# ColinWine/Multi-modal-Multi-label-Facial-Action-Unit-Detection-with-Transformer

Hardware: NVIDIA B200
Metric: AVFormer hot-path clips/sec (forward) (higher is better)
Workload: dtype bf16

## Files before the change

include/avformer_b200.h:

```cpp
#ifndef AVFORMER_B200_H_
#define AVFORMER_B200_H_

#include <stddef.h>
#include <stdint.h>

#ifdef __cplusplus
extern "C" {
#endif

#define AVF_ABI_VERSION 1

enum { AVF_FP32 = 0, AVF_BF16 = 1 };
enum { AVF_EINVAL = -1, AVF_ENODEVICE = -2, AVF_EWORKSPACE = -3, AVF_EUNSUPPORTED = -4 };

enum { AVF_EPI_BIAS = 1, AVF_EPI_GELU = 2, AVF_EPI_RESIDUAL = 4, AVF_EPI_DGELU = 8 ,
       AVF_EPI_SAVE_PRE = 16 ,
       AVF_EPI_DROPOUT = 32 ,
       AVF_EPI_ACCUMULATE = 64  };

typedef struct avf_layer_weights {
  const float* ln1_gamma;
  const float* ln1_beta;
  const void*  w_qkv;
  const void*  w_out;
  const float* b_out;
  const float* ln2_gamma;
  const float* ln2_beta;
  const void*  w_ff1;
  const float* b_ff1;
  const void*  w_ff2;
  const float* b_ff2;
} avf_layer_weights;

typedef struct avf_stack_shape {
  int32_t n_seq;
  int32_t n_tok;
  int32_t dim;
  int32_t heads;
  int32_t dim_head;
  int32_t mlp_dim;
  int32_t depth;
} avf_stack_shape;

int         avf_abi_version(void);
const char* avf_last_error(void);
uint64_t    avf_launch_count(void);
int         avf_device_info(int32_t* sm_count, int32_t* cc, int32_t* has_tcgen05);

int         avf_set_fused_enabled(int enabled);
int         avf_encoder_fused_supported(const avf_stack_shape* s, int mode);
int         avf_set_sm_cap(int cap);
int         avf_set_pdl_enabled(int enabled);
int         avf_debug_fused_prof(uint64_t* out64, int reset);
int         avf_debug_set_trap_buffer(void* host_mapped_words);
int         avf_debug_tmap_cache(uint64_t* hits, uint64_t* misses);
int         avf_debug_gemm_prof(uint64_t* out16);

size_t avf_encoder_workspace_bytes(const avf_stack_shape* s, int mode);

int avf_encoder_stack_fwd(int mode, const avf_stack_shape* s, const avf_layer_weights* layers,
                          float* x, int32_t ld_x, float* out, int32_t ld_out,
                          void* workspace, size_t workspace_bytes, void* stream);

int avf_layernorm_fwd(int out_mode, const float* x, int32_t ld_x, const float* gamma, const float* beta,
                      void* y, int32_t rows, int32_t dim, void* stream);
int avf_linear_fwd(int mode, const void* a, int32_t lda, const void* w, const float* bias,
                   const float* residual, int32_t ld_res, void* c, int32_t ldc, int c_mode,
                   int32_t m, int32_t n, int32_t k, int epilogue_flags, void* stream);
int avf_attention_fwd(int io_mode, const void* qkv, void* out, int32_t n_seq, int32_t n_tok,
                      int32_t heads, int32_t dim_head, void* stream);

int avf_sformer_tokens_pack(int io_mode, const void* fmap, const float* pos, float* x,
                            int32_t n_frames, int32_t dim, int32_t hw, void* stream);
int avf_sformer_tokens_unpack(int io_mode, const float* x, void* fmap,
                              int32_t n_frames, int32_t dim, int32_t hw, void* stream);
int avf_sformer_fwd(int mode, int io_mode, const avf_stack_shape* s, const avf_layer_weights* layers,
                    const float* pos, const void* fmap_in, void* fmap_out,
                    void* workspace, size_t workspace_bytes, void* stream);
size_t avf_sformer_workspace_bytes(const avf_stack_shape* s, int mode);

int avf_tformer_embed(int io_mode, const void* frames, const float* cls_token, const float* pos, float* x,
                      int32_t n_clips, int32_t n_frames, int32_t dim, void* stream);
size_t avf_tformer_workspace_bytes(const avf_stack_shape* s, int mode);
int avf_tformer_fwd(int mode, int io_mode, const avf_stack_shape* s, const avf_layer_weights* layers, const void* frames,
                    const float* cls_token, const float* pos, float* cls_out, void* workspace, size_t workspace_bytes, void* stream);
int avf_tformer_cls_extract(const float* x, float* cls, int32_t n_clips, int32_t n_tok, int32_t dim, void* stream);

int avf_au_former_front_fwd(int mode, const float* emb, int32_t ld_emb,
                            const float* bn_gamma, const float* bn_beta, const float* bn_mean, const float* bn_var,
                            const void* w_cat, const float* b_cat, const float* pos, float* x,
                            int32_t n_clips, int32_t in_dim, int32_t emb_dim,
                            void* workspace, size_t workspace_bytes, void* stream);
int avf_token_front_fwd(int mode, const float* emb, int32_t ld_emb,
                        const float* bn_gamma, const float* bn_beta, const float* bn_mean, const float* bn_var,
                        const void* w_cat, const float* b_cat, const float* pos, float* x,
                        int32_t n_clips, int32_t in_dim, int32_t emb_dim, int32_t n_tok,
                        void* workspace, size_t workspace_bytes, void* stream);

int avf_au_logits_fwd(const float* x, int32_t ld_x, const float* w_last, float* out21, int32_t* decisions,
                      int32_t n_clips, int32_t dim, void* stream);
int avf_au_bce_loss(const float* logits, int32_t ld_logits, const float* labels, const float* pos_weight,
                    float* loss_out, float* dlogits, int32_t n_clips, void* stream);

int avf_au_confusion_update(const float* pred, int32_t ld_pred, float threshold, const float* labels, int32_t ld_labels, float ignore,
                            uint64_t* counts48, int32_t n_rows, void* stream);

size_t avf_peer_gather_bytes(int32_t world, size_t n_floats);
int avf_logits_push(const float* logits, size_t n_floats, const uint64_t* peer_base, int32_t world, int32_t rank, const uint32_t* state, void* stream);
int avf_logits_wait(const void* my_base, size_t n_floats, int32_t world, uint32_t* state, uint64_t timeout_ns, void* stream);

size_t avf_peer_allreduce_bytes(int32_t world, size_t n_floats);
int avf_grad_allreduce(const uint64_t* peer_base, size_t n_floats, int32_t world, int32_t rank, uint32_t* state, uint64_t timeout_ns, void* stream);

int avf_adam_allreduce_step(const uint64_t* peer_base, size_t n_floats, int32_t world, int32_t rank, uint32_t* state, uint64_t timeout_ns,
                            float* params, float* exp_avg, float* exp_avg_sq, void* bf16_shadow, float lr, float beta1, float beta2, float eps,
                            float weight_decay, int32_t step, int decoupled, float grad_scale, void* stream);

int avf_cast_f32_to_bf16(const float* src, void* dst, size_t n, void* stream);
int avf_cast_bf16_to_f32(const void* src, float* dst, size_t n, void* stream);
int avf_add_row_periodic(float* x, int32_t ld_x, const float* pos, int32_t rows, int32_t dim, int32_t period, void* stream);


typedef struct avf_layer_grads {
  float* ln1_gamma; float* ln1_beta; float* w_qkv; float* w_out; float* b_out;
  float* ln2_gamma; float* ln2_beta; float* w_ff1; float* b_ff1; float* w_ff2; float* b_ff2;
} avf_layer_grads;

size_t avf_gemm_workspace_bytes(int mode, int trans_a, int trans_b, int32_t m, int32_t n, int32_t k);
int avf_gemm(int mode, int trans_a, int trans_b, const void* a, int32_t lda, const void* b, int32_t ldb,
             const float* bias, const float* residual, int32_t ld_res, void* aux, int32_t ld_aux,
             void* c, int32_t ldc, int c_mode, int32_t m, int32_t n, int32_t k, int epilogue_flags,
             void* workspace, size_t workspace_bytes, void* stream);

size_t avf_encoder_tape_bytes(const avf_stack_shape* s, int mode);
size_t avf_encoder_bwd_workspace_bytes(const avf_stack_shape* s, int mode);
int avf_encoder_stack_fwd_train(int mode, const avf_stack_shape* s, const avf_layer_weights* layers,
                                const float* x, int32_t ld_x, float* out, int32_t ld_out,
                                void* tape, size_t tape_bytes, float dropout_p, uint64_t dropout_seed,
                                const uint32_t* dropout_salt, void* stream);
int avf_encoder_stack_bwd(int mode, const avf_stack_shape* s, const avf_layer_weights* layers,
                          const void* tape, size_t tape_bytes, float* dx, int32_t ld_dx,
                          const avf_layer_grads* grads, int accumulate, void* workspace, size_t workspace_bytes,
                          float dropout_p, uint64_t dropout_seed, const uint32_t* dropout_salt, void* stream);
int avf_dropout_mask(float dropout_p, uint64_t dropout_seed, const uint32_t* dropout_salt, int32_t layer, int32_t site,
                     int32_t rows, int32_t cols, float* out, void* stream);

size_t avf_colsum_workspace_bytes(int32_t rows, int32_t cols);
int avf_colsum(int in_mode, const void* x, size_t ld, int32_t rows, int32_t cols, float* out,
               void* workspace, size_t workspace_bytes, void* stream);
size_t avf_layernorm_bwd_workspace_bytes(int32_t rows, int32_t dim);
int avf_layernorm_bwd(const float* x, int32_t ld_x, const float* gamma, const float* dy_norm, float* dres, int32_t ld_d,
                      void* dx_bf16, float* dgamma, float* dbeta, float* dbias, int32_t rows, int32_t dim,
                      void* workspace, size_t workspace_bytes, void* stream);
int avf_attention_bwd(int io_mode, const void* qkv, const void* dout, void* dqkv, int32_t n_seq, int32_t n_tok,
                      int32_t heads, int32_t dim_head, void* stream);

size_t avf_au_former_front_tape_bytes(int mode, int32_t n_clips, int32_t in_dim);
int avf_au_former_front_fwd_train(int mode, const float* emb, int32_t ld_emb,
                                  const float* bn_gamma, const float* bn_beta, float* bn_mean, float* bn_var,
                                  int batch_stats, float momentum, const void* w_cat, const float* b_cat, const float* pos,
                                  float* x, int32_t n_clips, int32_t in_dim, int32_t emb_dim,
                                  void* tape, size_t tape_bytes, void* stream);
size_t avf_au_former_front_bwd_workspace_bytes(int mode, int32_t n_clips, int32_t in_dim, int32_t emb_dim);
int avf_au_former_front_bwd(int mode, const float* emb, int32_t ld_emb, const float* bn_gamma,
                            const float* bn_mean, const float* bn_var, int batch_stats, const void* w_cat,
                            const void* tape, size_t tape_bytes, const float* dx,
                            float* demb, int32_t ld_demb, float* dbn_gamma, float* dbn_beta, float* dw_cat, float* db_cat,
                            int32_t n_clips, int32_t in_dim, int32_t emb_dim,
                            void* workspace, size_t workspace_bytes, void* stream);

int avf_au_logits_bwd(const float* dlogits, int32_t ld_dlogits, const float* x, int32_t ld_x, const float* w_last,
                      float* dx, int32_t ld_dx, float* dw_last, int32_t n_clips, int32_t dim, void* stream);

int avf_adam_step(float* params, const float* grads, float* exp_avg, float* exp_avg_sq, void* bf16_shadow, size_t n,
                  float lr, float beta1, float beta2, float eps, float weight_decay, int32_t step, int decoupled,
                  float grad_scale, void* stream);

#ifdef __cplusplus
}
#endif
#endif
```

multi-modal-multi-label-facial-action-unit-detection-with-transformer_b200/_lib.py:

```python
from __future__ import annotations

import ctypes
import glob
import os
import shutil
import subprocess
import threading

_PKG = os.path.dirname(os.path.abspath(__file__))
_ROOT = os.path.dirname(_PKG)
_CSRC = os.path.join(_PKG, "csrc")
LIB_PATH = os.path.join(_PKG, "libavformer_b200.so")
_OVERRIDE = os.environ.get("AVF_LIB_OVERRIDE", "")

NVCC_FLAGS = [
    "-gencode", "arch=compute_100a,code=sm_100a", "-lineinfo", "-O3", "-std=c++17",
    "-Xcompiler", "-fPIC", "-shared", "-cudart", "static", "-t", "0",
]

AVF_FP32, AVF_BF16 = 0, 1
EPI_BIAS, EPI_GELU, EPI_RESIDUAL, EPI_DGELU, EPI_SAVE_PRE = 1, 2, 4, 8, 16

_c_p = ctypes.c_void_p
_i32 = ctypes.c_int32
_sz = ctypes.c_size_t


class LayerWeights(ctypes.Structure):
    _fields_ = [(n, _c_p) for n in ("ln1_gamma", "ln1_beta", "w_qkv", "w_out", "b_out", "ln2_gamma", "ln2_beta",
                                    "w_ff1", "b_ff1", "w_ff2", "b_ff2")]


class LayerGrads(ctypes.Structure):
    _fields_ = LayerWeights._fields_


class StackShape(ctypes.Structure):
    _fields_ = [(n, _i32) for n in ("n_seq", "n_tok", "dim", "heads", "dim_head", "mlp_dim", "depth")]


SIGNATURES = {
    "avf_abi_version": (ctypes.c_int, []),
    "avf_last_error": (ctypes.c_char_p, []),
    "avf_launch_count": (ctypes.c_uint64, []),
    "avf_device_info": (ctypes.c_int, [ctypes.POINTER(_i32)] * 3),
    "avf_set_fused_enabled": (ctypes.c_int, [ctypes.c_int]),
    "avf_encoder_fused_supported": (ctypes.c_int, [ctypes.POINTER(StackShape), ctypes.c_int]),
    "avf_debug_fused_prof": (ctypes.c_int, [ctypes.POINTER(ctypes.c_uint64), ctypes.c_int]),
    "avf_encoder_workspace_bytes": (_sz, [ctypes.POINTER(StackShape), ctypes.c_int]),
    "avf_encoder_stack_fwd": (ctypes.c_int, [ctypes.c_int, ctypes.POINTER(StackShape), ctypes.POINTER(LayerWeights), _c_p, _i32,
                                             _c_p, _i32, _c_p, _sz, _c_p]),
    "avf_layernorm_fwd": (ctypes.c_int, [ctypes.c_int, _c_p, _i32, _c_p, _c_p, _c_p, _i32, _i32, _c_p]),
    "avf_linear_fwd": (ctypes.c_int, [ctypes.c_int, _c_p, _i32, _c_p, _c_p, _c_p, _i32, _c_p, _i32, ctypes.c_int, _i32, _i32, _i32,
                                      ctypes.c_int, _c_p]),
    "avf_attention_fwd": (ctypes.c_int, [ctypes.c_int, _c_p, _c_p, _i32, _i32, _i32, _i32, _c_p]),
    "avf_sformer_tokens_pack": (ctypes.c_int, [ctypes.c_int, _c_p, _c_p, _c_p, _i32, _i32, _i32, _c_p]),
    "avf_sformer_tokens_unpack": (ctypes.c_int, [ctypes.c_int, _c_p, _c_p, _i32, _i32, _i32, _c_p]),
    "avf_sformer_workspace_bytes": (_sz, [ctypes.POINTER(StackShape), ctypes.c_int]),
    "avf_sformer_fwd": (ctypes.c_int, [ctypes.c_int, ctypes.c_int, ctypes.POINTER(StackShape), ctypes.POINTER(LayerWeights), _c_p, _c_p,
                                       _c_p, _c_p, _sz, _c_p]),
    "avf_tformer_embed": (ctypes.c_int, [ctypes.c_int, _c_p, _c_p, _c_p, _c_p, _i32, _i32, _i32, _c_p]),
    "avf_tformer_workspace_bytes": (_sz, [ctypes.POINTER(StackShape), ctypes.c_int]),
    "avf_tformer_fwd": (ctypes.c_int, [ctypes.c_int, ctypes.c_int, ctypes.POINTER(StackShape), ctypes.POINTER(LayerWeights), _c_p, _c_p, _c_p, _c_p,
                                       _c_p, _sz, _c_p]),
    "avf_tformer_cls_extract": (ctypes.c_int, [_c_p, _c_p, _i32, _i32, _i32, _c_p]),
    "avf_au_former_front_fwd": (ctypes.c_int, [ctypes.c_int, _c_p, _i32, _c_p, _c_p, _c_p, _c_p, _c_p, _c_p, _c_p, _c_p, _i32, _i32, _i32,
                                               _c_p, _sz, _c_p]),
    "avf_token_front_fwd": (ctypes.c_int, [ctypes.c_int, _c_p, _i32, _c_p, _c_p, _c_p, _c_p, _c_p, _c_p, _c_p, _c_p, _i32, _i32, _i32, _i32,
                                           _c_p, _sz, _c_p]),
    "avf_au_logits_fwd": (ctypes.c_int, [_c_p, _i32, _c_p, _c_p, _c_p, _i32, _i32, _c_p]),
    "avf_au_bce_loss": (ctypes.c_int, [_c_p, _i32, _c_p, _c_p, _c_p, _c_p, _i32, _c_p]),
    "avf_au_confusion_update": (ctypes.c_int, [_c_p, _i32, ctypes.c_float, _c_p, _i32, ctypes.c_float, _c_p, _i32, _c_p]),
    "avf_peer_gather_bytes": (_sz, [_i32, _sz]),
    "avf_logits_push": (ctypes.c_int, [_c_p, _sz, _c_p, _i32, _i32, _c_p, _c_p]),
    "avf_logits_wait": (ctypes.c_int, [_c_p, _sz, _i32, _c_p, ctypes.c_uint64, _c_p]),
    "avf_peer_allreduce_bytes": (_sz, [_i32, _sz]),
    "avf_grad_allreduce": (ctypes.c_int, [_c_p, _sz, _i32, _i32, _c_p, ctypes.c_uint64, _c_p]),
    "avf_adam_allreduce_step": (ctypes.c_int, [_c_p, _sz, _i32, _i32, _c_p, ctypes.c_uint64, _c_p, _c_p, _c_p, _c_p] + [ctypes.c_float] * 5
                                + [_i32, ctypes.c_int, ctypes.c_float, _c_p]),
    "avf_cast_f32_to_bf16": (ctypes.c_int, [_c_p, _c_p, _sz, _c_p]),
    "avf_cast_bf16_to_f32": (ctypes.c_int, [_c_p, _c_p, _sz, _c_p]),
    "avf_add_row_periodic": (ctypes.c_int, [_c_p, _i32, _c_p, _i32, _i32, _i32, _c_p]),
    "avf_gemm_workspace_bytes": (_sz, [ctypes.c_int, ctypes.c_int, ctypes.c_int, _i32, _i32, _i32]),
    "avf_gemm": (ctypes.c_int, [ctypes.c_int, ctypes.c_int, ctypes.c_int, _c_p, _i32, _c_p, _i32, _c_p, _c_p, _i32, _c_p, _i32, _c_p, _i32,
                                ctypes.c_int, _i32, _i32, _i32, ctypes.c_int, _c_p, _sz, _c_p]),
    "avf_encoder_tape_bytes": (_sz, [ctypes.POINTER(StackShape), ctypes.c_int]),
    "avf_encoder_bwd_workspace_bytes": (_sz, [ctypes.POINTER(StackShape), ctypes.c_int]),
    "avf_encoder_stack_fwd_train": (ctypes.c_int, [ctypes.c_int, ctypes.POINTER(StackShape), ctypes.POINTER(LayerWeights), _c_p, _i32, _c_p, _i32,
                                                   _c_p, _sz, ctypes.c_float, ctypes.c_uint64, _c_p, _c_p]),
    "avf_encoder_stack_bwd": (ctypes.c_int, [ctypes.c_int, ctypes.POINTER(StackShape), ctypes.POINTER(LayerWeights), _c_p, _sz, _c_p, _i32,
                                             ctypes.POINTER(LayerGrads), ctypes.c_int, _c_p, _sz, ctypes.c_float, ctypes.c_uint64, _c_p, _c_p]),
    "avf_dropout_mask": (ctypes.c_int, [ctypes.c_float, ctypes.c_uint64, _c_p, _i32, _i32, _i32, _i32, _c_p, _c_p]),
    "avf_set_sm_cap": (ctypes.c_int, [ctypes.c_int]),
    "avf_set_pdl_enabled": (ctypes.c_int, [ctypes.c_int]),
    "avf_debug_set_trap_buffer": (ctypes.c_int, [_c_p]),
    "avf_debug_gemm_prof": (ctypes.c_int, [ctypes.POINTER(ctypes.c_uint64)]),
    "avf_debug_tmap_cache": (ctypes.c_int, [ctypes.POINTER(ctypes.c_uint64), ctypes.POINTER(ctypes.c_uint64)]),
    "avf_colsum_workspace_bytes": (_sz, [_i32, _i32]),
    "avf_colsum": (ctypes.c_int, [ctypes.c_int, _c_p, _sz, _i32, _i32, _c_p, _c_p, _sz, _c_p]),
    "avf_layernorm_bwd_workspace_bytes": (_sz, [_i32, _i32]),
    "avf_layernorm_bwd": (ctypes.c_int, [_c_p, _i32, _c_p, _c_p, _c_p, _i32, _c_p, _c_p, _c_p, _c_p, _i32, _i32, _c_p, _sz, _c_p]),
    "avf_attention_bwd": (ctypes.c_int, [ctypes.c_int, _c_p, _c_p, _c_p, _i32, _i32, _i32, _i32, _c_p]),
    "avf_au_former_front_tape_bytes": (_sz, [ctypes.c_int, _i32, _i32]),
    "avf_au_former_front_fwd_train": (ctypes.c_int, [ctypes.c_int, _c_p, _i32, _c_p, _c_p, _c_p, _c_p, ctypes.c_int, ctypes.c_float, _c_p, _c_p,
                                                     _c_p, _c_p, _i32, _i32, _i32, _c_p, _sz, _c_p]),
    "avf_au_former_front_bwd_workspace_bytes": (_sz, [ctypes.c_int, _i32, _i32, _i32]),
    "avf_au_former_front_bwd": (ctypes.c_int, [ctypes.c_int, _c_p, _i32, _c_p, _c_p, _c_p, ctypes.c_int, _c_p, _c_p, _sz, _c_p, _c_p, _i32,
                                               _c_p, _c_p, _c_p, _c_p, _i32, _i32, _i32, _c_p, _sz, _c_p]),
    "avf_au_logits_bwd": (ctypes.c_int, [_c_p, _i32, _c_p, _i32, _c_p, _c_p, _i32, _c_p, _i32, _i32, _c_p]),
    "avf_adam_step": (ctypes.c_int, [_c_p, _c_p, _c_p, _c_p, _c_p, _sz] + [ctypes.c_float] * 5 + [_i32, ctypes.c_int, ctypes.c_float, _c_p]),
}

_lock = threading.Lock()
_lib = None


def sources():
    return sorted(glob.glob(os.path.join(_CSRC, "*.cu")))


def _stale() -> bool:
    if not os.path.exists(LIB_PATH):
        return True
    t = os.path.getmtime(LIB_PATH)
    deps = sources() + glob.glob(os.path.join(_CSRC, "*.cuh")) + glob.glob(os.path.join(_CSRC, "*.h")) + \
        [os.path.join(_ROOT, "include", "avformer_b200.h")]
    return any(os.path.getmtime(d) > t for d in deps)


def build(force: bool = False, verbose: bool = False, out: str = "") -> str:
    if out:
        force = True
    if not force and not _stale():
        return LIB_PATH
    nvcc = shutil.which("nvcc") or "/usr/local/cuda/bin/nvcc"
    if not os.path.exists(nvcc):
        raise RuntimeError("avformer_b200: nvcc not found and libavformer_b200.so is missing/stale; cannot build the CUDA path")
    extra = os.environ.get("AVF_NVCC_EXTRA", "").split()
    cmd = [nvcc] + NVCC_FLAGS + extra + (["-Xptxas", "-v"] if verbose else []) + ["-o", out or LIB_PATH] + sources()
    res = subprocess.run(cmd, capture_output=True, text=True)
    if res.returncode != 0:
        raise RuntimeError("avformer_b200: nvcc failed\n" + res.stdout + res.stderr)
    if verbose:
        print(res.stderr)
    return out or LIB_PATH


def lib() -> ctypes.CDLL:
    global _lib
    if _lib is not None:
        return _lib
    with _lock:
        if _lib is None:
            if _OVERRIDE:
                handle = ctypes.CDLL(_OVERRIDE)
            else:
                try:
                    build()
                except RuntimeError:
                    if not os.path.exists(LIB_PATH):
                        raise
                handle = ctypes.CDLL(LIB_PATH)
            for name, (res, args) in SIGNATURES.items():
                fn = getattr(handle, name)
                fn.restype, fn.argtypes = res, args
            if os.environ.get("AVF_PDL", "") in ("0", "off"):
                handle.avf_set_pdl_enabled(0)
            if handle.avf_abi_version() != 1:
                raise RuntimeError("avformer_b200: ABI version mismatch")
            _lib = handle
    return _lib


def check(rc: int, what: str = "") -> None:
    if rc != 0:
        msg = lib().avf_last_error().decode("utf-8", "replace")
        raise RuntimeError(f"avformer_b200 {what} failed (code {rc}): {msg}")
```

multi-modal-multi-label-facial-action-unit-detection-with-transformer_b200/csrc/avf_api.cu:

```cuda
#include <atomic>
#include <cstdarg>
#include <cstdio>
#include <cstring>

#include "avf_common.cuh"
#include "avf_internal.h"

namespace avf {

static thread_local char g_err[512] = "";
static std::atomic<uint64_t> g_launches{0};
static std::atomic<int> g_pdl{1};
bool pdl_enabled() { return g_pdl.load() != 0; }
static std::atomic<int> g_sm_cap{0};
int sm_cap() { return g_sm_cap.load(); }
static std::atomic<int> g_fused{1};

void count_launch() { g_launches.fetch_add(1, std::memory_order_relaxed); }

void set_error(const char* fmt, ...) {
  va_list ap;
  va_start(ap, fmt);
  vsnprintf(g_err, sizeof(g_err), fmt, ap);
  va_end(ap);
}

int check_cuda(cudaError_t e, const char* what) {
  if (e == cudaSuccess) return 0;
  set_error("CUDA error %d (%s) at %s", int(e), cudaGetErrorString(e), what);
  return int(e);
}

static int require_device() {
  static int state = 0;
  if (state == 0) {
    int n = 0;
    cudaError_t e = cudaGetDeviceCount(&n);
    if (e != cudaSuccess || n == 0) {
      cudaGetLastError();
      state = -1;
    } else {
      state = 1;
    }
  }
  if (state < 0) {
    set_error("no CUDA device: the AVFormer B200 path has no CPU fallback");
    return AVF_ENODEVICE;
  }
  return 0;
}

static bool tcgen05_ok() {
  static int state = 0;
  if (state == 0) {
    int dev = 0, major = 0;
    if (cudaGetDevice(&dev) == cudaSuccess && cudaDeviceGetAttribute(&major, cudaDevAttrComputeCapabilityMajor, dev) == cudaSuccess)
      state = (major == 10) ? 1 : -1;
    else
      state = -1;
  }
  return state > 0;
}

static inline size_t align_up(size_t v, size_t a = 256) { return (v + a - 1) / a * a; }
static inline size_t elt(int mode) { return mode == AVF_BF16 ? 2 : 4; }

struct EncoderWs {
  void* ln;
  void* qkv;
  void* attn;
  void* hid;
  size_t total;
};

static EncoderWs carve_encoder_ws(const avf_stack_shape* s, int mode, void* base) {
  const size_t R = size_t(s->n_seq) * s->n_tok, I = size_t(s->heads) * s->dim_head, e = elt(mode);
  uint8_t* p = static_cast<uint8_t*>(base);
  EncoderWs w;
  size_t off = 0;
  w.ln = p + off;   off += align_up(R * s->dim * e);
  w.qkv = p + off;  off += align_up(R * 3 * I * e);
  w.attn = p + off; off += align_up(R * I * e);
  w.hid = p + off;  off += align_up(R * s->mlp_dim * e);
  w.total = off;
  return w;
}

static int check_shape(const avf_stack_shape* s) {
  AVF_REQUIRE(s != nullptr, AVF_EINVAL, "null stack shape");
  AVF_REQUIRE(s->n_seq > 0 && s->n_tok > 0 && s->depth > 0, AVF_EINVAL, "empty stack: n_seq=%d n_tok=%d depth=%d", s->n_seq, s->n_tok, s->depth);
  AVF_REQUIRE(s->dim % 128 == 0 && s->dim <= 1536, AVF_EUNSUPPORTED, "dim=%d must be a multiple of 128 (<= 1536)", s->dim);
  AVF_REQUIRE(s->dim_head == 32 || s->dim_head == 64, AVF_EUNSUPPORTED, "dim_head=%d (supported: 32, 64)", s->dim_head);
  AVF_REQUIRE((s->heads * s->dim_head) % 64 == 0 && s->mlp_dim % 64 == 0, AVF_EUNSUPPORTED, "inner=%d / mlp=%d must be multiples of 64", s->heads * s->dim_head, s->mlp_dim);
  AVF_REQUIRE(s->n_tok <= 64, AVF_EUNSUPPORTED, "n_tok=%d: sequences longer than 64 tokens are not part of this path", s->n_tok);
  return 0;
}

int linear(int mode, const void* a, int lda, const void* w, const float* bias, const float* res, int ld_res, void* c, int ldc,
           int c_mode, int m, int n, int k, int flags, cudaStream_t st) {
  if (mode == AVF_BF16) {
    AVF_REQUIRE(tcgen05_ok(), AVF_EUNSUPPORTED, "bf16 mode needs an sm_100 device (tcgen05)");
    return linear_umma(a, lda, w, bias, res, ld_res, c, ldc, c_mode, m, n, k, flags, st);
  }
  return linear_f32(static_cast<const float*>(a), lda, static_cast<const float*>(w), bias, res, ld_res, c, ldc, c_mode, m, n, k, flags, st);
}

static int encoder_stack(int mode, const avf_stack_shape* s, const avf_layer_weights* L, float* x, int ld_x, float* out, int ld_out,
                         void* ws, size_t ws_bytes, cudaStream_t st) {
  int e = check_shape(s);
  if (e) return e;
  AVF_REQUIRE(mode == AVF_BF16 || mode == AVF_FP32, AVF_EINVAL, "mode=%d", mode);
  AVF_REQUIRE(L != nullptr && x != nullptr && ws != nullptr, AVF_EINVAL, "null pointer argument");
  if (mode == AVF_BF16 && g_fused.load() && tcgen05_ok() && encoder_fused_supported(s) && ld_x % 4 == 0 && (out == nullptr || ld_out % 4 == 0))
    return encoder_fused(1, s, L, x, ld_x, out ? out : x, out ? ld_out : ld_x, nullptr, nullptr, st);
  const EncoderWs w = carve_encoder_ws(s, mode, ws);
  AVF_REQUIRE(ws_bytes >= w.total, AVF_EWORKSPACE, "workspace too small: %zu < %zu bytes", ws_bytes, w.total);
  const int R = s->n_seq * s->n_tok, D = s->dim, I = s->heads * s->dim_head, M = s->mlp_dim;
  for (int l = 0; l < s->depth; ++l) {
    const avf_layer_weights& W = L[l];
    if ((e = layernorm(mode, x, ld_x, W.ln1_gamma, W.ln1_beta, w.ln, R, D, st))) return e;
    if ((e = linear(mode, w.ln, D, W.w_qkv, nullptr, nullptr, 0, w.qkv, 3 * I, mode, R, 3 * I, D, 0, st))) return e;
    if ((e = attention_small(mode, w.qkv, w.attn, s->n_seq, s->n_tok, s->heads, s->dim_head, st))) return e;
    if ((e = linear(mode, w.attn, I, W.w_out, W.b_out, x, ld_x, x, ld_x, AVF_FP32, R, D, I, AVF_EPI_BIAS | AVF_EPI_RESIDUAL, st))) return e;
    if ((e = layernorm(mode, x, ld_x, W.ln2_gamma, W.ln2_beta, w.ln, R, D, st))) return e;
    if ((e = linear(mode, w.ln, D, W.w_ff1, W.b_ff1, nullptr, 0, w.hid, M, mode, R, M, D, AVF_EPI_BIAS | AVF_EPI_GELU, st))) return e;
    const bool last = (l == s->depth - 1) && out != nullptr;
    if ((e = linear(mode, w.hid, M, W.w_ff2, W.b_ff2, x, ld_x, last ? out : x, last ? ld_out : ld_x, AVF_FP32, R, D, M,
                    AVF_EPI_BIAS | AVF_EPI_RESIDUAL, st)))
      return e;
  }
  return 0;
}

}

using namespace avf;

extern "C" {

int avf_abi_version(void) { return AVF_ABI_VERSION; }

const char* avf_last_error(void) { return g_err; }

uint64_t avf_launch_count(void) { return g_launches.load(std::memory_order_relaxed); }

int avf_set_fused_enabled(int enabled) {
  const int old = g_fused.exchange(enabled ? 1 : 0);
  return old;
}

int avf_set_pdl_enabled(int enabled) { return g_pdl.exchange(enabled ? 1 : 0); }

int avf_set_sm_cap(int cap) { return g_sm_cap.exchange(cap > 0 ? cap : 0); }

int avf_encoder_fused_supported(const avf_stack_shape* s, int mode) {
  return (s != nullptr && mode == AVF_BF16 && s->n_seq > 0 && encoder_fused_supported(s)) ? 1 : 0;
}

int avf_debug_fused_prof(uint64_t* out64, int reset) { return fused_prof_read(reinterpret_cast<unsigned long long*>(out64), reset); }

int avf_debug_tmap_cache(uint64_t* hits, uint64_t* misses) {
  if (hits == nullptr || misses == nullptr) return AVF_EINVAL;
  tmap_cache_stats(hits, misses);
  return 0;
}

int avf_debug_gemm_prof(uint64_t* out16) { return gemm_prof_read(reinterpret_cast<unsigned long long*>(out16)); }

int avf_debug_set_trap_buffer(void* host_mapped_words) { return fused_set_trap_buffer(host_mapped_words); }

int avf_device_info(int32_t* sm_count, int32_t* cc, int32_t* has_tcgen05) {
  int e = require_device();
  if (e) return e;
  int dev = 0, sms = 0, major = 0, minor = 0;
  AVF_CUDA(cudaGetDevice(&dev));
  AVF_CUDA(cudaDeviceGetAttribute(&sms, cudaDevAttrMultiProcessorCount, dev));
  AVF_CUDA(cudaDeviceGetAttribute(&major, cudaDevAttrComputeCapabilityMajor, dev));
  AVF_CUDA(cudaDeviceGetAttribute(&minor, cudaDevAttrComputeCapabilityMinor, dev));
  if (sm_count) *sm_count = sms;
  if (cc) *cc = major * 10 + minor;
  if (has_tcgen05) *has_tcgen05 = major == 10 ? 1 : 0;
  return 0;
}

size_t avf_encoder_workspace_bytes(const avf_stack_shape* s, int mode) {
  if (s == nullptr || s->n_seq <= 0 || s->n_tok <= 0) return 0;
  return carve_encoder_ws(s, mode, nullptr).total;
}

int avf_encoder_stack_fwd(int mode, const avf_stack_shape* s, const avf_layer_weights* layers, float* x, int32_t ld_x, float* out,
                          int32_t ld_out, void* workspace, size_t workspace_bytes, void* stream) {
  int e = require_device();
  if (e) return e;
  return encoder_stack(mode, s, layers, x, ld_x, out, ld_out, workspace, workspace_bytes, static_cast<cudaStream_t>(stream));
}

int avf_layernorm_fwd(int out_mode, const float* x, int32_t ld_x, const float* gamma, const float* beta, void* y, int32_t rows,
                      int32_t dim, void* stream) {
  int e = require_device();
  if (e) return e;
  AVF_REQUIRE(x && gamma && beta && y, AVF_EINVAL, "layernorm: null pointer");
  return layernorm(out_mode, x, ld_x, gamma, beta, y, rows, dim, static_cast<cudaStream_t>(stream));
}

int avf_linear_fwd(int mode, const void* a, int32_t lda, const void* w, const float* bias, const float* residual, int32_t ld_res,
                   void* c, int32_t ldc, int c_mode, int32_t m, int32_t n, int32_t k, int epilogue_flags, void* stream) {
  int e = require_device();
  if (e) return e;
  AVF_REQUIRE(a && w && c, AVF_EINVAL, "linear: null pointer");
  AVF_REQUIRE(!(epilogue_flags & AVF_EPI_BIAS) || bias, AVF_EINVAL, "linear: bias flag without bias");
  AVF_REQUIRE(!(epilogue_flags & AVF_EPI_RESIDUAL) || residual, AVF_EINVAL, "linear: residual flag without residual");
  return linear(mode, a, lda, w, bias, residual, ld_res, c, ldc, c_mode, m, n, k, epilogue_flags, static_cast<cudaStream_t>(stream));
}

int avf_attention_fwd(int io_mode, const void* qkv, void* out, int32_t n_seq, int32_t n_tok, int32_t heads, int32_t dim_head, void* stream) {
  int e = require_device();
  if (e) return e;
  AVF_REQUIRE(qkv && out, AVF_EINVAL, "attention: null pointer");
  return attention_small(io_mode, qkv, out, n_seq, n_tok, heads, dim_head, static_cast<cudaStream_t>(stream));
}

int avf_sformer_tokens_pack(int io_mode, const void* fmap, const float* pos, float* x, int32_t n_frames, int32_t dim, int32_t hw, void* stream) {
  int e = require_device();
  if (e) return e;
  AVF_REQUIRE(fmap && x, AVF_EINVAL, "sformer_tokens_pack: null pointer");
  return sformer_pack(io_mode, fmap, pos, x, n_frames, dim, hw, static_cast<cudaStream_t>(stream));
}

int avf_sformer_tokens_unpack(int io_mode, const float* x, void* fmap, int32_t n_frames, int32_t dim, int32_t hw, void* stream) {
  int e = require_device();
  if (e) return e;
  AVF_REQUIRE(fmap && x, AVF_EINVAL, "sformer_tokens_unpack: null pointer");
  return sformer_unpack(io_mode, x, fmap, n_frames, dim, hw, static_cast<cudaStream_t>(stream));
}

size_t avf_sformer_workspace_bytes(const avf_stack_shape* s, int mode) {
  if (s == nullptr || s->n_seq <= 0 || s->n_tok <= 0) return 0;
  return align_up(size_t(s->n_seq) * s->n_tok * s->dim * 4) + carve_encoder_ws(s, mode, nullptr).total + align_up(encoder_fused_scratch_bytes());
}

int avf_sformer_fwd(int mode, int io_mode, const avf_stack_shape* s, const avf_layer_weights* layers, const float* pos,
                    const void* fmap_in, void* fmap_out, void* workspace, size_t workspace_bytes, void* stream) {
  int e = require_device();
  if (e) return e;
  if ((e = check_shape(s))) return e;
  AVF_REQUIRE(layers && pos && fmap_in && fmap_out && workspace, AVF_EINVAL, "sformer_fwd: null pointer");
  const size_t need = avf_sformer_workspace_bytes(s, mode);
  AVF_REQUIRE(workspace_bytes >= need, AVF_EWORKSPACE, "workspace too small: %zu < %zu bytes", workspace_bytes, need);
  cudaStream_t st = static_cast<cudaStream_t>(stream);
  if (mode == AVF_BF16 && io_mode == AVF_BF16 && g_fused.load() && tcgen05_ok() && encoder_fused_supported(s))
    return encoder_fused(0, s, layers, fmap_in, 0, fmap_out, 0, pos, workspace, st);
  float* x = static_cast<float*>(workspace);
  const size_t xbytes = align_up(size_t(s->n_seq) * s->n_tok * s->dim * 4);
  if ((e = sformer_pack(io_mode, fmap_in, pos, x, s->n_seq, s->dim, s->n_tok, st))) return e;
  if ((e = encoder_stack(mode, s, layers, x, s->dim, nullptr, 0, static_cast<uint8_t*>(workspace) + xbytes, workspace_bytes - xbytes, st))) return e;
  return sformer_unpack(io_mode, x, fmap_out, s->n_seq, s->dim, s->n_tok, st);
}

int avf_tformer_embed(int io_mode, const void* frames, const float* cls_token, const float* pos, float* x, int32_t n_clips,
                      int32_t n_frames, int32_t dim, void* stream) {
  int e = require_device();
  if (e) return e;
  AVF_REQUIRE(frames && cls_token && pos && x, AVF_EINVAL, "tformer_embed: null pointer");
  return tformer_embed(io_mode, frames, cls_token, pos, x, n_clips, n_frames, dim, static_cast<cudaStream_t>(stream));
}

size_t avf_tformer_workspace_bytes(const avf_stack_shape* s, int mode) {
  if (s == nullptr || s->n_seq <= 0 || s->n_tok <= 0) return 0;
  const size_t B = s->n_seq, D = s->dim, I = size_t(s->heads) * s->dim_head, M = s->mlp_dim, e = elt(mode);
  return align_up(B * s->n_tok * D * 4) + carve_encoder_ws(s, mode, nullptr).total + align_up(B * D * 4) + align_up(B * D * e) + align_up(B * I * e) +
         align_up(B * M * e);
}

int avf_tformer_fwd(int mode, int io_mode, const avf_stack_shape* s, const avf_layer_weights* layers, const void* frames,
                    const float* cls_token, const float* pos, float* cls_out, void* workspace, size_t workspace_bytes, void* stream) {
  int e = require_device();
  if (e) return e;
  if ((e = check_shape(s))) return e;
  AVF_REQUIRE(layers && frames && cls_token && pos && cls_out && workspace, AVF_EINVAL, "tformer_fwd: null pointer");
  AVF_REQUIRE(s->n_tok >= 2, AVF_EINVAL, "tformer_fwd: n_tok=%d (cls + at least one frame)", s->n_tok);
  const size_t need = avf_tformer_workspace_bytes(s, mode);
  AVF_REQUIRE(workspace_bytes >= need, AVF_EWORKSPACE, "workspace too small: %zu < %zu bytes", workspace_bytes, need);
  cudaStream_t st = static_cast<cudaStream_t>(stream);
  const int B = s->n_seq, N = s->n_tok, R = B * N, D = s->dim, I = s->heads * s->dim_head, M = s->mlp_dim;
  uint8_t* p = static_cast<uint8_t*>(workspace);
  float* x = reinterpret_cast<float*>(p);   p += align_up(size_t(R) * D * 4);
  void* enc_ws = p;
  const EncoderWs w = carve_encoder_ws(s, mode, enc_ws);
  p += w.total;
  float* xc = reinterpret_cast<float*>(p);  p += align_up(size_t(B) * D * 4);
  void* lnc = p;                            p += align_up(size_t(B) * D * elt(mode));
  void* oc = p;                             p += align_up(size_t(B) * I * elt(mode));
  void* hc = p;
  if ((e = tformer_embed(io_mode, frames, cls_token, pos, x, B, N - 1, D, st))) return e;
  if (s->depth > 1) {
    avf_stack_shape head = *s;
    head.depth = s->depth - 1;
    if ((e = encoder_stack(mode, &head, layers, x, D, nullptr, 0, enc_ws, w.total, st))) return e;
  }
  const avf_layer_weights& W = layers[s->depth - 1];
  if ((e = layernorm(mode, x, D, W.ln1_gamma, W.ln1_beta, w.ln, R, D, st))) return e;
  if ((e = linear(mode, w.ln, D, W.w_qkv, nullptr, nullptr, 0, w.qkv, 3 * I, mode, R, 3 * I, D, 0, st))) return e;
  if (mode == AVF_BF16) {
    if ((e = attention_mma_bf16(w.qkv, oc, B, N, s->heads, s->dim_head, st, 1))) return e;
  } else {
    if ((e = attention_small(mode, w.qkv, w.attn, B, N, s->heads, s->dim_head, st))) return e;
    AVF_CUDA(cudaMemcpy2DAsync(oc, size_t(I) * 4, w.attn, size_t(N) * I * 4, size_t(I) * 4, B, cudaMemcpyDeviceToDevice, st));
  }
  if ((e = rows_gather(x, size_t(N) * D, xc, B, D, st))) return e;
  if ((e = linear(mode, oc, I, W.w_out, W.b_out, xc, D, xc, D, AVF_FP32, B, D, I, AVF_EPI_BIAS | AVF_EPI_RESIDUAL, st))) return e;
  if ((e = layernorm(mode, xc, D, W.ln2_gamma, W.ln2_beta, lnc, B, D, st))) return e;
  if ((e = linear(mode, lnc, D, W.w_ff1, W.b_ff1, nullptr, 0, hc, M, mode, B, M, D, AVF_EPI_BIAS | AVF_EPI_GELU, st))) return e;
  return linear(mode, hc, M, W.w_ff2, W.b_ff2, xc, D, cls_out, D, AVF_FP32, B, D, M, AVF_EPI_BIAS | AVF_EPI_RESIDUAL, st);
}

int avf_tformer_cls_extract(const float* x, float* cls, int32_t n_clips, int32_t n_tok, int32_t dim, void* stream) {
  int e = require_device();
  if (e) return e;
  AVF_REQUIRE(x && cls, AVF_EINVAL, "tformer_cls_extract: null pointer");
  return rows_gather(x, size_t(n_tok) * dim, cls, n_clips, dim, static_cast<cudaStream_t>(stream));
}

int avf_token_front_fwd(int mode, const float* emb, int32_t ld_emb, const float* bn_gamma, const float* bn_beta, const float* bn_mean,
                        const float* bn_var, const void* w_cat, const float* b_cat, const float* pos, float* x, int32_t n_clips,
                        int32_t in_dim, int32_t emb_dim, int32_t n_tok, void* workspace, size_t workspace_bytes, void* stream) {
  int e = require_device();
  if (e) return e;
  AVF_REQUIRE(emb && bn_gamma && bn_beta && bn_mean && bn_var && w_cat && b_cat && pos && x && workspace, AVF_EINVAL, "token_front: null pointer");
  AVF_REQUIRE(n_clips > 0 && in_dim > 0 && emb_dim > 0 && n_tok > 0, AVF_EINVAL, "token_front: n_clips=%d n_tok=%d", n_clips, n_tok);
  const size_t need = align_up(size_t(n_clips) * in_dim * elt(mode));
  AVF_REQUIRE(workspace_bytes >= need, AVF_EWORKSPACE, "workspace too small: %zu < %zu bytes", workspace_bytes, need);
  cudaStream_t st = static_cast<cudaStream_t>(stream);
  if ((e = bn_rows(mode, emb, ld_emb, bn_gamma, bn_beta, bn_mean, bn_var, workspace, n_clips, in_dim, st))) return e;
  if ((e = linear(mode, workspace, in_dim, w_cat, b_cat, nullptr, 0, x, n_tok * emb_dim, AVF_FP32, n_clips, n_tok * emb_dim, in_dim, AVF_EPI_BIAS, st))) return e;
  return add_row_periodic(x, emb_dim, pos, n_clips * n_tok, emb_dim, n_tok, st);
}

int avf_au_former_front_fwd(int mode, const float* emb, int32_t ld_emb, const float* bn_gamma, const float* bn_beta, const float* bn_mean,
                            const float* bn_var, const void* w_cat, const float* b_cat, const float* pos, float* x, int32_t n_clips,
                            int32_t in_dim, int32_t emb_dim, void* workspace, size_t workspace_bytes, void* stream) {
  return avf_token_front_fwd(mode, emb, ld_emb, bn_gamma, bn_beta, bn_mean, bn_var, w_cat, b_cat, pos, x, n_clips, in_dim, emb_dim, 12, workspace,
                             workspace_bytes, stream);
}

int avf_au_logits_fwd(const float* x, int32_t ld_x, const float* w_last, float* out21, int32_t* decisions, int32_t n_clips, int32_t dim, void* stream) {
  int e = require_device();
  if (e) return e;
  AVF_REQUIRE(x && w_last, AVF_EINVAL, "au_logits: null pointer");
  return au_logits(x, ld_x, w_last, out21, decisions, n_clips, dim, static_cast<cudaStream_t>(stream));
}

int avf_au_bce_loss(const float* logits, int32_t ld_logits, const float* labels, const float* pos_weight, float* loss_out, float* dlogits,
                    int32_t n_clips, void* stream) {
  int e = require_device();
  if (e) return e;
  AVF_REQUIRE(logits && labels && pos_weight && loss_out, AVF_EINVAL, "au_bce_loss: null pointer");
  return au_bce(logits, ld_logits, labels, pos_weight, loss_out, dlogits, n_clips, static_cast<cudaStream_t>(stream));
}

size_t avf_peer_gather_bytes(int32_t world, size_t n_floats) { return (world > 0 && world <= 1024) ? peer_gather_bytes(world, n_floats) : 0; }

int avf_logits_push(const float* logits, size_t n_floats, const uint64_t* peer_base, int32_t world, int32_t rank, const uint32_t* state, void* stream) {
  int e = require_device();
  if (e) return e;
  AVF_REQUIRE(logits && peer_base && state, AVF_EINVAL, "logits_push: null pointer");
  AVF_REQUIRE(world > 0 && world <= 1024 && rank >= 0 && rank < world && n_floats > 0, AVF_EINVAL, "logits_push: world %d rank %d n %zu", world, rank, n_floats);
  return logits_push(logits, n_floats, reinterpret_cast<const unsigned long long*>(peer_base), world, rank, state, static_cast<cudaStream_t>(stream));
}

int avf_logits_wait(const void* my_base, size_t n_floats, int32_t world, uint32_t* state, uint64_t timeout_ns, void* stream) {
  int e = require_device();
  if (e) return e;
  AVF_REQUIRE(my_base && state, AVF_EINVAL, "logits_wait: null pointer");
  AVF_REQUIRE(world > 0 && world <= 1024 && n_floats > 0, AVF_EINVAL, "logits_wait: world %d n %zu", world, n_floats);
  return logits_wait(my_base, n_floats, world, state, timeout_ns, static_cast<cudaStream_t>(stream));
}

size_t avf_peer_allreduce_bytes(int32_t world, size_t n_floats) { return (world > 0 && world <= 16) ? peer_allreduce_bytes(world, n_floats) : 0; }

int avf_grad_allreduce(const uint64_t* peer_base, size_t n_floats, int32_t world, int32_t rank, uint32_t* state, uint64_t timeout_ns, void* stream) {
  int e = require_device();
  if (e) return e;
  AVF_REQUIRE(peer_base && state, AVF_EINVAL, "grad_allreduce: null pointer");
  AVF_REQUIRE(world > 0 && world <= 16 && rank >= 0 && rank < world && n_floats > 0, AVF_EINVAL, "grad_allreduce: world %d (1..16) rank %d n %zu", world, rank, n_floats);
  return grad_allreduce(reinterpret_cast<const unsigned long long*>(peer_base), n_floats, world, rank, state, timeout_ns, static_cast<cudaStream_t>(stream));
}

int avf_adam_allreduce_step(const uint64_t* peer_base, size_t n_floats, int32_t world, int32_t rank, uint32_t* state, uint64_t timeout_ns, float* params,
                            float* exp_avg, float* exp_avg_sq, void* bf16_shadow, float lr, float beta1, float beta2, float eps, float weight_decay, int32_t step,
                            int decoupled, float grad_scale, void* stream) {
  int e = require_device();
  if (e) return e;
  AVF_REQUIRE(peer_base && state, AVF_EINVAL, "adam_allreduce_step: null pointer");
  AVF_REQUIRE(world > 0 && world <= 16 && rank >= 0 && rank < world && n_floats > 0, AVF_EINVAL, "adam_allreduce_step: world %d (1..16) rank %d n %zu", world, rank, n_floats);
  return adam_allreduce_step(reinterpret_cast<const unsigned long long*>(peer_base), n_floats, world, rank, state, timeout_ns, params, exp_avg, exp_avg_sq, bf16_shadow,
                             lr, beta1, beta2, eps, weight_decay, step, decoupled, grad_scale, static_cast<cudaStream_t>(stream));
}

int avf_au_confusion_update(const float* pred, int32_t ld_pred, float threshold, const float* labels, int32_t ld_labels, float ignore,
                            uint64_t* counts48, int32_t n_rows, void* stream) {
  int e = require_device();
  if (e) return e;
  return au_confusion(pred, ld_pred, threshold, labels, ld_labels, ignore, reinterpret_cast<unsigned long long*>(counts48), n_rows,
                      static_cast<cudaStream_t>(stream));
}

int avf_cast_f32_to_bf16(const float* src, void* dst, size_t n, void* stream) {
  int e = require_device();
  if (e) return e;
  AVF_REQUIRE((src && dst) || n == 0, AVF_EINVAL, "cast: null pointer");
  return cast_f32_bf16(src, dst, n, static_cast<cudaStream_t>(stream));
}

int avf_cast_bf16_to_f32(const void* src, float* dst, size_t n, void* stream) {
  int e = require_device();
  if (e) return e;
  AVF_REQUIRE((src && dst) || n == 0, AVF_EINVAL, "cast: null pointer");
  return cast_bf16_f32(src, dst, n, static_cast<cudaStream_t>(stream));
}

int avf_add_row_periodic(float* x, int32_t ld_x, const float* pos, int32_t rows, int32_t dim, int32_t period, void* stream) {
  int e = require_device();
  if (e) return e;
  AVF_REQUIRE(x && pos, AVF_EINVAL, "add_row_periodic: null pointer");
  return add_row_periodic(x, ld_x, pos, rows, dim, period, static_cast<cudaStream_t>(stream));
}

}
```

multi-modal-multi-label-facial-action-unit-detection-with-transformer_b200/csrc/avf_internal.h:

```cpp
#pragma once
#include <cuda_runtime.h>
#include <stddef.h>

#include "../../include/avformer_b200.h"
#include "avf_common.cuh"

namespace avf {

int layernorm(int out_mode, const float* x, int ld_x, const float* g, const float* b, void* y, int rows, int dim, cudaStream_t st);
int bn_rows(int out_mode, const float* x, int ld_x, const float* g, const float* b, const float* mean, const float* var, void* y,
            int rows, int dim, cudaStream_t st);
int sformer_pack(int io_mode, const void* fmap, const float* pos, float* x, int n_frames, int dim, int hw, cudaStream_t st);
int sformer_unpack(int io_mode, const float* x, void* fmap, int n_frames, int dim, int hw, cudaStream_t st);
int tformer_embed(int io_mode, const void* frames, const float* cls, const float* pos, float* x, int n_clips, int T, int dim, cudaStream_t st);
int rows_gather(const float* x, size_t src_row_stride, float* y, int rows, int dim, cudaStream_t st);
int add_row_periodic(float* x, int ld_x, const float* pos, int rows, int dim, int period, cudaStream_t st);
int cast_f32_bf16(const float* s, void* d, size_t n, cudaStream_t st);
int cast_bf16_f32(const void* s, float* d, size_t n, cudaStream_t st);
int au_logits(const float* x, int ld_x, const float* w_last, float* out21, int* decisions, int n_clips, int dim, cudaStream_t st);
int au_bce(const float* logits, int ld, const float* labels, const float* pw, float* loss_out, float* dlogits, int n_clips, cudaStream_t st);
size_t peer_gather_bytes(int world, size_t n);
int logits_push(const float* logits, size_t n, const unsigned long long* peer_base, int world, int rank, const uint32_t* state, cudaStream_t st);
size_t peer_allreduce_bytes(int world, size_t n);
int grad_allreduce(const unsigned long long* peer_base, size_t n, int world, int rank, uint32_t* state, unsigned long long timeout_ns, cudaStream_t st);
int adam_allreduce_step(const unsigned long long* peer_base, size_t n, int world, int rank, uint32_t* state, unsigned long long timeout_ns, float* p, float* m,
                        float* v, void* shadow, float lr, float b1, float b2, float eps, float wd, int step, int decoupled, float grad_scale, cudaStream_t st);
int logits_wait(const void* my_base, size_t n, int world, uint32_t* state, unsigned long long timeout_ns, cudaStream_t st);
int au_confusion(const float* pred, int ld_pred, float thresh, const float* labels, int ld_lab, float ignore, unsigned long long* counts, int n_rows,
                 cudaStream_t st);

int linear_f32(const float* a, int lda, const float* w, const float* bias, const float* res, int ld_res, void* c, int ldc,
               int c_mode, int m, int n, int k, int flags, cudaStream_t st);
int attention_small(int io_mode, const void* qkv, void* out, int n_seq, int n_tok, int heads, int dim_head, cudaStream_t st);

int gemm_f32(int trans_a, int trans_b, const float* a, int lda, const float* w, int ldw, const float* bias, const float* res, int ld_res,
             float* aux, int ld_aux, void* c, int ldc, int c_mode, int m, int n, int k, int flags, cudaStream_t st, DropSpec drop = DropSpec{});

size_t colsum_workspace_bytes(int rows, int cols);
int colsum(int in_mode, const void* x, size_t ld, int rows, int cols, float* out, float beta, void* ws, size_t ws_bytes, cudaStream_t st);
size_t layernorm_bwd_workspace_bytes(int rows, int dim);
int layernorm_bwd(const float* x, int ld_x, const float* gamma, const float* dyn, float* dres, int ld_d, void* dxb, int dxb_mode, float* dgamma,
                  float* dbeta, float* dbias, float beta_acc, int rows, int dim, void* ws, size_t ws_bytes, cudaStream_t st,
                  DropSpec drop_in = DropSpec{}, DropSpec drop_out = DropSpec{});
int masked_copy(const float* x, void* y, int y_mode, int rows, int dim, DropSpec drop, cudaStream_t st);
int dropout_mask(float* out, int rows, int cols, DropSpec drop, cudaStream_t st);
int attention_bwd(int io_mode, const void* qkv, const void* dout, void* dqkv, int n_seq, int n_tok, int heads, int dim_head, cudaStream_t st);
int au_logits_bwd(const float* dl, int ld_dl, const float* x, int ld_x, const float* w_last, float* dx, int ld_dx, float* dw, int n_clips,
                  int dim, cudaStream_t st);
int bn_train_fwd(int out_mode, const float* x, int ld_x, const float* g, const float* b, float* run_mean, float* run_var, float momentum,
                 void* y, float* save_mean, float* save_rstd, int rows, int dim, cudaStream_t st);
int bn_bwd(const float* x, int ld_x, const float* dy, const float* g, const float* mean, const float* rstd_or_var, int batch_stats, float* dx,
           int ld_dx, float* dgamma, float* dbeta, int rows, int dim, cudaStream_t st);
int adam_step(float* p, const float* g, float* m, float* v, void* shadow, size_t n, float lr, float b1, float b2, float eps, float wd, int step,
              int decoupled, float grad_scale, cudaStream_t st);

int attention_mma_bf16(const void* qkv, void* out, int n_seq, int n_tok, int heads, int dim_head, cudaStream_t st, int q_rows = 0);
int attention_bwd_mma_bf16(const void* qkv, const void* dout, void* dqkv, int n_seq, int n_tok, int heads, int dim_head, cudaStream_t st);

bool encoder_fused_supported(const avf_stack_shape* s);
int fused_prof_read(unsigned long long* out64, int reset);
int fused_set_trap_buffer(void* host_mapped_words);
size_t encoder_fused_scratch_bytes();
int encoder_fused(int io_kind, const avf_stack_shape* s, const avf_layer_weights* L, const void* in, int ld_in, void* out, int ld_out,
                  const float* pos, void* scratch, cudaStream_t st);

int gemm_umma(int trans_a, int trans_b, const void* a, int lda, const void* w, int ldw, const float* bias, const float* res, int ld_res,
              const void* aux, int ld_aux, void* c, int ldc, int c_mode, int m, int n, int k, int flags, void* ws, size_t ws_bytes,
              cudaStream_t stream, DropSpec drop = DropSpec{});
size_t gemm_umma_workspace_bytes(int m, int n, int k);
void tmap_cache_stats(uint64_t* hits, uint64_t* misses);
int gemm_prof_read(unsigned long long* out16);
int linear_umma(const void* a, int lda, const void* w, const float* bias, const float* res, int ld_res, void* c, int ldc,
                int c_mode, int m, int n, int k, int flags, cudaStream_t st);

}
```

multi-modal-multi-label-facial-action-unit-detection-with-transformer_b200/csrc/avf_layer_fused.cu:

```cuda
#include <cuda.h>
#include <stdlib.h>

#include "avf_common.cuh"
#include "avf_fused_helpers.cuh"
#include "avf_internal.h"

namespace avf {

int make_tmap_bf16_2d(CUtensorMap* tm, const void* ptr, uint64_t rows, uint64_t cols, uint64_t ld, uint32_t box_rows, uint32_t box_cols = 64);

namespace {
using namespace fused;

#ifndef AVF_PROD_POLL
#define AVF_PROD_POLL 2
#endif
#ifndef AVF_PROD_FASTPATH
#define AVF_PROD_FASTPATH 1
#endif
#ifndef AVF_O_TMEM
#define AVF_O_TMEM 1
#endif

constexpr int DIM = 256, HEADS = 8, DH = 32;
constexpr int MAX_DEPTH = 3, MAX_MLP = 1024;
#ifndef AVF_FUSED_NSPLIT
#define AVF_FUSED_NSPLIT 2
#endif
constexpr int NSPLIT = AVF_FUSED_NSPLIT;
static_assert(NSPLIT == 2, "two threads per token row (the packed softmax exchanges a pair)");
constexpr int WORKER_T0 = 96;
constexpr int NUM_WORKERS = 128 * NSPLIT;
constexpr int NUM_THREADS = WORKER_T0 + NUM_WORKERS;
constexpr int RING = 9, RING_LO = 2, RING_HI = 4, SLOT_BYTES = 16384;
#ifndef AVF_QRING
#define AVF_QRING 6
#endif
constexpr int QRING = AVF_QRING, QSLOT_BYTES = 12288;
#ifndef AVF_MLP_GROUP
#define AVF_MLP_GROUP 4
#endif
constexpr int MLPG = AVF_MLP_GROUP;
static_assert(MLPG == 2 || MLPG == 4, "MLP group size");

constexpr int OFF_A0 = 0;
constexpr int OFF_Q = 65536;
constexpr int OFF_K = OFF_Q + 8192;
constexpr int OFF_V = OFF_K + 8192;
constexpr int OFF_RING = OFF_V + 16384;
constexpr int OFF_OST = OFF_RING + (RING_HI - RING_LO) * SLOT_BYTES;
constexpr int OFF_QRING = OFF_OST + (AVF_O_TMEM ? 0 : 8192);
constexpr int OFF_OUTST = OFF_QRING;
static_assert(QRING * QSLOT_BYTES >= 2 * 64 * 256 * 2, "the NCHW output staging lives in the QKV ring");
static_assert(QRING >= 6 && QRING < 8, "one head-full barrier per head parity needs 6 or 7 sub-slots (see qkv_producer_main)");
constexpr int QRING_END = OFF_QRING + QRING * QSLOT_BYTES;
constexpr int OFF_XCH = QRING_END > OFF_Q + RING * SLOT_BYTES ? QRING_END : OFF_Q + RING * SLOT_BYTES;
static_assert(OFF_XCH - OFF_Q >= RING * SLOT_BYTES, "the nine MLP ring slots fit in [OFF_Q, OFF_XCH)");
static_assert(OFF_RING == OFF_Q + RING_LO * SLOT_BYTES, "ring slots are contiguous from OFF_Q");
__host__ __device__ constexpr int slot_offset(uint32_t s) { return OFF_Q + int(s) * SLOT_BYTES; }
constexpr int OFF_VEC = OFF_XCH + 2 * 128 * 4 * 4;
constexpr int V_BOUT = 0, V_BFF2 = 256, V_BFF1 = 512;
constexpr int V_B16 = V_BFF1 + MAX_MLP;
constexpr int OFF_BAR = OFF_VEC + (V_B16 + 512) * 4;
constexpr int SMEM_USED = OFF_BAR + 512;
constexpr int SMEM_ALLOC = SMEM_USED + 1024;
static_assert(SMEM_ALLOC <= 232448, "shared memory budget");

#ifndef AVF_A0_HALF
#define AVF_A0_HALF 1
#endif
#if AVF_A0_HALF
__device__ __forceinline__ constexpr int kpanel(int i) { return ((i & 1) << 1) | (i >> 1); }
#else
__device__ __forceinline__ constexpr int kpanel(int i) { return i; }
#endif

constexpr uint32_t TM_X = 0, TM_D1 = 256, TM_O = 352, TM_S = 384, TM_H0 = 256, TM_H1 = 384;

enum {
  B_RING_FULL = 0, B_RING_EMPTY = RING, B_X0_FULL = 2 * RING, B_A0_FREE, B_A0_READY, B_D1_FULL, B_STAGED, B_S_FULL, B_P_READY, B_O_FULL,
  B_O_DRAINED, B_X1_FULL, B_HACC_FULL, B_HACC_FULL1, B_H_READY, B_H_READY1, B_X2_FULL,
  B_QG_FULL, B_QR_EMPTY = B_QG_FULL + 2, B_A1_FREE = B_QR_EMPTY + QRING, B_OUT_READ, B_QKV_FREE, B_G_FULL, B_TQ_FULL = B_G_FULL + 8, B_A0_HALF = B_TQ_FULL + 4, NUM_BARS
};
static_assert(NUM_BARS * 8 + 8 + 16 <= 512, "barrier block (+ TMEM slot + tile queue)");

__device__ __forceinline__ int* tile_queue(uint64_t* bars) { return reinterpret_cast<int*>(bars + NUM_BARS) + 2; }
__device__ __forceinline__ int next_tile(uint64_t* bars, uint32_t k) {
  mbar_wait(&bars[B_TQ_FULL + (k & 3u)], (k >> 2) & 1u);
  return *reinterpret_cast<volatile int*>(tile_queue(bars) + (k & 3u));
}

enum { IO_NCHW_BF16 = 0, IO_ROWS_F32 = 1 };
constexpr int POS_LD = 64;

enum { PW_INPUT = 0, PW_VEC, PW_LN1, PW_WAIT_D1, PW_E1, PW_WAIT_O, PW_E3, PW_WAIT_S, PW_E2, PW_WAIT_X1, PW_LN2, PW_WAIT_HACC, PW_GELU, PW_WAIT_X2,
       PW_OUTPUT, PW_TILES, PW_E2_LD, PW_E2_EXP, PW_E2_XCH, PW_E2_ST,
       PM_WAIT_A0 = 32, PM_QKV, PM_WAIT_STAGED, PM_S, PM_WAIT_P, PM_PV, PM_WAIT_OD7, PM_OUT, PM_WAIT_A0B, PM_FF1, PM_WAIT_H, PM_FF2, PM_RINGWAIT,
       PM_RW_QKV, PM_RW_OUT, PM_RW_FF1, PM_RW_FF2, PM_REFILL_CYC, PM_REFILL_N };

struct LayerArgs {
  CUtensorMap tm_qkv, tm_out, tm_w1, tm_w2;
  const float *ln1_g, *ln1_b, *b_out, *ln2_g, *ln2_b, *b_ff1, *b_ff2;
  uint64_t pad_;
};

struct FusedArgs {
  LayerArgs layer[MAX_DEPTH];
  const void* in;
  void* out;
  const float* pos;
  const float* pos_t;
  int ld_in, ld_out;
  int* tile_counter;
  int n_seq, n_tok, slot, slot_log2, spt, n_tiles, n_chunks, depth;
};

__device__ unsigned* g_trap_buffer = nullptr;

constexpr int CW = DIM / NSPLIT;

struct Worker {
  uint8_t* smem;
  uint64_t* bars;
  const float* vec;
  uint32_t tl;
  int lane, q, g, row;
  uint32_t xslot;

  __device__ __forceinline__ const float* exchange(float mine) {
    float* s = reinterpret_cast<float*>(smem + OFF_XCH) + xslot * (128 * 4);
    xslot ^= 1;
    s[row * 4 + g] = mine;
    bar_sync(1 + q, 32 * NSPLIT);
    return s + row * 4;
  }
  __device__ __forceinline__ float2 exchange_pair(float a, float b) {
    static_assert(NSPLIT == 2, "pair exchange is written for two threads per row");
    float* s = reinterpret_cast<float*>(smem + OFF_XCH) + xslot * (128 * 4);
    xslot ^= 1;
    *reinterpret_cast<float2*>(s + row * 4 + g * 2) = make_float2(a, b);
    bar_sync(1 + q, 32 * NSPLIT);
    return *reinterpret_cast<const float2*>(s + row * 4 + (g ^ 1) * 2);
  }
  __device__ __forceinline__ float exchange_sum(float mine) {
    const float* v = exchange(mine);
    if constexpr (NSPLIT == 2) return v[0] + v[1];
    const float4 f = *reinterpret_cast<const float4*>(v);
    return (f.x + f.y) + (f.z + f.w);
  }
  __device__ __forceinline__ float exchange_max(float mine) {
    const float* v = exchange(mine);
    if constexpr (NSPLIT == 2) return fmaxf(v[0], v[1]);
    const float4 f = *reinterpret_cast<const float4*>(v);
    return fmaxf(fmaxf(f.x, f.y), fmaxf(f.z, f.w));
  }
  __device__ __forceinline__ void arrive(int bar) {
    fence_proxy_async_smem();
    tc_fence_before();
    __syncwarp();
    if (lane == 0) mbar_arrive(&bars[bar]);
  }
  __device__ __forceinline__ void arrive_tmem_only(int bar) {
    tc_fence_before();
    __syncwarp();
    if (lane == 0) mbar_arrive(&bars[bar]);
  }
  struct Stats {
    float shift, s, ss;
    __device__ __forceinline__ void add(const float (&x)[32], bool first) {
      if (first) shift = x[0];
      const uint64_t nshift = f2_pack(-shift, -shift);
      uint64_t s2 = f2_pack(0.f, 0.f), q2 = s2;
#pragma unroll
      for (int j = 0; j < 32; j += 2) {
        const uint64_t d = f2_add(f2_pack(x[j], x[j + 1]), nshift);
        s2 = f2_add(s2, d);
        q2 = f2_fma(d, d, q2);
      }
      float a, b;
      f2_unpack(s2, a, b);
      s += a + b;
      f2_unpack(q2, a, b);
      ss += a + b;
    }
  };
  __device__ __forceinline__ void finish_stats(const Stats& st, float& mean, float& rstd) {
    constexpr float n = float(CW);
    const float mean_g = st.shift + st.s * (1.f / n);
    const float m2_g = fmaxf(st.ss - st.s * st.s * (1.f / n), 0.f);
    mean = exchange_sum(mean_g) * (1.f / NSPLIT);
    const float dm = mean_g - mean;
    const float m2 = exchange_sum(fmaf(dm * dm, n, m2_g));
    rstd = rsqrtf(m2 * (1.f / DIM) + 1e-5f);
  }
  __device__ __forceinline__ void stats_from_tmem(float& mean, float& rstd) {
    Stats st{0.f, 0.f, 0.f};
#pragma unroll
    for (int c0 = 0; c0 < CW; c0 += 32) {
      float x[32];
      tmem_ld32(tl + TM_X + g * CW + c0, reinterpret_cast<uint32_t(&)[32]>(x));
      tmem_ld_wait();
      st.add(x, c0 == 0);
    }
    finish_stats(st, mean, rstd);
  }
  __device__ __forceinline__ void normalize_from_tmem(float mean, float rstd, int ln_sel, int v_next_bias) {
    const int cbase = g * CW;
    const float nmr = -mean * rstd;
    const uint64_t rstd2 = f2_pack(rstd, rstd), nmr2 = f2_pack(nmr, nmr);
#pragma unroll 1
    for (int c0 = 0; c0 < CW; c0 += 32) {
      float x[32];
      tmem_ld32(tl + TM_X + cbase + c0, reinterpret_cast<uint32_t(&)[32]>(x));
      tmem_ld_wait();
      const int col0 = cbase + c0;
      uint8_t* dst = smem + OFF_A0 + (col0 >> 6) * 16384 + row * 128;
      const int chunk0 = (col0 & 63) >> 3;
#pragma unroll
      for (int ch = 0; ch < 4; ++ch) {
        const __nv_bfloat16* v16 = reinterpret_cast<const __nv_bfloat16*>(vec + V_B16) + ln_sel * 512 + col0 + ch * 8;
        const uint4 gm = *reinterpret_cast<const uint4*>(v16), bt = *reinterpret_cast<const uint4*>(v16 + 256);
        uint4 pk;
        pk.x = fma_bf16x2(cvt_bf16x2_pair(f2_fma(f2_pack(x[ch * 8], x[ch * 8 + 1]), rstd2, nmr2)), gm.x, bt.x);
        pk.y = fma_bf16x2(cvt_bf16x2_pair(f2_fma(f2_pack(x[ch * 8 + 2], x[ch * 8 + 3]), rstd2, nmr2)), gm.y, bt.y);
        pk.z = fma_bf16x2(cvt_bf16x2_pair(f2_fma(f2_pack(x[ch * 8 + 4], x[ch * 8 + 5]), rstd2, nmr2)), gm.z, bt.z);
        pk.w = fma_bf16x2(cvt_bf16x2_pair(f2_fma(f2_pack(x[ch * 8 + 6], x[ch * 8 + 7]), rstd2, nmr2)), gm.w, bt.w);
        *reinterpret_cast<uint4*>(dst + (((chunk0 + ch) ^ (row & 7)) << 4)) = pk;
      }
#pragma unroll
      for (int j = 0; j < 32; j += 4) {
        const ulonglong2 b = *reinterpret_cast<const ulonglong2*>(vec + v_next_bias + col0 + j);
        f2_unpack(f2_add(f2_pack(x[j], x[j + 1]), b.x), x[j], x[j + 1]);
        f2_unpack(f2_add(f2_pack(x[j + 2], x[j + 3]), b.y), x[j + 2], x[j + 3]);
      }
      tmem_st32(tl + TM_X + col0, reinterpret_cast<const uint32_t(&)[32]>(x));
#if AVF_A0_HALF
      if (c0 == 32) arrive(B_A0_HALF);
#endif
    }
    tmem_st_wait();
    arrive(B_A0_READY);
  }
};

template <int NC, int TAILV>
__device__ __forceinline__ float softmax_fixed(Worker& w, uint32_t ts, uint32_t tp, float sm_scale, Prof& pf) {
  float s[NC][8];
#pragma unroll
  for (int c = 0; c < NC; ++c) tmem_ld8(ts + c * 8, reinterpret_cast<uint32_t(&)[8]>(s[c]));
  tmem_ld_wait();
  pf.mark(PW_E2_LD);
  float mc[NC];
#pragma unroll
  for (int c = 0; c < NC; ++c) {
    if (TAILV > 0 && c == NC - 1) {
      mc[c] = s[c][0];
#pragma unroll
      for (int j = 1; j < 8; ++j)
        if (j < TAILV) mc[c] = fmaxf(mc[c], s[c][j]);
    } else {
      mc[c] = fmaxf(fmaxf(fmaxf(s[c][0], s[c][1]), fmaxf(s[c][2], s[c][3])), fmaxf(fmaxf(s[c][4], s[c][5]), fmaxf(s[c][6], s[c][7])));
    }
  }
  float mloc = mc[0];
#pragma unroll
  for (int c = 1; c < NC; ++c) mloc = fmaxf(mloc, mc[c]);
  pf.mark(PW_E2_EXP);
  const float mrow = w.exchange_max(mloc);
  pf.mark(PW_E2_XCH);
  const float nml = -mrow * sm_scale;
  const uint64_t sc2 = f2_pack(sm_scale, sm_scale), nml2 = f2_pack(nml, nml);
  uint64_t sum2 = f2_pack(0.f, 0.f);
  float sum_lo = 0.f;
#pragma unroll
  for (int c = 0; c < NC; ++c) {
    const int nv = (TAILV > 0 && c == NC - 1) ? TAILV : 8;
    uint32_t e[4];
#pragma unroll
    for (int j = 0; j < 4; ++j) {
      if (2 * j + 1 < nv) {
        e[j] = ex2_bf16x2(cvt_bf16x2_pair(f2_fma(f2_pack(s[c][2 * j], s[c][2 * j + 1]), sc2, nml2)));
        sum2 = f2_add(sum2, f2_pack(__uint_as_float(e[j] << 16), __uint_as_float(e[j] & 0xFFFF0000u)));
      } else if (2 * j < nv) {
        e[j] = ex2_bf16x2(cvt_bf16x2(fmaf(s[c][2 * j], sm_scale, nml), -INFINITY)) & 0xFFFFu;
        sum_lo += __uint_as_float(e[j] << 16);
      } else {
        e[j] = 0u;
      }
    }
    tmem_st4(tp + c * 4, e[0], e[1], e[2], e[3]);
  }
  float a, b;
  f2_unpack(sum2, a, b);
  return sum_lo + (a + b);
}

__host__ __device__ constexpr int slot_of(int n_tok) { return n_tok <= 16 ? 16 : (n_tok <= 32 ? 32 : 64); }
__host__ __device__ constexpr int log2_of(int v) { return v == 16 ? 4 : (v == 32 ? 5 : 6); }

template <int IO, int NTOK>
__device__ void worker_main(const FusedArgs& a, uint8_t* smem, uint64_t* bars, uint32_t tmem) {
  Worker w;
  w.smem = smem;
  w.bars = bars;
  w.vec = reinterpret_cast<const float*>(smem + OFF_VEC);
  const int wt = threadIdx.x - WORKER_T0;
  w.lane = wt & 31;
  w.q = (threadIdx.x >> 5) & 3;
  w.g = wt >> 7;
  w.row = w.q * 32 + w.lane;
  w.tl = tmem + (uint32_t(w.q * 32) << 16);
  w.xslot = 0;
  const int q = w.q, g = w.g, row = w.row;
  const uint32_t tl = w.tl;
  const float* vec = w.vec;
  const int n_tok = NTOK ? NTOK : a.n_tok, slot = NTOK ? slot_of(NTOK) : a.slot, spt = NTOK ? 128 / slot_of(NTOK) : a.spt;
  const int slot_log2 = NTOK ? log2_of(slot_of(NTOK)) : a.slot_log2;
  const int seq_in_tile = row >> slot_log2, t_in_seq = row & (slot - 1);
  const int lo = seq_in_tile * slot, hi = lo + n_tok;
  const int s0 = (q * 32) >> slot_log2, s1 = (q * 32 + 31) >> slot_log2;
  const int c_lo = (s0 * slot) >> 3, c_hi = (s1 * slot + n_tok + 7) >> 3;
  constexpr int MAXC = 8 / NSPLIT;
  const int per = (c_hi - c_lo + NSPLIT - 1) / NSPLIT;
  const int my_c0 = c_lo + g * per;
  const int my_nc = max(0, min(per, c_hi - my_c0));
  const bool warp_one_seq = s0 == s1;
  const float sm_scale = 1.4426950408889634f * rsqrtf(float(DH));
  uint32_t n_x0 = 0, n_x1 = 0, n_x2 = 0, n_hacc0 = 0, n_hacc1 = 0;
  bool vec_loaded = false;
  Prof pf;
  pf.start(blockIdx.x == 0 && wt == 0);

  for (uint32_t tk = 0;; ++tk) {
    const int tile = next_tile(bars, tk);
    if (tile < 0) break;
    const int seqs_here = min(spt, a.n_seq - tile * spt);
    const bool valid = seq_in_tile < seqs_here && t_in_seq < n_tok;
    const size_t grow = (size_t(tile) * spt + seq_in_tile) * n_tok + t_in_seq;

    float mean, rstd;
    {
      Worker::Stats st{0.f, 0.f, 0.f};
      const int t_safe = valid ? t_in_seq : 0, seq_safe = valid ? seq_in_tile : 0;
      const float* pp = (IO == IO_ROWS_F32 && a.pos != nullptr) ? a.pos + t_safe * DIM + g * CW : nullptr;
      const float4* ppt = reinterpret_cast<const float4*>(a.pos_t) + size_t(g * CW / 4) * POS_LD + t_safe;
      if constexpr (IO == IO_NCHW_BF16) mbar_wait(&bars[B_X0_FULL], (n_x0++) & 1);
      const __nv_bfloat16* src16 = reinterpret_cast<const __nv_bfloat16*>(smem + OFF_A0) + size_t(seq_safe * DIM + g * CW) * n_tok + t_safe;
      const float* src32 = static_cast<const float*>(a.in) + ((size_t(tile) * spt + seq_safe) * n_tok + t_safe) * a.ld_in + g * CW;
#pragma unroll 1
      for (int c0 = 0; c0 < CW; c0 += 32) {
        float x[32];
        if constexpr (IO == IO_NCHW_BF16) {
          float4 p[8];
#pragma unroll
#ifdef AVF_EXP_POS_HOT
          for (int j = 0; j < 8; ++j) p[j] = __ldg(ppt + j * POS_LD);
#else
          for (int j = 0; j < 8; ++j) p[j] = __ldg(ppt + (c0 / 4 + j) * POS_LD);
#endif
#pragma unroll
          for (int j = 0; j < 8; ++j) {
            f2_unpack(f2_add(f2_pack(__bfloat162float(src16[(c0 + 4 * j) * n_tok]), __bfloat162float(src16[(c0 + 4 * j + 1) * n_tok])),
                             f2_pack(p[j].x, p[j].y)), x[4 * j], x[4 * j + 1]);
            f2_unpack(f2_add(f2_pack(__bfloat162float(src16[(c0 + 4 * j + 2) * n_tok]), __bfloat162float(src16[(c0 + 4 * j + 3) * n_tok])),
                             f2_pack(p[j].z, p[j].w)), x[4 * j + 2], x[4 * j + 3]);
          }
        } else {
          float4 p4[8];
          if (pp != nullptr) {
#pragma unroll
            for (int j = 0; j < 8; ++j) p4[j] = __ldg(reinterpret_cast<const float4*>(pp + c0) + j);
          }
#pragma unroll
          for (int j = 0; j < 32; j += 4) {
            const float4 x4 = *reinterpret_cast<const float4*>(src32 + c0 + j);
            x[j] = x4.x; x[j + 1] = x4.y; x[j + 2] = x4.z; x[j + 3] = x4.w;
          }
          if (pp != nullptr) {
#pragma unroll
            for (int j = 0; j < 8; ++j) {
              x[4 * j] += p4[j].x; x[4 * j + 1] += p4[j].y; x[4 * j + 2] += p4[j].z; x[4 * j + 3] += p4[j].w;
            }
          }
        }
        st.add(x, c0 == 0);
        tmem_st32(tl + TM_X + g * CW + c0, reinterpret_cast<const uint32_t(&)[32]>(x));
      }
      tmem_st_wait();
      w.finish_stats(st, mean, rstd);
      if constexpr (IO == IO_NCHW_BF16) {
        if (threadIdx.x == WORKER_T0) {
          bulk_wait_read0();
          mbar_arrive(&bars[B_OUT_READ]);
        }
        bar_sync(5, NUM_WORKERS);
      }
    }
    pf.mark(PW_INPUT);

    for (int l = 0; l < a.depth; ++l) {
      const LayerArgs& L = a.layer[l];
      if (a.depth > 1 || !vec_loaded) {
        if (vec_loaded) bar_sync(5, NUM_WORKERS);
        float* vs = reinterpret_cast<float*>(smem + OFF_VEC);
        for (int i = wt; i < DIM; i += NUM_WORKERS) {
          vs[V_BOUT + i] = L.b_out[i]; vs[V_BFF2 + i] = L.b_ff2[i];
          __nv_bfloat16* v16 = reinterpret_cast<__nv_bfloat16*>(vs + V_B16);
          v16[i] = __float2bfloat16_rn(L.ln1_g[i]); v16[256 + i] = __float2bfloat16_rn(L.ln1_b[i]);
          v16[512 + i] = __float2bfloat16_rn(L.ln2_g[i]); v16[768 + i] = __float2bfloat16_rn(L.ln2_b[i]);
        }
        for (int i = wt; i < a.n_chunks * 128; i += NUM_WORKERS) vs[V_BFF1 + i] = L.b_ff1[i];
        bar_sync(5, NUM_WORKERS);
        vec_loaded = true;
      }
      pf.mark(PW_VEC);
      w.normalize_from_tmem(mean, rstd, 0, V_BOUT);
      pf.mark(PW_LN1);

      float inv_l = 0.f;
#pragma unroll 1
      for (int h = 0; h <= HEADS; ++h) {
        if (h < HEADS) {
          mbar_wait(&bars[B_D1_FULL], h & 1);
          tc_fence_after();
          pf.mark(PW_WAIT_D1);
          constexpr int NCH = 12 / NSPLIT;
          const uint32_t sw = uint32_t((row >> 1) & 3);
          uint32_t r[NCH * 8];
          if constexpr (NSPLIT == 2) {
            tmem_ld32(tl + TM_D1 + g * 48, reinterpret_cast<uint32_t(&)[32]>(r[0]));
            tmem_ld16(tl + TM_D1 + g * 48 + 32, reinterpret_cast<uint32_t(&)[16]>(r[32]));
          } else {
            tmem_ld16(tl + TM_D1 + g * 24, reinterpret_cast<uint32_t(&)[16]>(r[0]));
            tmem_ld8(tl + TM_D1 + g * 24 + 16, reinterpret_cast<uint32_t(&)[8]>(r[16]));
          }
          tmem_ld_wait();
#pragma unroll
          for (int c = 0; c < NCH; ++c) {
            const int id = g * NCH + c;
            uint8_t* base = id < 4 ? smem + OFF_Q : (id < 8 ? smem + OFF_K : smem + OFF_V + (h & 1) * 8192);
            *reinterpret_cast<uint4*>(base + row * 64 + ((uint32_t(id & 3) ^ sw) << 4)) = pack8u(&r[c * 8]);
          }
          w.arrive(B_STAGED);
          pf.mark(PW_E1);
        }
        if (h > 0) {
          mbar_wait(&bars[B_O_FULL], (h - 1) & 1);
          tc_fence_after();
          pf.mark(PW_WAIT_O);
          constexpr int OW = DH / NSPLIT;
          uint32_t r[OW];
          if constexpr (OW == 16) tmem_ld16(tl + TM_O + g * OW, reinterpret_cast<uint32_t(&)[16]>(r[0]));
          else tmem_ld8(tl + TM_O + g * OW, reinterpret_cast<uint32_t(&)[8]>(r[0]));
          tmem_ld_wait();
#if AVF_FUSED_PACKED
          {
            const float* sums = reinterpret_cast<const float*>(smem + OFF_XCH) + ((h - 1) & 1) * (128 * 4) + row * 4 + 2;
            asm("rcp.approx.ftz.f32 %0, %1;" : "=f"(inv_l) : "f"(sums[0] + sums[1]));
          }
#endif
          const uint64_t inv2 = f2_pack(inv_l, inv_l);
#if AVF_O_TMEM
          static_assert(OW == 16, "TMEM-resident O operand is written for two threads per row");
          uint32_t pk[8];
#pragma unroll
          for (int j = 0; j < 8; ++j) pk[j] = cvt_bf16x2_pair(f2_mul(f2_pack(__uint_as_float(r[2 * j]), __uint_as_float(r[2 * j + 1])), inv2));
          tmem_st8(tl + TM_O + g * OW, pk);
          tmem_st_wait();
          w.arrive_tmem_only(B_O_DRAINED);
#else
          uint8_t* ob = smem + OFF_OST + row * 64;
          const uint32_t sw = uint32_t((row >> 1) & 3);
#pragma unroll
          for (int c = 0; c < OW / 8; ++c) {
            uint4 pk;
            pk.x = cvt_bf16x2_pair(f2_mul(f2_pack(__uint_as_float(r[c * 8]), __uint_as_float(r[c * 8 + 1])), inv2));
            pk.y = cvt_bf16x2_pair(f2_mul(f2_pack(__uint_as_float(r[c * 8 + 2]), __uint_as_float(r[c * 8 + 3])), inv2));
            pk.z = cvt_bf16x2_pair(f2_mul(f2_pack(__uint_as_float(r[c * 8 + 4]), __uint_as_float(r[c * 8 + 5])), inv2));
            pk.w = cvt_bf16x2_pair(f2_mul(f2_pack(__uint_as_float(r[c * 8 + 6]), __uint_as_float(r[c * 8 + 7])), inv2));
            *reinterpret_cast<uint4*>(ob + ((uint32_t(g * (OW / 8) + c) ^ sw) << 4)) = pk;
          }
          w.arrive(B_O_DRAINED);
#endif
          pf.mark(PW_E3);
        }
        if (h < HEADS) {
          mbar_wait(&bars[B_S_FULL], h & 1);
          tc_fence_after();
          pf.mark(PW_WAIT_S);
          if constexpr (NTOK > 32 && NSPLIT == 2 && AVF_FUSED_PACKED) {
            constexpr int NCH_ALL = (NTOK + 7) / 8, NC1 = NCH_ALL - 4, TAILV = NTOK & 7;
            static_assert(NC1 >= 1 && NC1 <= 4, "softmax split");
            const uint32_t sb = tl + TM_S + uint32_t(seq_in_tile) * 64, pb = tl + TM_S + uint32_t(seq_in_tile) * 32;
            const float sum_g = g == 0 ? softmax_fixed<4, 0>(w, sb, pb, sm_scale, pf) : softmax_fixed<NC1, TAILV>(w, sb + 32, pb + 16, sm_scale, pf);
            reinterpret_cast<float*>(smem + OFF_XCH)[(h & 1) * (128 * 4) + row * 4 + 2 + g] = sum_g;
            if (g == seq_in_tile) {
              zero_p_columns(tl + TM_S, 32 * g + NCH_ALL * 4, 32 * g + 32);
            } else {
              tmem_st16_zero(tl + TM_S + 32 * g);
              tmem_st16_zero(tl + TM_S + 32 * g + 16);
            }
            tmem_st_wait();
            pf.mark(PW_E2_ST);
            w.arrive_tmem_only(B_P_READY);
            pf.mark(PW_E2);
          } else {
          float s[MAXC][8];
#pragma unroll
          for (int c = 0; c < MAXC; ++c)
            if (c < my_nc) tmem_ld8(tl + TM_S + (my_c0 + c) * 8, reinterpret_cast<uint32_t(&)[8]>(s[c]));
          tmem_ld_wait();
          pf.mark(PW_E2_LD);
          float mloc = -INFINITY;
#pragma unroll
          for (int c = 0; c < MAXC; ++c) {
            if (c < my_nc) {
              const int col0 = (my_c0 + c) * 8;
              if (!warp_one_seq || col0 + 8 > hi) {
#pragma unroll
                for (int j = 0; j < 8; ++j) s[c][j] = (col0 + j >= lo && col0 + j < hi) ? s[c][j] : -INFINITY;
              }
              mloc = fmaxf(mloc, fmaxf(fmaxf(fmaxf(s[c][0], s[c][1]), fmaxf(s[c][2], s[c][3])), fmaxf(fmaxf(s[c][4], s[c][5]), fmaxf(s[c][6], s[c][7]))));
            }
          }
#if AVF_FUSED_PACKED
          pf.mark(PW_E2_EXP);
          const float mrow = w.exchange_max(mloc);
          pf.mark(PW_E2_XCH);
          const float nml = -mrow * sm_scale;
          float sum_g = 0.f;
#pragma unroll
          for (int c = 0; c < MAXC; ++c) {
            if (c < my_nc) {
              uint32_t e[4];
#pragma unroll
              for (int j = 0; j < 4; ++j) {
                e[j] = ex2_bf16x2(cvt_bf16x2(fmaf(s[c][2 * j], sm_scale, nml), fmaf(s[c][2 * j + 1], sm_scale, nml)));
                sum_g += __uint_as_float(e[j] << 16) + __uint_as_float(e[j] & 0xFFFF0000u);
              }
              tmem_st4(tl + TM_S + (my_c0 + c) * 4, e[0], e[1], e[2], e[3]);
            }
          }
          reinterpret_cast<float*>(smem + OFF_XCH)[(h & 1) * (128 * 4) + row * 4 + 2 + g] = sum_g;
#else
          const float nml = mloc == -INFINITY ? 0.f : -mloc * sm_scale;
          float sum_g = 0.f;
#pragma unroll
          for (int c = 0; c < MAXC; ++c) {
            if (c < my_nc) {
#pragma unroll
              for (int j = 0; j < 8; ++j) s[c][j] = fast_exp2(fmaf(s[c][j], sm_scale, nml));
              sum_g += ((s[c][0] + s[c][1]) + (s[c][2] + s[c][3])) + ((s[c][4] + s[c][5]) + (s[c][6] + s[c][7]));
            }
          }
          pf.mark(PW_E2_EXP);
          const float2 other = w.exchange_pair(mloc, sum_g);
          pf.mark(PW_E2_XCH);
          const float mrow = fmaxf(mloc, other.x);
          const float f = fast_exp2((mloc - mrow) * sm_scale), fo = fast_exp2((other.x - mrow) * sm_scale);
          inv_l = 1.f / fmaf(sum_g, f, other.y * fo);
#pragma unroll
          for (int c = 0; c < MAXC; ++c) {
            if (c < my_nc)
              tmem_st4(tl + TM_S + (my_c0 + c) * 4, pack_bf16x2(s[c][0] * f, s[c][1] * f), pack_bf16x2(s[c][2] * f, s[c][3] * f),
                       pack_bf16x2(s[c][4] * f, s[c][5] * f), pack_bf16x2(s[c][6] * f, s[c][7] * f));
          }
#endif
          {
            const int z_lo = g * 32, z_hi = z_lo + 32, w_lo = c_lo * 4, w_hi = c_hi * 4;
            zero_p_columns(tl + TM_S, z_lo, min(z_hi, max(z_lo, w_lo)));
            zero_p_columns(tl + TM_S, max(z_lo, min(z_hi, w_hi)), z_hi);
          }
          tmem_st_wait();
          pf.mark(PW_E2_ST);
          w.arrive_tmem_only(B_P_READY);
          pf.mark(PW_E2);
          }
        }
      }

      mbar_wait(&bars[B_X1_FULL], (n_x1++) & 1);
      tc_fence_after();
      pf.mark(PW_WAIT_X1);
      w.stats_from_tmem(mean, rstd);
      w.normalize_from_tmem(mean, rstd, 1, V_BFF2);
      pf.mark(PW_LN2);

#pragma unroll 1
      for (int c = 0; c < a.n_chunks; ++c) {
        const int b = c & 1;
        if (b == 0) mbar_wait(&bars[B_HACC_FULL], (n_hacc0++) & 1);
        else mbar_wait(&bars[B_HACC_FULL1], (n_hacc1++) & 1);
        tc_fence_after();
        pf.mark(PW_WAIT_HACC);
        constexpr int HW = 128 / NSPLIT;
        const uint32_t hbase = tl + (b ? TM_H1 : TM_H0) + g * HW;
#pragma unroll
        for (int c0 = 0; c0 < HW; c0 += 32) {
          const float* bias = vec + V_BFF1 + c * 128 + g * HW + c0;
          uint32_t r[32], yk[16];
          tmem_ld32(hbase + c0, r);
          tmem_ld_wait();
#pragma unroll
          for (int j = 0; j < 32; j += 4) {
            const float4 b4 = *reinterpret_cast<const float4*>(bias + j);
#if AVF_FUSED_PACKED
            yk[j / 2] = gelu_bf16x2(cvt_bf16x2_pair(f2_add(f2_pack(__uint_as_float(r[j]), __uint_as_float(r[j + 1])), f2_pack(b4.x, b4.y))));
            yk[j / 2 + 1] = gelu_bf16x2(cvt_bf16x2_pair(f2_add(f2_pack(__uint_as_float(r[j + 2]), __uint_as_float(r[j + 3])), f2_pack(b4.z, b4.w))));
#else
            yk[j / 2] = pack_bf16x2(gelu_fast(__uint_as_float(r[j]) + b4.x), gelu_fast(__uint_as_float(r[j + 1]) + b4.y));
            yk[j / 2 + 1] = pack_bf16x2(gelu_fast(__uint_as_float(r[j + 2]) + b4.z), gelu_fast(__uint_as_float(r[j + 3]) + b4.w));
#endif
          }
          tmem_st16(hbase + c0 / 2, yk);
        }
        tmem_st_wait();
        w.arrive_tmem_only(B_H_READY + b);
        pf.mark(PW_GELU);
      }

      mbar_wait(&bars[B_X2_FULL], (n_x2++) & 1);
      tc_fence_after();
      pf.mark(PW_WAIT_X2);
      if (l + 1 < a.depth) w.stats_from_tmem(mean, rstd);
    }

    {
      __nv_bfloat16* dst16 = reinterpret_cast<__nv_bfloat16*>(smem + OFF_OUTST) + size_t(seq_in_tile * DIM + g * CW) * n_tok + t_in_seq;
      float* dst32 = static_cast<float*>(a.out) + grow * a.ld_out + g * CW;
#pragma unroll 1
      for (int c0 = 0; c0 < CW; c0 += 32) {
        float x[32];
        tmem_ld32(tl + TM_X + g * CW + c0, reinterpret_cast<uint32_t(&)[32]>(x));
        tmem_ld_wait();
        if (valid) {
          if constexpr (IO == IO_NCHW_BF16) {
#pragma unroll
            for (int j = 0; j < 32; ++j) dst16[(c0 + j) * n_tok] = __float2bfloat16_rn(x[j]);
          } else {
#pragma unroll
            for (int j = 0; j < 32; j += 4) *reinterpret_cast<float4*>(dst32 + c0 + j) = make_float4(x[j], x[j + 1], x[j + 2], x[j + 3]);
          }
        }
      }
      if constexpr (IO == IO_NCHW_BF16) {
        fence_proxy_async_smem();
        bar_sync(5, NUM_WORKERS);
        if (threadIdx.x == WORKER_T0) {
          __nv_bfloat16* gdst = static_cast<__nv_bfloat16*>(a.out) + size_t(tile) * spt * n_tok * DIM;
          bulk_store_1d(gdst, smem + OFF_OUTST, uint32_t(seqs_here) * n_tok * DIM * 2);
        }
      }
    }
    pf.mark(PW_OUTPUT);
    pf.count(PW_TILES);
  }
  pf.flush(0, 32);
  if constexpr (IO == IO_NCHW_BF16) {
    if (threadIdx.x == WORKER_T0) bulk_wait_all0();
  }
}

template <int IO>
__device__ void producer_main(const FusedArgs& a, uint8_t* smem, uint64_t* bars) {
  uint32_t it = 0;
  int load_tile = blockIdx.x;
  uint32_t n_free = 0;
  bool need_free = false;
  auto poll_loader = [&]() {
    if (IO != IO_NCHW_BF16 || load_tile < 0) return;
    if (need_free) {
#if AVF_PROD_POLL >= 1
      if (!mbar_test_wait(&bars[B_A0_FREE], n_free & 1)) return;
#else
      if (!mbar_try_wait(&bars[B_A0_FREE], n_free & 1)) return;
#endif
      ++n_free;
    }
    const int seqs_here = min(a.spt, a.n_seq - load_tile * a.spt);
    const uint32_t bytes = uint32_t(seqs_here) * a.n_tok * DIM * 2;
    mbar_expect_tx(&bars[B_X0_FULL], bytes);
    bulk_load_1d(smem + OFF_A0, static_cast<const __nv_bfloat16*>(a.in) + size_t(load_tile) * a.spt * a.n_tok * DIM, bytes, &bars[B_X0_FULL]);
    load_tile = -1;
    need_free = true;
  };
  uint32_t pbits = 0, n_gate = 0;
  auto poll_wait = [&](uint64_t* bar, uint32_t parity) {
#if AVF_PROD_FASTPATH
    if (mbar_try_wait(bar, parity)) return;
#endif
    poll_loader();
    const long long t0 = clock64();
#if AVF_PROD_POLL == 1
    while (!mbar_test_wait(bar, parity)) {
#else
    while (!mbar_try_wait(bar, parity)) {
#endif
      poll_loader();
      if (clock64() - t0 > 4000000000LL) {
        unsigned* tb = g_trap_buffer;
        if (tb != nullptr) {
          tb[0] = blockIdx.x; tb[1] = threadIdx.x; tb[2] = (smem_u32(bar) & 1023u) >> 3; tb[3] = parity;
          __threadfence_system();
        }
        printf("avf: fused encoder producer timed out (block %d item %u)\n", blockIdx.x, it);
        __trap();
      }
    }
  };
  uint32_t gidx = 0;
  auto load = [&](uint32_t s, const CUtensorMap* tm, int c0, int c1, uint64_t* full_bar, uint32_t expect_bytes) {
    poll_wait(&bars[B_RING_EMPTY + s], ((pbits >> s) & 1u) ^ 1u);
    pbits ^= 1u << s;
    if (expect_bytes != 0) mbar_expect_tx(full_bar, expect_bytes);
    tma_load_2d(smem + slot_offset(s), tm, full_bar, c0, c1);
    ++it;
  };
  uint32_t kpub = 0;
  auto publish = [&](int t) {
    tile_queue(bars)[kpub & 3u] = t;
    mbar_arrive(&bars[B_TQ_FULL + (kpub & 3u)]);
    ++kpub;
  };
  int cur = blockIdx.x;
  publish(cur);
  for (;;) {
    int nxt;
    if (a.tile_counter != nullptr) nxt = atomicAdd(a.tile_counter, 1) + int(gridDim.x);
    else nxt = cur + int(gridDim.x);
    if (nxt >= a.n_tiles) nxt = -1;
    publish(nxt);
    if (IO == IO_NCHW_BF16) {
      while (load_tile >= 0) poll_loader();
      load_tile = nxt;
    }
    for (int l = 0; l < a.depth; ++l) {
      const LayerArgs& L = a.layer[l];
      for (int h = 0; h < HEADS; ++h) {
        const uint32_t s = RING_LO + h % (RING_HI - RING_LO);
        load(s, &L.tm_out, h * DH, 0, &bars[B_RING_FULL + s], SLOT_BYTES);
      }
      poll_wait(&bars[B_QKV_FREE], (n_gate++) & 1);
      uint32_t m = 0;
      auto ff1 = [&](int c) {
        for (int kp = 0; kp < 4; ++kp) {
          if (kp % MLPG == 0) ++gidx;
          load((m++) % RING, &L.tm_w1, kpanel(kp) * 64, c * 128, &bars[B_G_FULL + ((gidx - 1) & 7u)], kp % MLPG == 0 ? MLPG * SLOT_BYTES : 0);
        }
      };
      auto ff2 = [&](int c) {
        for (int i = 0; i < 4; ++i) {
          const int kp = i >> 1, nh = i & 1;
          if (i % MLPG == 0) ++gidx;
          load((m++) % RING, &L.tm_w2, c * 128 + kp * 64, nh * 128, &bars[B_G_FULL + ((gidx - 1) & 7u)], i % MLPG == 0 ? MLPG * SLOT_BYTES : 0);
        }
      };
      ff1(0);
      if (a.n_chunks > 1) ff1(1);
      for (int c = 0; c < a.n_chunks; ++c) {
        ff2(c);
        if (c + 2 < a.n_chunks) ff1(c + 2);
      }
    }
    if (nxt < 0) break;
    cur = nxt;
  }
}

template <int IO>
__device__ void qkv_producer_main(const FusedArgs& a, uint8_t* smem, uint64_t* bars) {
  uint32_t qit = 0, hq = 0, n_free = 0, n_read = 0;
  bool first = true;
  for (uint32_t tk = 0; next_tile(bars, tk) >= 0; ++tk) {
    if constexpr (IO == IO_NCHW_BF16) mbar_wait(&bars[B_OUT_READ], (n_read++) & 1);
    for (int l = 0; l < a.depth; ++l) {
      const LayerArgs& L = a.layer[l];
      if (!first) mbar_wait(&bars[B_A1_FREE], (n_free++) & 1);
      first = false;
      for (int h = 0; h < HEADS; ++h, ++hq) {
        uint64_t* fb = &bars[B_QG_FULL + (hq & 1u)];
        for (int kp = 0; kp < 4; ++kp) {
          const uint32_t s = qit % QRING, ph = (qit / QRING) & 1;
          mbar_wait(&bars[B_QR_EMPTY + s], ph ^ 1);
          uint8_t* d = smem + OFF_QRING + s * QSLOT_BYTES;
          if (kp == 0) mbar_expect_tx(fb, 4 * QSLOT_BYTES);
          for (int s3 = 0; s3 < 3; ++s3) tma_load_2d(d + s3 * 4096, &L.tm_qkv, fb, kpanel(kp) * 64, s3 * (HEADS * DH) + h * DH);
          ++qit;
        }
      }
    }
  }
}

__device__ void mma_main(const FusedArgs& a, uint8_t* smem, uint64_t* bars, uint32_t tmem) {
  const bool leader = elect_one();
  const uint32_t a0 = smem_u32(smem + OFF_A0);
  const uint32_t qs = smem_u32(smem + OFF_Q), ks = smem_u32(smem + OFF_K), vs = smem_u32(smem + OFF_V);
  const uint32_t smem0 = smem_u32(smem), qring = smem_u32(smem + OFF_QRING), ost = smem_u32(smem + OFF_OST);
  const int kmax = 128;
  const uint32_t id_qkv = make_idesc_bf16(128, 96), id_s = make_idesc_bf16(128, kmax), id_pv = make_idesc_bf16(128, DH, 0, 1),
                 id_128 = make_idesc_bf16(128, 128), id_256 = make_idesc_bf16(128, 256);
  uint32_t obits = 0, m = 0, qit = 0, hq = 0, gidx = 0, n_a0 = 0, n_hready[2] = {0, 0};
  Prof pf;
  pf.start(blockIdx.x == 0 && leader);
  int ring_phase = PM_QKV;
  auto slot_wait = [&](uint32_t s) -> uint32_t {
    pf.mark(ring_phase);
    mbar_wait(&bars[B_RING_FULL + s], (obits >> s) & 1u);
    obits ^= 1u << s;
    tc_fence_after();
    pf.mark(PM_RW_OUT);
    return smem0 + uint32_t(slot_offset(s));
  };
  auto group_wait = [&]() {
    pf.mark(ring_phase);
    mbar_wait(&bars[B_G_FULL + (gidx & 7u)], (gidx >> 3) & 1u);
    ++gidx;
    tc_fence_after();
    pf.mark(ring_phase == PM_FF1 ? PM_RW_FF1 : PM_RW_FF2);
  };
  auto slot_release = [&](uint32_t s) {
    if (leader) umma_commit(&bars[B_RING_EMPTY + s]);
  };
  auto a0_wait = [&](int i, bool fresh) {
#if AVF_A0_HALF
    if (!fresh || (i != 0 && i != 2)) return;
    pf.mark(ring_phase);
    if (i == 0) mbar_wait(&bars[B_A0_HALF], n_a0 & 1);
    else mbar_wait(&bars[B_A0_READY], (n_a0++) & 1);
#else
    if (!fresh || i != 0) return;
    pf.mark(ring_phase);
    mbar_wait(&bars[B_A0_READY], (n_a0++) & 1);
#endif
    tc_fence_after();
    pf.mark(ring_phase == PM_QKV ? PM_WAIT_A0 : PM_WAIT_A0B);
  };
  auto qkv = [&](bool fresh) {
    pf.mark(ring_phase);
    mbar_wait(&bars[B_QG_FULL + (hq & 1u)], (hq >> 1) & 1u);
    ++hq;
    tc_fence_after();
    pf.mark(PM_RW_QKV);
    for (int i = 0; i < 4; ++i) {
      const int kp = kpanel(i);
      a0_wait(i, fresh);
      const uint32_t s = qit % QRING;
      const uint64_t da = make_desc_sw128_kmajor(a0 + kp * 16384), db = make_desc_sw128_kmajor(qring + s * QSLOT_BYTES);
#pragma unroll
      for (int k = 0; k < 4; ++k) if (leader) umma_bf16(tmem + TM_D1, da + uint64_t(k * 2), db + uint64_t(k * 2), id_qkv, (i | k) != 0 ? 1u : 0u);
      if (leader) umma_commit(&bars[B_QR_EMPTY + s]);
      ++qit;
    }
    if (leader) umma_commit(&bars[B_D1_FULL]);
  };
  auto outproj = [&](int h) {
    const uint32_t s = RING_LO + h % (RING_HI - RING_LO), sb = slot_wait(s);
    const uint64_t db = desc_sw64(sb);
#if AVF_O_TMEM
    if (leader) umma_bf16_ts(tmem + TM_X, tmem + TM_O, db, id_256, 1u);
    if (leader) umma_bf16_ts(tmem + TM_X, tmem + TM_O + 16, db + 2, id_256, 1u);
#else
    const uint64_t da = desc_sw64(ost);
    if (leader) umma_bf16(tmem + TM_X, da, db, id_256, 1u);
    if (leader) umma_bf16(tmem + TM_X, da + 2, db + 2, id_256, 1u);
#endif
    slot_release(s);
  };
  bool last_layer = false;
  auto ff1 = [&](int c, bool fresh) {
    const uint32_t d = tmem + ((c & 1) ? TM_H1 : TM_H0);
    for (int i = 0; i < 4; ++i) {
      const int kp = kpanel(i);
      if (i % MLPG == 0) group_wait();
      a0_wait(i, fresh);
      const uint32_t s = (m++) % RING, sb = smem0 + uint32_t(slot_offset(s));
      const uint64_t da = make_desc_sw128_kmajor(a0 + kp * 16384), db = make_desc_sw128_kmajor(sb);
#pragma unroll
      for (int k = 0; k < 4; ++k) if (leader) umma_bf16(d, da + uint64_t(k * 2), db + uint64_t(k * 2), id_128, (i | k) != 0 ? 1u : 0u);
      slot_release(s);
    }
    if (leader) umma_commit(&bars[B_HACC_FULL + (c & 1)]);
    if (c == a.n_chunks - 1 && last_layer) if (leader) umma_commit(&bars[B_A0_FREE]);
  };

  for (uint32_t tk = 0; next_tile(bars, tk) >= 0; ++tk) {
    for (int l = 0; l < a.depth; ++l) {
      last_layer = l == a.depth - 1;
      ring_phase = PM_QKV;
      qkv(true);
      pf.mark(PM_QKV);
      for (int h = 0; h < HEADS; ++h) {
        mbar_wait(&bars[B_STAGED], h & 1);
        tc_fence_after();
        pf.mark(PM_WAIT_STAGED);
        {
          const uint64_t da = desc_sw64(qs), db = desc_sw64(ks);
          if (leader) umma_bf16(tmem + TM_S, da, db, id_s, 0u);
          if (leader) umma_bf16(tmem + TM_S, da + 2, db + 2, id_s, 1u);
          if (leader) umma_commit(&bars[B_S_FULL]);
        }
        pf.mark(PM_S);
        if (h + 1 < HEADS) qkv(false);
        pf.mark(PM_QKV);
        if (h > 0) {
          mbar_wait(&bars[B_O_DRAINED], (h - 1) & 1);
          tc_fence_after();
          pf.mark(PM_WAIT_OD7);
          ring_phase = PM_OUT;
          outproj(h - 1);
          pf.mark(PM_OUT);
          ring_phase = PM_QKV;
        }
        mbar_wait(&bars[B_P_READY], h & 1);
        tc_fence_after();
        pf.mark(PM_WAIT_P);
        for (int k = 0; k < kmax / 16; ++k)
          if (leader) umma_bf16_ts(tmem + TM_O, tmem + TM_S + uint32_t(k * 8), desc_sw64(vs + (h & 1) * 8192 + k * 1024), id_pv, k != 0 ? 1u : 0u);
        if (leader) umma_commit(&bars[B_O_FULL]);
        pf.mark(PM_PV);
      }
      mbar_wait(&bars[B_O_DRAINED], (HEADS - 1) & 1);
      tc_fence_after();
      pf.mark(PM_WAIT_OD7);
      ring_phase = PM_OUT;
      outproj(HEADS - 1);
      if (leader) umma_commit(&bars[B_X1_FULL]);
      if (leader) umma_commit(&bars[B_QKV_FREE]);
      m = 0;
      pf.mark(PM_OUT);

      ring_phase = PM_FF1;
      ff1(0, true);
      if (a.n_chunks > 1) ff1(1, false);
      for (int c = 0; c < a.n_chunks; ++c) {
        const int b = c & 1;
        pf.mark(PM_FF1);
        mbar_wait(&bars[B_H_READY + b], (n_hready[b]++) & 1);
        tc_fence_after();
        pf.mark(PM_WAIT_H);
        ring_phase = PM_FF2;
        for (int kp = 0; kp < 2; ++kp)
          for (int nh = 0; nh < 2; ++nh) {
            if ((kp * 2 + nh) % MLPG == 0) group_wait();
            const uint32_t s = (m++) % RING, sb = smem0 + uint32_t(slot_offset(s));
            const uint32_t ta = tmem + (b ? TM_H1 : TM_H0) + uint32_t(kp * 64);
            const uint64_t db = make_desc_sw128_kmajor(sb);
#pragma unroll
            for (int k = 0; k < 4; ++k) if (leader) umma_bf16_ts(tmem + TM_X + nh * 128, ta + uint32_t(k * 8), db + uint64_t(k * 2), id_128, 1u);
            slot_release(s);
          }
        pf.mark(PM_FF2);
        ring_phase = PM_FF1;
        if (c + 2 < a.n_chunks) ff1(c + 2, false);
      }
      if (leader) umma_commit(&bars[B_X2_FULL]);
      if (leader) umma_commit(&bars[B_A1_FREE]);
    }
  }
  pf.flush(32, 64);
}

template <int IO, int NTOK>
__global__ void __launch_bounds__(NUM_THREADS, 1) encoder_fused_kernel(const __grid_constant__ FusedArgs a) {
  extern __shared__ __align__(1024) uint8_t smem_raw[];
  uint8_t* smem = smem_raw;
  if (threadIdx.x == 0 && (smem_u32(smem_raw) & 1023u) != 0u) {
    printf("avf: encoder_fused_kernel: dynamic shared memory base is not 1024-byte aligned enough\n");
    __trap();
  }
  uint64_t* bars = reinterpret_cast<uint64_t*>(smem + OFF_BAR);
  uint32_t* tmem_slot = reinterpret_cast<uint32_t*>(bars + NUM_BARS);
  const int warp = threadIdx.x >> 5, lane = threadIdx.x & 31;

  if (threadIdx.x == 0) {
    for (int l = 0; l < a.depth; ++l) {
      tma_prefetch_desc(&a.layer[l].tm_qkv);
      tma_prefetch_desc(&a.layer[l].tm_out);
      tma_prefetch_desc(&a.layer[l].tm_w1);
      tma_prefetch_desc(&a.layer[l].tm_w2);
    }
    for (int i = 0; i < NUM_BARS; ++i) {
      const bool by_workers = i == B_A0_READY || i == B_A0_HALF || i == B_STAGED || i == B_P_READY || i == B_O_DRAINED || i == B_H_READY || i == B_H_READY1;
      mbar_init(&bars[i], by_workers ? NUM_WORKERS / 32 : 1);
    }
    fence_barrier_init();
  }
  if (warp == 1) {
    tmem_alloc(tmem_slot, 512);
    tmem_relinquish();
  }
  tc_fence_before();
  __syncthreads();
  tc_fence_after();
  const uint32_t tmem = *tmem_slot;
  pdl_wait();
  pdl_trigger();

  if (warp == 0) {
    if (lane == 0) producer_main<IO>(a, smem, bars);
  } else if (warp == 1) {
    mma_main(a, smem, bars, tmem);
  } else if (warp == 2) {
    if (lane == 0) qkv_producer_main<IO>(a, smem, bars);
  } else {
    worker_main<IO, NTOK>(a, smem, bars, tmem);
  }

  tc_fence_before();
  __syncthreads();
  if (warp == 1) tmem_dealloc(tmem, 512);
}

__global__ void __launch_bounds__(256) pos_transpose_kernel(const float* __restrict__ pos, float* __restrict__ pos_t, int n_tok, int* tile_counter) {
  pdl_wait();
  pdl_trigger();
  if (blockIdx.x == 0 && threadIdx.x == 0 && tile_counter != nullptr) *tile_counter = 0;
  const int c = blockIdx.x * 4 + (threadIdx.x & 3), t = threadIdx.x >> 2;
  pos_t[(blockIdx.x * POS_LD + t) * 4 + (threadIdx.x & 3)] = t < n_tok ? pos[t * DIM + c] : 0.f;
}

bool dynamic_tiles_enabled() {
  static int v = -1;
  if (v < 0) {
    const char* e = getenv("AVF_FUSED_DYNAMIC_TILES");
    v = (e != nullptr && e[0] == '0') ? 0 : 1;
  }
  return v != 0;
}

bool fixed_ntok_enabled() {
  static int v = -1;
  if (v < 0) {
    const char* e = getenv("AVF_FUSED_FIXED_NTOK");
    v = (e != nullptr && e[0] == '0') ? 0 : 1;
  }
  return v != 0;
}

int sm_count_cached() { return sm_count_of_current_device(); }

}

int fused_set_trap_buffer(void* host_mapped_words) {
  unsigned* p = static_cast<unsigned*>(host_mapped_words);
  AVF_CUDA(cudaMemcpyToSymbol(g_trap_buffer, &p, sizeof(p)));
  return 0;
}

int fused_prof_read(unsigned long long* out64, int reset) {
#ifdef AVF_FUSED_PROF
  AVF_CUDA(cudaDeviceSynchronize());
  AVF_CUDA(cudaMemcpyFromSymbol(out64, g_prof, sizeof(unsigned long long) * 64));
  if (reset) {
    static unsigned long long zeros[64] = {0};
    AVF_CUDA(cudaMemcpyToSymbol(g_prof, zeros, sizeof(zeros)));
  }
  return 0;
#else
  (void)out64; (void)reset;
  return AVF_EUNSUPPORTED;
#endif
}

bool encoder_fused_supported(const avf_stack_shape* s) {
  return s->dim == DIM && s->heads == HEADS && s->dim_head == DH && s->mlp_dim % 128 == 0 && s->mlp_dim >= 128 && s->mlp_dim <= MAX_MLP && s->n_tok >= 1 &&
         s->n_tok <= 64 && s->depth >= 1 && s->depth <= MAX_DEPTH;
}

size_t encoder_fused_scratch_bytes() { return size_t(DIM) * POS_LD * sizeof(float) + 64; }

int encoder_fused(int io_kind, const avf_stack_shape* s, const avf_layer_weights* L, const void* in, int ld_in, void* out, int ld_out,
                  const float* pos, void* scratch, cudaStream_t st) {
  AVF_REQUIRE(encoder_fused_supported(s), AVF_EUNSUPPORTED, "fused encoder: unsupported shape dim=%d heads=%d dh=%d mlp=%d n_tok=%d depth=%d",
              s->dim, s->heads, s->dim_head, s->mlp_dim, s->n_tok, s->depth);
  AVF_REQUIRE(io_kind == IO_ROWS_F32 || (pos != nullptr && scratch != nullptr), AVF_EINVAL,
              "fused encoder: NCHW input needs the positional embedding and the scratch buffer");
  AVF_REQUIRE(io_kind == IO_NCHW_BF16 || (ld_in % 4 == 0 && ld_out % 4 == 0), AVF_EINVAL, "fused encoder: row strides must be multiples of 4");
  static thread_local FusedArgs a;
  static_assert(sizeof(FusedArgs) <= 4000, "kernel parameter space");
  a.in = in; a.out = out; a.pos = pos; a.pos_t = static_cast<const float*>(scratch); a.ld_in = ld_in; a.ld_out = ld_out;
  a.tile_counter = nullptr;
  if (io_kind == IO_NCHW_BF16) {
    if (dynamic_tiles_enabled()) a.tile_counter = reinterpret_cast<int*>(static_cast<uint8_t*>(scratch) + size_t(DIM) * POS_LD * sizeof(float));
    launch_pdl(pos_transpose_kernel, DIM / 4, 256, 0, st, pos, static_cast<float*>(scratch), s->n_tok, a.tile_counter);
    AVF_LAUNCH_CHECK("pos_transpose_kernel");
  }
  a.n_seq = s->n_seq; a.n_tok = s->n_tok;
  a.slot = 16; a.slot_log2 = 4;
  while (a.slot < s->n_tok) { a.slot *= 2; ++a.slot_log2; }
  a.spt = 128 / a.slot;
  a.n_tiles = ceil_div(s->n_seq, a.spt);
  a.n_chunks = s->mlp_dim / 128; a.depth = s->depth;
  const int inner = HEADS * DH;
  for (int l = 0; l < s->depth; ++l) {
    LayerArgs& A = a.layer[l];
    int e;
    if ((e = make_tmap_bf16_2d(&A.tm_qkv, L[l].w_qkv, 3 * inner, DIM, DIM, 32))) return e;
    if ((e = make_tmap_bf16_2d(&A.tm_out, L[l].w_out, DIM, inner, inner, 256, DH))) return e;
    if ((e = make_tmap_bf16_2d(&A.tm_w1, L[l].w_ff1, s->mlp_dim, DIM, DIM, 128))) return e;
    if ((e = make_tmap_bf16_2d(&A.tm_w2, L[l].w_ff2, DIM, s->mlp_dim, s->mlp_dim, 128))) return e;
    A.ln1_g = L[l].ln1_gamma; A.ln1_b = L[l].ln1_beta; A.b_out = L[l].b_out;
    A.ln2_g = L[l].ln2_gamma; A.ln2_b = L[l].ln2_beta; A.b_ff1 = L[l].b_ff1; A.b_ff2 = L[l].b_ff2;
  }
  static PerDeviceOnce once;
  if (once.first()) {
    AVF_CUDA(cudaFuncSetAttribute(encoder_fused_kernel<IO_NCHW_BF16, 49>, cudaFuncAttributeMaxDynamicSharedMemorySize, SMEM_ALLOC));
    AVF_CUDA(cudaFuncSetAttribute(encoder_fused_kernel<IO_NCHW_BF16, 0>, cudaFuncAttributeMaxDynamicSharedMemorySize, SMEM_ALLOC));
    AVF_CUDA(cudaFuncSetAttribute(encoder_fused_kernel<IO_ROWS_F32, 0>, cudaFuncAttributeMaxDynamicSharedMemorySize, SMEM_ALLOC));
  }
  const int cap = sm_cap();
  const int grid = min(a.n_tiles, cap > 0 ? min(cap, sm_count_cached()) : sm_count_cached());
  if (io_kind == IO_NCHW_BF16 && a.n_tok == 49 && NSPLIT == 2 && fixed_ntok_enabled())
    launch_pdl(encoder_fused_kernel<IO_NCHW_BF16, 49>, grid, NUM_THREADS, SMEM_ALLOC, st, a);
  else if (io_kind == IO_NCHW_BF16)
    launch_pdl(encoder_fused_kernel<IO_NCHW_BF16, 0>, grid, NUM_THREADS, SMEM_ALLOC, st, a);
  else
    launch_pdl(encoder_fused_kernel<IO_ROWS_F32, 0>, grid, NUM_THREADS, SMEM_ALLOC, st, a);
  AVF_LAUNCH_CHECK("encoder_fused_kernel");
  return 0;
}

}
```

multi-modal-multi-label-facial-action-unit-detection-with-transformer_b200/encoder.py:

```python
from __future__ import annotations

from typing import Optional

import torch
from torch import nn

from . import functional as AF

_DEFAULT_PRECISION = "bf16"


def set_default_precision(precision: str) -> None:
    global _DEFAULT_PRECISION
    AF._mode(precision)
    _DEFAULT_PRECISION = precision


def default_precision() -> str:
    return _DEFAULT_PRECISION


def _rank_salt() -> int:
    import torch.distributed as dist
    if not (dist.is_available() and dist.is_initialized()):
        return 0
    h = (dist.get_rank() * 0x9E3779B97F4A7C15) & 0xFFFFFFFFFFFFFFFF
    h ^= h >> 31
    h = (h * 0xBF58476D1CE4E5B9) & 0xFFFFFFFFFFFFFFFF
    h ^= h >> 29
    return h & ((1 << 62) - 1)


def needs_grad(module: nn.Module, *inputs: torch.Tensor) -> bool:
    if not torch.is_grad_enabled():
        return False
    return any(t is not None and t.requires_grad for t in inputs) or any(p.requires_grad for p in module.parameters())


class GELU(nn.Module):

    def forward(self, x):
        raise RuntimeError("GELU is fused into FeedForward's first linear; call FeedForward or Transformer")


class Residual(nn.Module):
    def __init__(self, fn):
        super().__init__()
        self.fn = fn

    def forward(self, x, **kw):
        return self.fn(x, **kw) + x


class PreNorm(nn.Module):
    def __init__(self, dim, fn):
        super().__init__()
        self.norm = nn.LayerNorm(dim)
        self.fn = fn

    def forward(self, x, **kw):
        prec = default_precision()
        y = AF.layernorm_fwd(x, self.norm.weight, self.norm.bias, prec)
        return self.fn(y.view(x.shape), **kw)


class FeedForward(nn.Module):
    def __init__(self, dim, hidden_dim, dropout=0.0):
        super().__init__()
        self.net = nn.Sequential(nn.Linear(dim, hidden_dim), GELU(), nn.Dropout(dropout), nn.Linear(hidden_dim, dim), nn.Dropout(dropout))

    def forward(self, x):
        prec = default_precision()
        cast = AF.to_bf16 if prec == "bf16" else (lambda t: t.detach().float())
        a = x.reshape(-1, x.shape[-1])
        a = a if a.dtype == (torch.bfloat16 if prec == "bf16" else torch.float32) else cast(a)
        h = AF.linear_fwd(a, cast(self.net[0].weight), self.net[0].bias, gelu=True, out_dtype=a.dtype, precision=prec)
        y = AF.linear_fwd(h, cast(self.net[3].weight), self.net[3].bias, out_dtype=torch.float32, precision=prec)
        return y.view(*x.shape[:-1], -1)


class Attention(nn.Module):
    def __init__(self, dim, heads=8, dim_head=64, dropout=0.0):
        super().__init__()
        inner = dim_head * heads
        self.heads, self.dim_head = heads, dim_head
        self.scale = dim_head ** -0.5
        self.to_qkv = nn.Linear(dim, inner * 3, bias=False)
        project_out = not (heads == 1 and dim_head == dim)
        self.to_out = nn.Sequential(nn.Linear(inner, dim), nn.Dropout(dropout)) if project_out else nn.Identity()

    def forward(self, x, mask=None):
        if mask is not None:
            raise NotImplementedError("attention masks are never passed on the AVFormer path (models/heads.py:225-232 is dead code)")
        prec = default_precision()
        cast = AF.to_bf16 if prec == "bf16" else (lambda t: t.detach().float())
        b, n, _ = x.shape
        a = x.reshape(b * n, -1)
        a = a if a.dtype == (torch.bfloat16 if prec == "bf16" else torch.float32) else cast(a)
        qkv = AF.linear_fwd(a, cast(self.to_qkv.weight), out_dtype=a.dtype, precision=prec)
        o = AF.attention_fwd(qkv, b, n, self.heads, self.dim_head)
        if isinstance(self.to_out, nn.Identity):
            return AF.to_f32(o).view(b, n, -1) if o.dtype != torch.float32 else o.view(b, n, -1)
        y = AF.linear_fwd(o, cast(self.to_out[0].weight), self.to_out[0].bias, out_dtype=torch.float32, precision=prec)
        return y.view(b, n, -1)


class Transformer(nn.Module):

    def __init__(self, dim, depth, heads, dim_head, mlp_dim, dropout=0.0):
        super().__init__()
        self.dim, self.depth, self.heads, self.dim_head, self.mlp_dim, self.dropout = dim, depth, heads, dim_head, mlp_dim, dropout
        self.layers = nn.ModuleList([
            nn.ModuleList([Residual(PreNorm(dim, Attention(dim, heads=heads, dim_head=dim_head, dropout=dropout))),
                           Residual(PreNorm(dim, FeedForward(dim, mlp_dim, dropout=dropout)))])
            for _ in range(depth)])
        self.precision: Optional[str] = None
        self.fixed_dropout_seed: Optional[int] = None
        self.dropout_salt: Optional[torch.Tensor] = None
        self._packed: Optional[AF.PackedStack] = None

    def _layer_tensors(self):
        for attn, ff in self.layers:
            a, f = attn.fn, ff.fn
            yield dict(ln1_gamma=a.norm.weight, ln1_beta=a.norm.bias, w_qkv=a.fn.to_qkv.weight,
                       w_out=a.fn.to_out[0].weight, b_out=a.fn.to_out[0].bias,
                       ln2_gamma=f.norm.weight, ln2_beta=f.norm.bias,
                       w_ff1=f.fn.net[0].weight, b_ff1=f.fn.net[0].bias, w_ff2=f.fn.net[3].weight, b_ff2=f.fn.net[3].bias)

    def packed(self) -> AF.PackedStack:
        mode = AF._mode(self.precision or default_precision())
        p = self._packed
        if p is None or p.mode != mode or p.stale():
            p = self._packed = AF.PackedStack(list(self._layer_tensors()), mode)
        return p

    def shape(self, n_seq: int, n_tok: int):
        return AF.make_shape(n_seq, n_tok, self.dim, self.heads, self.dim_head, self.mlp_dim, self.depth)

    def param_list(self):
        names = [n for n, _ in AF.LayerWeights._fields_]
        return [lw[n] for lw in self._layer_tensors() for n in names]

    def dropout_state(self):
        if not self.training or self.dropout <= 0.0:
            return 0.0, 0, None
        seed = self.fixed_dropout_seed
        if seed is None:
            seed = int(torch.randint(0, 2 ** 62, (1,)).item())
            seed ^= _rank_salt()
        return float(self.dropout), seed, self.dropout_salt

    def forward_(self, x2d: torch.Tensor, n_seq: int, n_tok: int, out: Optional[torch.Tensor] = None, ld_out: int = 0) -> torch.Tensor:
        p, seed, salt = self.dropout_state()
        if p > 0.0:
            y, _ = AF.encoder_stack_fwd_train(x2d, self.packed(), self.shape(n_seq, n_tok), p, seed, salt)
            if out is None:
                x2d.copy_(y)
                return x2d
            torch.as_strided(out, (y.shape[0], y.shape[1]), (ld_out, 1)).copy_(y)
            return out
        return AF.encoder_stack_fwd_(x2d, self.packed(), self.shape(n_seq, n_tok), out, ld_out)

    def forward_train(self, x2d: torch.Tensor, n_seq: int, n_tok: int) -> torch.Tensor:
        from .autograd import EncoderStackFn
        return EncoderStackFn.apply(x2d, self, n_seq, n_tok, *self.param_list())

    def forward(self, x: torch.Tensor, mask=None) -> torch.Tensor:
        if mask is not None:
            raise NotImplementedError("attention masks are never passed on the AVFormer path (models/heads.py:225-232 is dead code)")
        AF._cuda(x, "x")
        b, n, d = x.shape
        if needs_grad(self, x):
            return self.forward_train(x.reshape(b * n, d), b, n).view(b, n, d)
        y = x.detach().float().reshape(b * n, d).clone()
        return self.forward_(y, b, n).view(b, n, d)
```

multi-modal-multi-label-facial-action-unit-detection-with-transformer_b200/functional.py:

```python
from __future__ import annotations

import ctypes
from typing import Dict, List, Optional, Sequence, Tuple

import torch

from . import _lib
from ._lib import AVF_BF16, AVF_FP32, LayerWeights, StackShape, check

PRECISIONS = {"fp32": AVF_FP32, "bf16": AVF_BF16}


def _mode(precision) -> int:
    if isinstance(precision, int):
        return precision
    try:
        return PRECISIONS[precision]
    except KeyError:
        raise ValueError(f"precision must be 'bf16' or 'fp32', got {precision!r}") from None


def _io_mode(t: torch.Tensor) -> int:
    if t.dtype == torch.float32:
        return AVF_FP32
    if t.dtype == torch.bfloat16:
        return AVF_BF16
    raise TypeError(f"avformer_b200: unsupported activation dtype {t.dtype} (float32 or bfloat16)")


def _cuda(t: torch.Tensor, name: str) -> torch.Tensor:
    if not t.is_cuda:
        raise RuntimeError(f"avformer_b200: '{name}' is on {t.device}; the B200 path has no CPU fallback")
    if t.device.index != torch.cuda.current_device():
        raise RuntimeError(f"avformer_b200: '{name}' is on {t.device} but the current CUDA device is cuda:{torch.cuda.current_device()}; "
                           f"select the tensor's device first (torch.cuda.set_device / with torch.cuda.device(...))")
    return t


def _ptr(t: Optional[torch.Tensor]):
    return None if t is None else ctypes.c_void_p(t.data_ptr())


def _stream():
    return ctypes.c_void_p(torch.cuda.current_stream().cuda_stream)


def _f32c(t: torch.Tensor) -> torch.Tensor:
    t = t.detach()
    return t if (t.dtype == torch.float32 and t.is_contiguous()) else t.float().contiguous()


_workspaces: Dict[Tuple[int, int], torch.Tensor] = {}


def workspace(nbytes: int, device: torch.device) -> torch.Tensor:
    key = (device.index if device.index is not None else torch.cuda.current_device(), torch.cuda.current_stream().cuda_stream)
    buf = _workspaces.get(key)
    if buf is None or buf.numel() < nbytes:
        buf = torch.empty(max(nbytes, 1 << 20), dtype=torch.uint8, device=device)
        _workspaces[key] = buf
    return buf


def to_bf16(src: torch.Tensor) -> torch.Tensor:
    src = _f32c(_cuda(src, "src"))
    dst = torch.empty(src.shape, dtype=torch.bfloat16, device=src.device)
    check(_lib.lib().avf_cast_f32_to_bf16(_ptr(src), _ptr(dst), src.numel(), _stream()), "cast_f32_to_bf16")
    return dst


def to_f32(src: torch.Tensor) -> torch.Tensor:
    src = _cuda(src, "src").contiguous()
    dst = torch.empty(src.shape, dtype=torch.float32, device=src.device)
    check(_lib.lib().avf_cast_bf16_to_f32(_ptr(src), _ptr(dst), src.numel(), _stream()), "cast_bf16_to_f32")
    return dst


def fresh_bf16_image(param: torch.Tensor) -> Optional[torch.Tensor]:
    img = getattr(param, "_avf_bf16", None)
    if img is not None and img[1] == param._version and img[0].device == param.device:
        return img[0]
    return None


def _src_version(t: torch.Tensor) -> tuple:
    return (t.data_ptr(), t._version, getattr(t, "_avf_wver", 0))


class PackedStack:

    def __init__(self, layers: Sequence[Dict[str, torch.Tensor]], mode: int):
        self.mode = mode
        self.depth = len(layers)
        self.keep: List[torch.Tensor] = []
        self.sources: List[torch.Tensor] = []
        self.array = (LayerWeights * self.depth)()
        mats = ("w_qkv", "w_out", "w_ff1", "w_ff2")
        for i, lw in enumerate(layers):
            for name, _ in LayerWeights._fields_:
                src = lw[name]
                self.sources.append(src)
                t = _f32c(_cuda(src, name))
                if name in mats and mode == AVF_BF16:
                    t = fresh_bf16_image(src)
                    if t is None:
                        t = to_bf16(_f32c(src))
                self.keep.append(t)
                setattr(self.array[i], name, t.data_ptr())
        self.versions = [_src_version(s) for s in self.sources]
        self.epoch = WEIGHTS_EPOCH

    def stale(self) -> bool:
        return self.epoch != WEIGHTS_EPOCH or any(_src_version(s) != v for s, v in zip(self.sources, self.versions))


def make_shape(n_seq, n_tok, dim, heads, dim_head, mlp_dim, depth) -> StackShape:
    return StackShape(n_seq, n_tok, dim, heads, dim_head, mlp_dim, depth)


def encoder_stack_fwd_(x: torch.Tensor, packed: PackedStack, shape: StackShape, out: Optional[torch.Tensor] = None,
                       ld_out: int = 0) -> torch.Tensor:
    _cuda(x, "x")
    if x.dtype != torch.float32 or x.stride(-1) != 1:
        raise TypeError("encoder_stack_fwd_: x must be a float32 residual stream with unit column stride")
    L = _lib.lib()
    need = L.avf_encoder_workspace_bytes(ctypes.byref(shape), packed.mode)
    ws = workspace(need, x.device)
    check(L.avf_encoder_stack_fwd(packed.mode, ctypes.byref(shape), packed.array, _ptr(x), x.stride(0), _ptr(out), ld_out,
                                  _ptr(ws), ws.numel(), _stream()), "encoder_stack_fwd")
    return x if out is None else out


def layernorm_fwd(x: torch.Tensor, gamma: torch.Tensor, beta: torch.Tensor, precision="bf16") -> torch.Tensor:
    x = _f32c(_cuda(x, "x"))
    rows, dim = x.numel() // x.shape[-1], x.shape[-1]
    mode = _mode(precision)
    y = torch.empty(x.shape, dtype=torch.bfloat16 if mode == AVF_BF16 else torch.float32, device=x.device)
    check(_lib.lib().avf_layernorm_fwd(mode, _ptr(x), dim, _ptr(_f32c(gamma)), _ptr(_f32c(beta)), _ptr(y), rows, dim, _stream()), "layernorm_fwd")
    return y


def linear_fwd(a: torch.Tensor, w: torch.Tensor, bias: Optional[torch.Tensor] = None, residual: Optional[torch.Tensor] = None,
               gelu: bool = False, out_dtype: torch.dtype = torch.float32, precision="bf16") -> torch.Tensor:
    mode = _mode(precision)
    want = torch.bfloat16 if mode == AVF_BF16 else torch.float32
    _cuda(a, "a")
    if a.dtype != want or w.dtype != want:
        raise TypeError(f"linear_fwd({precision}): operands must be {want}, got {a.dtype} / {w.dtype}")
    a, w = a.contiguous(), w.contiguous()
    m, k = a.shape
    n = w.shape[0]
    c = torch.empty((m, n), dtype=out_dtype, device=a.device)
    flags = (1 if bias is not None else 0) | (2 if gelu else 0) | (4 if residual is not None else 0)
    if residual is not None:
        residual = _f32c(residual)
    if bias is not None:
        bias = _f32c(bias)
    check(_lib.lib().avf_linear_fwd(mode, _ptr(a), k, _ptr(w), _ptr(bias), _ptr(residual), n, _ptr(c), n, _io_mode(c), m, n, k, flags,
                                    _stream()), "linear_fwd")
    return c


def attention_fwd(qkv: torch.Tensor, n_seq: int, n_tok: int, heads: int, dim_head: int) -> torch.Tensor:
    qkv = _cuda(qkv, "qkv").contiguous()
    out = torch.empty((n_seq * n_tok, heads * dim_head), dtype=qkv.dtype, device=qkv.device)
    check(_lib.lib().avf_attention_fwd(_io_mode(qkv), _ptr(qkv), _ptr(out), n_seq, n_tok, heads, dim_head, _stream()), "attention_fwd")
    return out


def sformer_fwd(fmap: torch.Tensor, pos: torch.Tensor, packed: PackedStack, heads: int, dim_head: int, mlp_dim: int,
                out: Optional[torch.Tensor] = None) -> torch.Tensor:
    fmap = _cuda(fmap, "fmap").contiguous()
    F_, C, H, W = fmap.shape
    shape = make_shape(F_, H * W, C, heads, dim_head, mlp_dim, packed.depth)
    L = _lib.lib()
    need = L.avf_sformer_workspace_bytes(ctypes.byref(shape), packed.mode)
    ws = workspace(need, fmap.device)
    if out is None:
        out = torch.empty_like(fmap)
    elif out.shape != fmap.shape or out.dtype != fmap.dtype or not out.is_contiguous():
        raise ValueError("sformer_fwd: `out` must be a contiguous tensor with the shape and dtype of the input map")
    check(L.avf_sformer_fwd(packed.mode, _io_mode(fmap), ctypes.byref(shape), packed.array, _ptr(_f32c(pos)), _ptr(fmap), _ptr(out),
                            _ptr(ws), ws.numel(), _stream()), "sformer_fwd")
    return out


def tformer_embed(frames: torch.Tensor, cls_token: torch.Tensor, pos: torch.Tensor, n_frames: int) -> torch.Tensor:
    frames = _cuda(frames, "frames").contiguous()
    dim = frames.shape[-1]
    n_clips = frames.numel() // (n_frames * dim)
    x = torch.empty((n_clips * (n_frames + 1), dim), dtype=torch.float32, device=frames.device)
    check(_lib.lib().avf_tformer_embed(_io_mode(frames), _ptr(frames), _ptr(_f32c(cls_token)), _ptr(_f32c(pos)), _ptr(x), n_clips, n_frames,
                                       dim, _stream()), "tformer_embed")
    return x


def tformer_fwd(frames: torch.Tensor, cls_token: torch.Tensor, pos: torch.Tensor, packed: PackedStack, shape: StackShape) -> torch.Tensor:
    frames = _cuda(frames, "frames").contiguous()
    cls = torch.empty((shape.n_seq, shape.dim), dtype=torch.float32, device=frames.device)
    L = _lib.lib()
    ws = workspace(L.avf_tformer_workspace_bytes(ctypes.byref(shape), packed.mode), frames.device)
    check(L.avf_tformer_fwd(packed.mode, _io_mode(frames), ctypes.byref(shape), packed.array, _ptr(frames), _ptr(_f32c(cls_token)), _ptr(_f32c(pos)),
                            _ptr(cls), _ptr(ws), ws.numel(), _stream()), "tformer_fwd")
    return cls


def tformer_cls_extract(x: torch.Tensor, n_clips: int, n_tok: int) -> torch.Tensor:
    dim = x.shape[-1]
    cls = torch.empty((n_clips, dim), dtype=torch.float32, device=x.device)
    check(_lib.lib().avf_tformer_cls_extract(_ptr(x), _ptr(cls), n_clips, n_tok, dim, _stream()), "tformer_cls_extract")
    return cls


def au_former_front(emb: torch.Tensor, ld_emb: int, n_clips: int, bn: Sequence[torch.Tensor], w_cat: torch.Tensor, b_cat: torch.Tensor,
                    pos: torch.Tensor, mode: int) -> torch.Tensor:
    _cuda(emb, "emb")
    in_dim, emb_dim = w_cat.shape[1], w_cat.shape[0] // 12
    x = torch.empty((n_clips * 12, emb_dim), dtype=torch.float32, device=emb.device)
    ws = workspace(n_clips * in_dim * 4 + 256, emb.device)
    g, b, mu, var = (_f32c(t) for t in bn)
    check(_lib.lib().avf_au_former_front_fwd(mode, _ptr(emb), ld_emb, _ptr(g), _ptr(b), _ptr(mu), _ptr(var), _ptr(w_cat), _ptr(b_cat),
                                             _ptr(_f32c(pos)), _ptr(x), n_clips, in_dim, emb_dim, _ptr(ws), ws.numel(), _stream()),
          "au_former_front_fwd")
    return x


def token_front(emb: torch.Tensor, ld_emb: int, n_clips: int, n_tok: int, bn: Sequence[torch.Tensor], w_cat: torch.Tensor, b_cat: torch.Tensor,
                pos: torch.Tensor, mode: int) -> torch.Tensor:
    _cuda(emb, "emb")
    in_dim, emb_dim = w_cat.shape[1], w_cat.shape[0] // n_tok
    x = torch.empty((n_clips * n_tok, emb_dim), dtype=torch.float32, device=emb.device)
    ws = workspace(n_clips * in_dim * 4 + 256, emb.device)
    g, b, mu, var = (_f32c(t) for t in bn)
    check(_lib.lib().avf_token_front_fwd(mode, _ptr(emb), ld_emb, _ptr(g), _ptr(b), _ptr(mu), _ptr(var), _ptr(w_cat), _ptr(b_cat),
                                         _ptr(_f32c(pos)), _ptr(x), n_clips, in_dim, emb_dim, n_tok, _ptr(ws), ws.numel(), _stream()),
          "token_front_fwd")
    return x


def au_logits(x: torch.Tensor, w_last: torch.Tensor, n_clips: int, want_decisions: bool = False):
    _cuda(x, "x")
    out = torch.empty((n_clips, 21), dtype=torch.float32, device=x.device)
    dec = torch.empty((n_clips, 12), dtype=torch.int32, device=x.device) if want_decisions else None
    check(_lib.lib().avf_au_logits_fwd(_ptr(x), x.stride(0), _ptr(w_last), _ptr(out), _ptr(dec), n_clips, x.shape[-1], _stream()), "au_logits_fwd")
    return (out, dec) if want_decisions else out


def au_bce_loss(y_pred: torch.Tensor, y_true: torch.Tensor, pos_weight: torch.Tensor, want_grad: bool = False):
    _cuda(y_pred, "y_pred")
    if y_pred.dtype != torch.float32 or y_pred.stride(-1) != 1:
        y_pred = y_pred.float().contiguous()
    y_true = _f32c(_cuda(y_true, "y_true"))
    n = y_pred.shape[0]
    res = torch.empty(2, dtype=torch.float32, device=y_pred.device)
    grad = torch.empty((n, 12), dtype=torch.float32, device=y_pred.device) if want_grad else None
    check(_lib.lib().avf_au_bce_loss(_ptr(y_pred), y_pred.stride(0), _ptr(y_true), _ptr(_f32c(pos_weight)), _ptr(res), _ptr(grad), n, _stream()),
          "au_bce_loss")
    return res[0], res[1], grad


def add_row_periodic_(x: torch.Tensor, pos: torch.Tensor, period: int) -> torch.Tensor:
    check(_lib.lib().avf_add_row_periodic(_ptr(x), x.stride(0), _ptr(_f32c(pos)), x.shape[0], x.shape[1], period, _stream()), "add_row_periodic")
    return x


def device_info() -> Dict[str, int]:
    a, b, c = _lib._i32(), _lib._i32(), _lib._i32()
    check(_lib.lib().avf_device_info(ctypes.byref(a), ctypes.byref(b), ctypes.byref(c)), "device_info")
    return {"sm_count": a.value, "cc": b.value, "has_tcgen05": c.value}


def set_fused_enabled(enabled: bool) -> bool:
    return bool(_lib.lib().avf_set_fused_enabled(1 if enabled else 0))


def encoder_fused_supported(shape: StackShape, precision="bf16") -> bool:
    return bool(_lib.lib().avf_encoder_fused_supported(ctypes.byref(shape), _mode(precision)))


WEIGHTS_EPOCH = 0


def bump_weights_epoch() -> None:
    global WEIGHTS_EPOCH
    WEIGHTS_EPOCH += 1


def _act_dtype(mode: int) -> torch.dtype:
    return torch.bfloat16 if mode == AVF_BF16 else torch.float32


def gemm(a: torch.Tensor, b: torch.Tensor, trans_a: bool = False, trans_b: bool = False, m: Optional[int] = None, n: Optional[int] = None,
         k: Optional[int] = None, bias=None, residual=None, aux=None, flags: int = 0, out_dtype=torch.float32, precision="bf16") -> torch.Tensor:
    mode = _mode(precision)
    _cuda(a, "a")
    a, b = a.contiguous(), b.contiguous()
    m = m if m is not None else (a.shape[1] if trans_a else a.shape[0])
    k = k if k is not None else (a.shape[0] if trans_a else a.shape[1])
    n = n if n is not None else (b.shape[1] if trans_b else b.shape[0])
    c = torch.empty((m, n), dtype=out_dtype, device=a.device)
    L = _lib.lib()
    need = L.avf_gemm_workspace_bytes(mode, int(trans_a), int(trans_b), m, n, k)
    ws = workspace(max(need, 256), a.device)
    check(L.avf_gemm(mode, int(trans_a), int(trans_b), _ptr(a), a.stride(0), _ptr(b), b.stride(0), _ptr(bias), _ptr(residual),
                     residual.stride(0) if residual is not None else 0, _ptr(aux), aux.stride(0) if aux is not None else 0, _ptr(c), n,
                     _io_mode(c), m, n, k, flags, _ptr(ws), ws.numel(), _stream()), "gemm")
    return c


def colsum(x: torch.Tensor) -> torch.Tensor:
    _cuda(x, "x")
    rows, cols = x.shape
    out = torch.empty(cols, dtype=torch.float32, device=x.device)
    L = _lib.lib()
    ws = workspace(L.avf_colsum_workspace_bytes(rows, cols), x.device)
    check(L.avf_colsum(_io_mode(x), _ptr(x), x.stride(0), rows, cols, _ptr(out), _ptr(ws), ws.numel(), _stream()), "colsum")
    return out


def layernorm_bwd_(x: torch.Tensor, gamma: torch.Tensor, dy_norm: torch.Tensor, dres: torch.Tensor, want_bf16: bool = False):
    rows, dim = dres.shape
    dev = dres.device
    dg, db, dbias = (torch.empty(dim, dtype=torch.float32, device=dev) for _ in range(3))
    xb = torch.empty((rows, dim), dtype=torch.bfloat16, device=dev) if want_bf16 else None
    L = _lib.lib()
    ws = workspace(L.avf_layernorm_bwd_workspace_bytes(rows, dim), dev)
    check(L.avf_layernorm_bwd(_ptr(x), x.stride(0), _ptr(_f32c(gamma)), _ptr(dy_norm), _ptr(dres), dres.stride(0), _ptr(xb), _ptr(dg), _ptr(db),
                              _ptr(dbias), rows, dim, _ptr(ws), ws.numel(), _stream()), "layernorm_bwd")
    return dres, xb, dg, db, dbias


def attention_bwd(qkv: torch.Tensor, dout: torch.Tensor, n_seq: int, n_tok: int, heads: int, dim_head: int) -> torch.Tensor:
    qkv, dout = _cuda(qkv, "qkv").contiguous(), dout.contiguous()
    dqkv = torch.empty_like(qkv)
    check(_lib.lib().avf_attention_bwd(_io_mode(qkv), _ptr(qkv), _ptr(dout), _ptr(dqkv), n_seq, n_tok, heads, dim_head, _stream()), "attention_bwd")
    return dqkv


def encoder_stack_fwd_train(x: torch.Tensor, packed: PackedStack, shape: StackShape, dropout_p: float = 0.0, dropout_seed: int = 0,
                            dropout_salt: Optional[torch.Tensor] = None):
    _cuda(x, "x")
    if x.dtype != torch.float32 or x.stride(-1) != 1:
        raise TypeError("encoder_stack_fwd_train: x must be a float32 residual stream with unit column stride")
    L = _lib.lib()
    tape = torch.empty(L.avf_encoder_tape_bytes(ctypes.byref(shape), packed.mode), dtype=torch.uint8, device=x.device)
    y = torch.empty((x.shape[0], shape.dim), dtype=torch.float32, device=x.device)
    check(L.avf_encoder_stack_fwd_train(packed.mode, ctypes.byref(shape), packed.array, _ptr(x), x.stride(0), _ptr(y), shape.dim, _ptr(tape),
                                        tape.numel(), float(dropout_p), int(dropout_seed), _ptr(dropout_salt), _stream()), "encoder_stack_fwd_train")
    return y, tape


def encoder_stack_bwd_(dx: torch.Tensor, packed: PackedStack, shape: StackShape, tape: torch.Tensor, want: Sequence[bool],
                       dropout_p: float = 0.0, dropout_seed: int = 0, dropout_salt: Optional[torch.Tensor] = None,
                       into: Optional[Sequence[Optional[torch.Tensor]]] = None):
    from ._lib import LayerGrads
    names = [n for n, _ in LayerWeights._fields_]
    n_par = packed.depth * len(names)
    direct = into is not None and all((not want[i]) or (into[i] is not None and into[i].dtype == torch.float32 and into[i].is_contiguous()
                                                         and into[i].is_cuda) for i in range(n_par))
    grads: List[Optional[torch.Tensor]] = []
    arr = (LayerGrads * packed.depth)()
    for l in range(packed.depth):
        for j, name in enumerate(names):
            i = l * len(names) + j
            g = None
            if want[i]:
                g = into[i] if direct else torch.empty(packed.sources[i].shape, dtype=torch.float32, device=dx.device)
            grads.append(None if direct else g)
            setattr(arr[l], name, g.data_ptr() if g is not None else None)
    L = _lib.lib()
    ws = workspace(L.avf_encoder_bwd_workspace_bytes(ctypes.byref(shape), packed.mode), dx.device)
    check(L.avf_encoder_stack_bwd(packed.mode, ctypes.byref(shape), packed.array, _ptr(tape), tape.numel(), _ptr(dx), dx.stride(0), arr,
                                  1 if direct else 0, _ptr(ws), ws.numel(), float(dropout_p), int(dropout_seed), _ptr(dropout_salt), _stream()),
          "encoder_stack_bwd")
    return dx, grads


def sformer_tokens_pack(fmap: torch.Tensor, pos: Optional[torch.Tensor]) -> torch.Tensor:
    fmap = _cuda(fmap, "fmap").contiguous()
    F_, C, H, W = fmap.shape
    x = torch.empty((F_ * H * W, C), dtype=torch.float32, device=fmap.device)
    check(_lib.lib().avf_sformer_tokens_pack(_io_mode(fmap), _ptr(fmap), _ptr(_f32c(pos)) if pos is not None else None, _ptr(x), F_, C, H * W,
                                             _stream()), "sformer_tokens_pack")
    return x


def sformer_tokens_unpack(x: torch.Tensor, shape4, dtype: torch.dtype) -> torch.Tensor:
    F_, C, H, W = shape4
    fmap = torch.empty((F_, C, H, W), dtype=dtype, device=x.device)
    check(_lib.lib().avf_sformer_tokens_unpack(_io_mode(fmap), _ptr(x), _ptr(fmap), F_, C, H * W, _stream()), "sformer_tokens_unpack")
    return fmap


def au_former_front_train(emb: torch.Tensor, n_clips: int, bn_w, bn_b, run_mean, run_var, batch_stats: bool, momentum: float,
                          w_cat: torch.Tensor, b_cat: torch.Tensor, pos: torch.Tensor, mode: int):
    _cuda(emb, "emb")
    in_dim, emb_dim = w_cat.shape[1], w_cat.shape[0] // 12
    L = _lib.lib()
    tape = torch.empty(L.avf_au_former_front_tape_bytes(mode, n_clips, in_dim), dtype=torch.uint8, device=emb.device)
    x = torch.empty((n_clips * 12, emb_dim), dtype=torch.float32, device=emb.device)
    check(L.avf_au_former_front_fwd_train(mode, _ptr(emb), emb.stride(0), _ptr(_f32c(bn_w)), _ptr(_f32c(bn_b)), _ptr(run_mean), _ptr(run_var),
                                          int(batch_stats), float(momentum), _ptr(w_cat), _ptr(b_cat), _ptr(_f32c(pos)), _ptr(x), n_clips, in_dim,
                                          emb_dim, _ptr(tape), tape.numel(), _stream()), "au_former_front_fwd_train")
    return x, tape


def au_former_front_bwd(emb: torch.Tensor, n_clips: int, bn_w, run_mean, run_var, batch_stats: bool, w_cat: torch.Tensor, tape: torch.Tensor,
                        dx: torch.Tensor, mode: int, want_emb=True, want_bn=True, want_w=True):
    in_dim, emb_dim = w_cat.shape[1], w_cat.shape[0] // 12
    dev = dx.device
    dx = dx.contiguous()
    demb = torch.empty((n_clips, in_dim), dtype=torch.float32, device=dev) if want_emb else None
    dg = torch.empty(in_dim, dtype=torch.float32, device=dev) if want_bn else None
    db = torch.empty(in_dim, dtype=torch.float32, device=dev) if want_bn else None
    dw = torch.empty((12 * emb_dim, in_dim), dtype=torch.float32, device=dev) if want_w else None
    dbc = torch.empty(12 * emb_dim, dtype=torch.float32, device=dev)
    L = _lib.lib()
    ws = workspace(L.avf_au_former_front_bwd_workspace_bytes(mode, n_clips, in_dim, emb_dim), dev)
    check(L.avf_au_former_front_bwd(mode, _ptr(emb), emb.stride(0), _ptr(_f32c(bn_w)), _ptr(run_mean), _ptr(run_var), int(batch_stats), _ptr(w_cat),
                                    _ptr(tape), tape.numel(), _ptr(dx), _ptr(demb), in_dim, _ptr(dg), _ptr(db), _ptr(dw), _ptr(dbc), n_clips, in_dim,
                                    emb_dim, _ptr(ws), ws.numel(), _stream()), "au_former_front_bwd")
    return demb, dg, db, dw, dbc


def au_logits_bwd(dlogits: torch.Tensor, x: torch.Tensor, w_last: torch.Tensor, n_clips: int, want_dx=True, want_dw=True):
    dim = w_last.shape[1]
    dx = torch.empty((n_clips * 12, dim), dtype=torch.float32, device=x.device) if want_dx else None
    dw = torch.empty((12, dim), dtype=torch.float32, device=x.device) if want_dw else None
    check(_lib.lib().avf_au_logits_bwd(_ptr(dlogits), dlogits.stride(0), _ptr(x), x.stride(0), _ptr(w_last), _ptr(dx), dim, _ptr(dw), n_clips, dim,
                                       _stream()), "au_logits_bwd")
    return dx, dw


def adam_step_(p: torch.Tensor, g: torch.Tensor, m: torch.Tensor, v: torch.Tensor, step: int, lr: float, beta1: float, beta2: float, eps: float,
               weight_decay: float, decoupled: bool = False, grad_scale: float = 1.0, shadow: Optional[torch.Tensor] = None) -> None:
    _cuda(p, "params")
    check(_lib.lib().avf_adam_step(_ptr(p), _ptr(g), _ptr(m), _ptr(v), _ptr(shadow), p.numel(), lr, beta1, beta2, eps, weight_decay, step,
                                   int(decoupled), grad_scale, _stream()), "adam_step")


def dropout_mask(dropout_p: float, dropout_seed: int, layer: int, site: int, rows: int, cols: int, device,
                 dropout_salt: Optional[torch.Tensor] = None) -> torch.Tensor:
    out = torch.empty((rows, cols), dtype=torch.float32, device=device)
    check(_lib.lib().avf_dropout_mask(float(dropout_p), int(dropout_seed), _ptr(dropout_salt), layer, site, rows, cols, _ptr(out), _stream()),
          "dropout_mask")
    return out
```

multi-modal-multi-label-facial-action-unit-detection-with-transformer_b200/heads.py:

```python
from __future__ import annotations

from typing import Optional

import torch
from torch import nn

from . import functional as AF
from .encoder import Transformer, default_precision, needs_grad


class _PackedFront:

    def __init__(self, linears, mode):
        self.mode = mode
        self.sources = [p for l in linears for p in (l.weight, l.bias)]
        w = torch.cat([l.weight.detach().float() for l in linears], dim=0).contiguous()
        self.w = AF.to_bf16(w) if mode == AF.AVF_BF16 else w
        self.b = torch.cat([l.bias.detach().float() for l in linears], dim=0).contiguous()
        self.versions = [AF._src_version(s) for s in self.sources]
        self.epoch = AF.WEIGHTS_EPOCH

    def stale(self):
        return self.epoch != AF.WEIGHTS_EPOCH or any(AF._src_version(s) != v for s, v in zip(self.sources, self.versions))


class _PackedLast:
    def __init__(self, linears):
        self.sources = [l.weight for l in linears]
        self.w = torch.cat([l.weight.detach().float() for l in linears], dim=0).contiguous()
        self.versions = [AF._src_version(s) for s in self.sources]
        self.epoch = AF.WEIGHTS_EPOCH

    def stale(self):
        return self.epoch != AF.WEIGHTS_EPOCH or any(AF._src_version(s) != v for s, v in zip(self.sources, self.versions))


class AU_former(nn.Module):

    def __init__(self, input_dim=512, emb_dim=128, dropout=0.0):
        super().__init__()
        self.emb_dim = input_dim
        self.token_dim = emb_dim
        self.AU_BN1 = nn.BatchNorm1d(input_dim)
        for i in range(1, 13):
            setattr(self, f"AU_linear_p{i}", nn.Linear(input_dim, emb_dim))
        self.pos_embedding = nn.Parameter(torch.randn(1, 12, emb_dim))
        self.corr_transformer = Transformer(emb_dim, depth=2, heads=8, mlp_dim=256, dim_head=32, dropout=dropout)
        for i in range(1, 13):
            setattr(self, f"AU_linear_last{i}", nn.Linear(emb_dim, 1, bias=False))
        self._front: Optional[_PackedFront] = None
        self._last: Optional[_PackedLast] = None

    def _packed_front(self):
        mode = AF._mode(self.corr_transformer.precision or default_precision())
        if self._front is None or self._front.mode != mode or self._front.stale():
            self._front = _PackedFront([getattr(self, f"AU_linear_p{i}") for i in range(1, 13)], mode)
        return self._front

    def _packed_last(self):
        if self._last is None or self._last.stale():
            self._last = _PackedLast([getattr(self, f"AU_linear_last{i}") for i in range(1, 13)])
        return self._last

    def tokens_into(self, emb: torch.Tensor, ld_emb: int, n_clips: int, out: Optional[torch.Tensor] = None, ld_out: int = 0):
        f = self._packed_front()
        bn = self.AU_BN1
        if bn.training:
            view = torch.as_strided(emb, (n_clips, f.w.shape[1]), (ld_emb, 1))
            x, _ = AF.au_former_front_train(view, n_clips, bn.weight, bn.bias, bn.running_mean, bn.running_var, True,
                                            0.1 if bn.momentum is None else bn.momentum, f.w, f.b, self.pos_embedding[0], f.mode)
            bn.num_batches_tracked += 1
        else:
            x = AF.au_former_front(emb, ld_emb, n_clips, (bn.weight, bn.bias, bn.running_mean, bn.running_var), f.w, f.b,
                                   self.pos_embedding[0], f.mode)
        return self.corr_transformer.forward_(x, n_clips, 12, out, ld_out)

    def front_params(self):
        return [p for i in range(1, 13) for p in (getattr(self, f"AU_linear_p{i}").weight, getattr(self, f"AU_linear_p{i}").bias)]

    def tokens_train(self, emb: torch.Tensor, n_clips: int) -> torch.Tensor:
        from .autograd import AUFrontFn
        x = AUFrontFn.apply(emb, self.AU_BN1.weight, self.AU_BN1.bias, self.pos_embedding, self, n_clips, *self.front_params())
        return self.corr_transformer.forward_train(x, n_clips, 12)

    def forward(self, emb):
        AF._cuda(emb, "emb")
        bs = emb.shape[0]
        if needs_grad(self, emb):
            tok = self.tokens_train(emb, bs)
            with torch.no_grad():
                au_out = AF.au_logits(tok.detach(), self._packed_last().w, bs)[:, :12]
            return au_out, tok.view(bs, 12, -1)
        emb = emb.detach().float().contiguous()
        tok = self.tokens_into(emb, emb.shape[1], bs)
        au_out = AF.au_logits(tok, self._packed_last().w, bs)[:, :12]
        return au_out, tok.view(bs, 12, -1)


class former_AU_head(nn.Module):

    def __init__(self, emb_dim=128, dropout=0.0):
        super().__init__()
        self.pos_embedding = nn.Parameter(torch.randn(1, 12, emb_dim))
        self.corr_transformer = Transformer(emb_dim, depth=3, heads=8, mlp_dim=256, dim_head=32, dropout=dropout)
        for i in range(1, 13):
            setattr(self, f"AU_linear_last{i}", nn.Linear(emb_dim, 1, bias=False))
        self._last: Optional[_PackedLast] = None

    def _packed_last(self):
        if self._last is None or self._last.stale():
            self._last = _PackedLast([getattr(self, f"AU_linear_last{i}") for i in range(1, 13)])
        return self._last

    def logits21_(self, tokens2d: torch.Tensor, n_clips: int, want_decisions: bool = False):
        AF.add_row_periodic_(tokens2d, self.pos_embedding[0], 12)
        self.corr_transformer.forward_(tokens2d, n_clips, 12)
        return AF.au_logits(tokens2d, self._packed_last().w, n_clips, want_decisions)

    def last_params(self):
        return [getattr(self, f"AU_linear_last{i}").weight for i in range(1, 13)]

    def logits21_train(self, tokens2d: torch.Tensor, n_clips: int) -> torch.Tensor:
        from .autograd import AddPosFn, AULogitsFn
        x = AddPosFn.apply(tokens2d, self.pos_embedding, 12)
        x = self.corr_transformer.forward_train(x, n_clips, 12)
        return AULogitsFn.apply(x, self, n_clips, *self.last_params())

    def forward(self, input):
        AF._cuda(input, "input")
        bs = input.shape[0]
        if needs_grad(self, input):
            return self.logits21_train(input.reshape(bs * 12, -1), bs)[:, :12]
        tok = input.detach().float().reshape(bs * 12, -1).clone()
        return self.logits21_(tok, bs)[:, :12]


tformer_AU_head = former_AU_head


class VA_former(nn.Module):

    def __init__(self, input_dim=512, emb_dim=128, dropout=0.0):
        super().__init__()
        self.emb_dim = input_dim
        self.VA_BN1 = nn.BatchNorm1d(input_dim)
        self.VA_linear_p1 = nn.Linear(input_dim, emb_dim)
        self.VA_linear_p2 = nn.Linear(input_dim, emb_dim)
        self.pos_embedding = nn.Parameter(torch.randn(1, 2, emb_dim))
        self.corr_transformer = Transformer(emb_dim, depth=2, heads=8, mlp_dim=128, dim_head=32, dropout=dropout)
        self.VA_linear_last1 = nn.Linear(emb_dim, 1, bias=False)
        self.VA_linear_last2 = nn.Linear(emb_dim, 1, bias=False)
        self._front: Optional[_PackedFront] = None

    def _packed_front(self):
        mode = AF._mode(self.corr_transformer.precision or default_precision())
        if self._front is None or self._front.mode != mode or self._front.stale():
            self._front = _PackedFront([self.VA_linear_p1, self.VA_linear_p2], mode)
        return self._front

    @torch.no_grad()
    def forward(self, emb):
        AF._cuda(emb, "emb")
        if self.training:
            raise RuntimeError("VA_former: only the inference kernels are instantiated for this variant; call .eval()")
        bs = emb.shape[0]
        emb = emb.detach().float().contiguous()
        f = self._packed_front()
        bn = self.VA_BN1
        x = AF.token_front(emb, emb.shape[1], bs, 2, (bn.weight, bn.bias, bn.running_mean, bn.running_var), f.w, f.b, self.pos_embedding[0], f.mode)
        tok = self.corr_transformer.forward_(x, bs, 2).view(bs, 2, -1)
        w = torch.stack([self.VA_linear_last1.weight[0], self.VA_linear_last2.weight[0]]).float()
        va_out = (tok * w.unsqueeze(0)).sum(-1)
        return va_out, tok
```

Before: 469,800.

## Extend fused tcgen05 encoder to D=128 stacks with fused pos-add and AU logits

Templates the persistent fused encoder-layer kernel on the model dimension so the small 128-dim token transformers (AU and VA heads) can use it instead of the multi-kernel path. The positional-embedding add and the final per-AU logit projection are folded into that kernel through a new token_stack entry point, which removes separate launches and round trips of the residual stream. This adds template complexity, changes QKV ring barrier parity bookkeeping, and gives an environment switch to turn the small-dim fused path off.

After: 485,500 (median of 6 runs). 1.03x the previous value.

```diff
diff --git a/include/avformer_b200.h b/include/avformer_b200.h
--- a/include/avformer_b200.h
+++ b/include/avformer_b200.h
@@ -48,6 +48,7 @@
 int         avf_device_info(int32_t* sm_count, int32_t* cc, int32_t* has_tcgen05);
 
 int         avf_set_fused_enabled(int enabled);
+int         avf_set_fused_small_enabled(int enabled);
 int         avf_encoder_fused_supported(const avf_stack_shape* s, int mode);
 int         avf_set_sm_cap(int cap);
 int         avf_set_pdl_enabled(int enabled);
@@ -61,6 +62,9 @@
 int avf_encoder_stack_fwd(int mode, const avf_stack_shape* s, const avf_layer_weights* layers,
                           float* x, int32_t ld_x, float* out, int32_t ld_out,
                           void* workspace, size_t workspace_bytes, void* stream);
+int avf_token_stack_fwd(int mode, const avf_stack_shape* s, const avf_layer_weights* layers, float* x, int32_t ld_x, const float* pos,
+                        float* out, int32_t ld_out, const float* w_last, float* out21, int32_t* decisions,
+                        void* workspace, size_t workspace_bytes, void* stream);
 
 int avf_layernorm_fwd(int out_mode, const float* x, int32_t ld_x, const float* gamma, const float* beta,
                       void* y, int32_t rows, int32_t dim, void* stream);
diff --git a/multi-modal-multi-label-facial-action-unit-detection-with-transformer_b200/_lib.py b/multi-modal-multi-label-facial-action-unit-detection-with-transformer_b200/_lib.py
--- a/multi-modal-multi-label-facial-action-unit-detection-with-transformer_b200/_lib.py
+++ b/multi-modal-multi-label-facial-action-unit-detection-with-transformer_b200/_lib.py
@@ -45,11 +45,14 @@
     "avf_launch_count": (ctypes.c_uint64, []),
     "avf_device_info": (ctypes.c_int, [ctypes.POINTER(_i32)] * 3),
     "avf_set_fused_enabled": (ctypes.c_int, [ctypes.c_int]),
+    "avf_set_fused_small_enabled": (ctypes.c_int, [ctypes.c_int]),
     "avf_encoder_fused_supported": (ctypes.c_int, [ctypes.POINTER(StackShape), ctypes.c_int]),
     "avf_debug_fused_prof": (ctypes.c_int, [ctypes.POINTER(ctypes.c_uint64), ctypes.c_int]),
     "avf_encoder_workspace_bytes": (_sz, [ctypes.POINTER(StackShape), ctypes.c_int]),
     "avf_encoder_stack_fwd": (ctypes.c_int, [ctypes.c_int, ctypes.POINTER(StackShape), ctypes.POINTER(LayerWeights), _c_p, _i32,
                                              _c_p, _i32, _c_p, _sz, _c_p]),
+    "avf_token_stack_fwd": (ctypes.c_int, [ctypes.c_int, ctypes.POINTER(StackShape), ctypes.POINTER(LayerWeights), _c_p, _i32, _c_p,
+                                           _c_p, _i32, _c_p, _c_p, _c_p, _c_p, _sz, _c_p]),
     "avf_layernorm_fwd": (ctypes.c_int, [ctypes.c_int, _c_p, _i32, _c_p, _c_p, _c_p, _i32, _i32, _c_p]),
     "avf_linear_fwd": (ctypes.c_int, [ctypes.c_int, _c_p, _i32, _c_p, _c_p, _c_p, _i32, _c_p, _i32, ctypes.c_int, _i32, _i32, _i32,
                                       ctypes.c_int, _c_p]),
@@ -166,6 +169,8 @@
                 fn.restype, fn.argtypes = res, args
             if os.environ.get("AVF_PDL", "") in ("0", "off"):
                 handle.avf_set_pdl_enabled(0)
+            if os.environ.get("AVF_FUSED_SMALL", "") in ("0", "off"):
+                handle.avf_set_fused_small_enabled(0)
             if handle.avf_abi_version() != 1:
                 raise RuntimeError("avformer_b200: ABI version mismatch")
             _lib = handle
diff --git a/multi-modal-multi-label-facial-action-unit-detection-with-transformer_b200/csrc/avf_api.cu b/multi-modal-multi-label-facial-action-unit-detection-with-transformer_b200/csrc/avf_api.cu
--- a/multi-modal-multi-label-facial-action-unit-detection-with-transformer_b200/csrc/avf_api.cu
+++ b/multi-modal-multi-label-facial-action-unit-detection-with-transformer_b200/csrc/avf_api.cu
@@ -15,6 +15,7 @@
 static std::atomic<int> g_sm_cap{0};
 int sm_cap() { return g_sm_cap.load(); }
 static std::atomic<int> g_fused{1};
+static std::atomic<int> g_fused_small{1};
 
 void count_launch() { g_launches.fetch_add(1, std::memory_order_relaxed); }
 
@@ -105,14 +106,19 @@
   return linear_f32(static_cast<const float*>(a), lda, static_cast<const float*>(w), bias, res, ld_res, c, ldc, c_mode, m, n, k, flags, st);
 }
 
+static bool fused_rows(int mode, const avf_stack_shape* s, int ld_x, const float* out, int ld_out) {
+  return mode == AVF_BF16 && g_fused.load() && tcgen05_ok() && encoder_fused_supported(s) && (s->dim == 256 || g_fused_small.load()) &&
+         ld_x % 4 == 0 && (out == nullptr || ld_out % 4 == 0);
+}
+
 static int encoder_stack(int mode, const avf_stack_shape* s, const avf_layer_weights* L, float* x, int ld_x, float* out, int ld_out,
                          void* ws, size_t ws_bytes, cudaStream_t st) {
   int e = check_shape(s);
   if (e) return e;
   AVF_REQUIRE(mode == AVF_BF16 || mode == AVF_FP32, AVF_EINVAL, "mode=%d", mode);
   AVF_REQUIRE(L != nullptr && x != nullptr && ws != nullptr, AVF_EINVAL, "null pointer argument");
-  if (mode == AVF_BF16 && g_fused.load() && tcgen05_ok() && encoder_fused_supported(s) && ld_x % 4 == 0 && (out == nullptr || ld_out % 4 == 0))
-    return encoder_fused(1, s, L, x, ld_x, out ? out : x, out ? ld_out : ld_x, nullptr, nullptr, st);
+  if (fused_rows(mode, s, ld_x, out, ld_out))
+    return encoder_fused(1, s, L, x, ld_x, out ? out : x, out ? ld_out : ld_x, nullptr, nullptr, nullptr, nullptr, nullptr, st);
   const EncoderWs w = carve_encoder_ws(s, mode, ws);
   AVF_REQUIRE(ws_bytes >= w.total, AVF_EWORKSPACE, "workspace too small: %zu < %zu bytes", ws_bytes, w.total);
   const int R = s->n_seq * s->n_tok, D = s->dim, I = s->heads * s->dim_head, M = s->mlp_dim;
@@ -149,12 +155,14 @@
   return old;
 }
 
+int avf_set_fused_small_enabled(int enabled) { return g_fused_small.exchange(enabled ? 1 : 0); }
+
 int avf_set_pdl_enabled(int enabled) { return g_pdl.exchange(enabled ? 1 : 0); }
 
 int avf_set_sm_cap(int cap) { return g_sm_cap.exchange(cap > 0 ? cap : 0); }
 
 int avf_encoder_fused_supported(const avf_stack_shape* s, int mode) {
-  return (s != nullptr && mode == AVF_BF16 && s->n_seq > 0 && encoder_fused_supported(s)) ? 1 : 0;
+  return (s != nullptr && mode == AVF_BF16 && s->n_seq > 0 && encoder_fused_supported(s) && (s->dim == 256 || g_fused_small.load())) ? 1 : 0;
 }
 
 int avf_debug_fused_prof(uint64_t* out64, int reset) { return fused_prof_read(reinterpret_cast<unsigned long long*>(out64), reset); }
@@ -195,6 +203,22 @@
   return encoder_stack(mode, s, layers, x, ld_x, out, ld_out, workspace, workspace_bytes, static_cast<cudaStream_t>(stream));
 }
 
+int avf_token_stack_fwd(int mode, const avf_stack_shape* s, const avf_layer_weights* layers, float* x, int32_t ld_x, const float* pos, float* out,
+                        int32_t ld_out, const float* w_last, float* out21, int32_t* decisions, void* workspace, size_t workspace_bytes, void* stream) {
+  int e = require_device();
+  if (e) return e;
+  if ((e = check_shape(s))) return e;
+  AVF_REQUIRE(layers && x && workspace, AVF_EINVAL, "token_stack: null pointer");
+  AVF_REQUIRE(w_last == nullptr || (s->n_tok == 12 && out21 != nullptr), AVF_EINVAL, "token_stack: AU logits need 12 tokens per clip and out21 (n_tok=%d)",
+              s->n_tok);
+  cudaStream_t st = static_cast<cudaStream_t>(stream);
+  if (g_fused_small.load() && fused_rows(mode, s, ld_x, out, ld_out))
+    return encoder_fused(1, s, layers, x, ld_x, (out || w_last) ? out : x, out ? ld_out : ld_x, pos, nullptr, w_last, out21, decisions, st);
+  if (pos != nullptr && (e = add_row_periodic(x, ld_x, pos, s->n_seq * s->n_tok, s->dim, s->n_tok, st))) return e;
+  if ((e = encoder_stack(mode, s, layers, x, ld_x, out, ld_out, workspace, workspace_bytes, st))) return e;
+  return w_last == nullptr ? 0 : au_logits(out ? out : x, out ? ld_out : ld_x, w_last, out21, decisions, s->n_seq, s->dim, st);
+}
+
 int avf_layernorm_fwd(int out_mode, const float* x, int32_t ld_x, const float* gamma, const float* beta, void* y, int32_t rows,
                       int32_t dim, void* stream) {
   int e = require_device();
@@ -248,8 +272,8 @@
   const size_t need = avf_sformer_workspace_bytes(s, mode);
   AVF_REQUIRE(workspace_bytes >= need, AVF_EWORKSPACE, "workspace too small: %zu < %zu bytes", workspace_bytes, need);
   cudaStream_t st = static_cast<cudaStream_t>(stream);
-  if (mode == AVF_BF16 && io_mode == AVF_BF16 && g_fused.load() && tcgen05_ok() && encoder_fused_supported(s))
-    return encoder_fused(0, s, layers, fmap_in, 0, fmap_out, 0, pos, workspace, st);
+  if (mode == AVF_BF16 && io_mode == AVF_BF16 && g_fused.load() && tcgen05_ok() && encoder_fused_supported(s) && s->dim == 256)
+    return encoder_fused(0, s, layers, fmap_in, 0, fmap_out, 0, pos, workspace, nullptr, nullptr, nullptr, st);
   float* x = static_cast<float*>(workspace);
   const size_t xbytes = align_up(size_t(s->n_seq) * s->n_tok * s->dim * 4);
   if ((e = sformer_pack(io_mode, fmap_in, pos, x, s->n_seq, s->dim, s->n_tok, st))) return e;
@@ -326,14 +350,14 @@
                         int32_t in_dim, int32_t emb_dim, int32_t n_tok, void* workspace, size_t workspace_bytes, void* stream) {
   int e = require_device();
   if (e) return e;
-  AVF_REQUIRE(emb && bn_gamma && bn_beta && bn_mean && bn_var && w_cat && b_cat && pos && x && workspace, AVF_EINVAL, "token_front: null pointer");
+  AVF_REQUIRE(emb && bn_gamma && bn_beta && bn_mean && bn_var && w_cat && b_cat && x && workspace, AVF_EINVAL, "token_front: null pointer");
   AVF_REQUIRE(n_clips > 0 && in_dim > 0 && emb_dim > 0 && n_tok > 0, AVF_EINVAL, "token_front: n_clips=%d n_tok=%d", n_clips, n_tok);
   const size_t need = align_up(size_t(n_clips) * in_dim * elt(mode));
   AVF_REQUIRE(workspace_bytes >= need, AVF_EWORKSPACE, "workspace too small: %zu < %zu bytes", workspace_bytes, need);
   cudaStream_t st = static_cast<cudaStream_t>(stream);
   if ((e = bn_rows(mode, emb, ld_emb, bn_gamma, bn_beta, bn_mean, bn_var, workspace, n_clips, in_dim, st))) return e;
   if ((e = linear(mode, workspace, in_dim, w_cat, b_cat, nullptr, 0, x, n_tok * emb_dim, AVF_FP32, n_clips, n_tok * emb_dim, in_dim, AVF_EPI_BIAS, st))) return e;
-  return add_row_periodic(x, emb_dim, pos, n_clips * n_tok, emb_dim, n_tok, st);
+  return pos == nullptr ? 0 : add_row_periodic(x, emb_dim, pos, n_clips * n_tok, emb_dim, n_tok, st);
 }
 
 int avf_au_former_front_fwd(int mode, const float* emb, int32_t ld_emb, const float* bn_gamma, const float* bn_beta, const float* bn_mean,
diff --git a/multi-modal-multi-label-facial-action-unit-detection-with-transformer_b200/csrc/avf_internal.h b/multi-modal-multi-label-facial-action-unit-detection-with-transformer_b200/csrc/avf_internal.h
--- a/multi-modal-multi-label-facial-action-unit-detection-with-transformer_b200/csrc/avf_internal.h
+++ b/multi-modal-multi-label-facial-action-unit-detection-with-transformer_b200/csrc/avf_internal.h
@@ -62,7 +62,7 @@
 int fused_set_trap_buffer(void* host_mapped_words);
 size_t encoder_fused_scratch_bytes();
 int encoder_fused(int io_kind, const avf_stack_shape* s, const avf_layer_weights* L, const void* in, int ld_in, void* out, int ld_out,
-                  const float* pos, void* scratch, cudaStream_t st);
+                  const float* pos, void* scratch, const float* w_last, float* out21, int* decisions, cudaStream_t st);
 
 int gemm_umma(int trans_a, int trans_b, const void* a, int lda, const void* w, int ldw, const float* bias, const float* res, int ld_res,
               const void* aux, int ld_aux, void* c, int ldc, int c_mode, int m, int n, int k, int flags, void* ws, size_t ws_bytes,
diff --git a/multi-modal-multi-label-facial-action-unit-detection-with-transformer_b200/csrc/avf_layer_fused.cu b/multi-modal-multi-label-facial-action-unit-detection-with-transformer_b200/csrc/avf_layer_fused.cu
--- a/multi-modal-multi-label-facial-action-unit-detection-with-transformer_b200/csrc/avf_layer_fused.cu
+++ b/multi-modal-multi-label-facial-action-unit-detection-with-transformer_b200/csrc/avf_layer_fused.cu
@@ -37,11 +37,17 @@
 #define AVF_QRING 6
 #endif
 constexpr int QRING = AVF_QRING, QSLOT_BYTES = 12288;
+template <int D> constexpr int KPH = D / 64;
+template <int D> constexpr int NQG = (QRING + KPH<D> - 1) / KPH<D>;
+constexpr int MAX_QG = NQG<128>;
+static_assert(KPH<256> * (NQG<256> - 1) < QRING && QRING <= KPH<256> * NQG<256>, "head-full barrier parity (D = 256)");
+static_assert(KPH<128> * (NQG<128> - 1) < QRING && QRING <= KPH<128> * NQG<128>, "head-full barrier parity (D = 128)");
 #ifndef AVF_MLP_GROUP
 #define AVF_MLP_GROUP 4
 #endif
 constexpr int MLPG = AVF_MLP_GROUP;
 static_assert(MLPG == 2 || MLPG == 4, "MLP group size");
+template <int D> constexpr int GSLOTS = MLPG < D / 64 ? MLPG : D / 64;
 
 constexpr int OFF_A0 = 0;
 constexpr int OFF_Q = 65536;
@@ -52,14 +58,14 @@
 constexpr int OFF_QRING = OFF_OST + (AVF_O_TMEM ? 0 : 8192);
 constexpr int OFF_OUTST = OFF_QRING;
 static_assert(QRING * QSLOT_BYTES >= 2 * 64 * 256 * 2, "the NCHW output staging lives in the QKV ring");
-static_assert(QRING >= 6 && QRING < 8, "one head-full barrier per head parity needs 6 or 7 sub-slots (see qkv_producer_main)");
+static_assert(QRING >= 6 && QRING < 8, "six or seven QKV sub-slots (one and a half heads in flight at D = 256; see NQG)");
 constexpr int QRING_END = OFF_QRING + QRING * QSLOT_BYTES;
 constexpr int OFF_XCH = QRING_END > OFF_Q + RING * SLOT_BYTES ? QRING_END : OFF_Q + RING * SLOT_BYTES;
 static_assert(OFF_XCH - OFF_Q >= RING * SLOT_BYTES, "the nine MLP ring slots fit in [OFF_Q, OFF_XCH)");
 static_assert(OFF_RING == OFF_Q + RING_LO * SLOT_BYTES, "ring slots are contiguous from OFF_Q");
 __host__ __device__ constexpr int slot_offset(uint32_t s) { return OFF_Q + int(s) * SLOT_BYTES; }
 constexpr int OFF_VEC = OFF_XCH + 2 * 128 * 4 * 4;
-constexpr int V_BOUT = 0, V_BFF2 = 256, V_BFF1 = 512;
+constexpr int V_BOUT = 0, V_BFF2 = DIM, V_BFF1 = 2 * DIM;
 constexpr int V_B16 = V_BFF1 + MAX_MLP;
 constexpr int OFF_BAR = OFF_VEC + (V_B16 + 512) * 4;
 constexpr int SMEM_USED = OFF_BAR + 512;
@@ -69,18 +75,16 @@
 #ifndef AVF_A0_HALF
 #define AVF_A0_HALF 1
 #endif
-#if AVF_A0_HALF
-__device__ __forceinline__ constexpr int kpanel(int i) { return ((i & 1) << 1) | (i >> 1); }
-#else
-__device__ __forceinline__ constexpr int kpanel(int i) { return i; }
-#endif
+template <int D> constexpr bool A0_HALF = AVF_A0_HALF && D == 256;
+template <int D>
+__device__ __forceinline__ constexpr int kpanel(int i) { return A0_HALF<D> ? (((i & 1) << 1) | (i >> 1)) : i; }
 
 constexpr uint32_t TM_X = 0, TM_D1 = 256, TM_O = 352, TM_S = 384, TM_H0 = 256, TM_H1 = 384;
 
 enum {
   B_RING_FULL = 0, B_RING_EMPTY = RING, B_X0_FULL = 2 * RING, B_A0_FREE, B_A0_READY, B_D1_FULL, B_STAGED, B_S_FULL, B_P_READY, B_O_FULL,
   B_O_DRAINED, B_X1_FULL, B_HACC_FULL, B_HACC_FULL1, B_H_READY, B_H_READY1, B_X2_FULL,
-  B_QG_FULL, B_QR_EMPTY = B_QG_FULL + 2, B_A1_FREE = B_QR_EMPTY + QRING, B_OUT_READ, B_QKV_FREE, B_G_FULL, B_TQ_FULL = B_G_FULL + 8, B_A0_HALF = B_TQ_FULL + 4, NUM_BARS
+  B_QG_FULL, B_QR_EMPTY = B_QG_FULL + MAX_QG, B_A1_FREE = B_QR_EMPTY + QRING, B_OUT_READ, B_QKV_FREE, B_G_FULL, B_TQ_FULL = B_G_FULL + 8, B_A0_HALF = B_TQ_FULL + 4, NUM_BARS
 };
 static_assert(NUM_BARS * 8 + 8 + 16 <= 512, "barrier block (+ TMEM slot + tile queue)");
 
@@ -109,6 +113,9 @@
   const void* in;
   void* out;
   const float* pos;
+  const float* w_last;
+  float* out21;
+  int* decisions;
   const float* pos_t;
   int ld_in, ld_out;
   int* tile_counter;
@@ -117,9 +124,10 @@
 
 __device__ unsigned* g_trap_buffer = nullptr;
 
-constexpr int CW = DIM / NSPLIT;
-
+template <int D>
 struct Worker {
+  static constexpr int CW = D / NSPLIT;
+
   uint8_t* smem;
   uint64_t* bars;
   const float* vec;
@@ -191,7 +199,7 @@
     mean = exchange_sum(mean_g) * (1.f / NSPLIT);
     const float dm = mean_g - mean;
     const float m2 = exchange_sum(fmaf(dm * dm, n, m2_g));
-    rstd = rsqrtf(m2 * (1.f / DIM) + 1e-5f);
+    rstd = rsqrtf(m2 * (1.f / D) + 1e-5f);
   }
   __device__ __forceinline__ void stats_from_tmem(float& mean, float& rstd) {
     Stats st{0.f, 0.f, 0.f};
@@ -218,8 +226,8 @@
       const int chunk0 = (col0 & 63) >> 3;
 #pragma unroll
       for (int ch = 0; ch < 4; ++ch) {
-        const __nv_bfloat16* v16 = reinterpret_cast<const __nv_bfloat16*>(vec + V_B16) + ln_sel * 512 + col0 + ch * 8;
-        const uint4 gm = *reinterpret_cast<const uint4*>(v16), bt = *reinterpret_cast<const uint4*>(v16 + 256);
+        const __nv_bfloat16* v16 = reinterpret_cast<const __nv_bfloat16*>(vec + V_B16) + ln_sel * (2 * DIM) + col0 + ch * 8;
+        const uint4 gm = *reinterpret_cast<const uint4*>(v16), bt = *reinterpret_cast<const uint4*>(v16 + DIM);
         uint4 pk;
         pk.x = fma_bf16x2(cvt_bf16x2_pair(f2_fma(f2_pack(x[ch * 8], x[ch * 8 + 1]), rstd2, nmr2)), gm.x, bt.x);
         pk.y = fma_bf16x2(cvt_bf16x2_pair(f2_fma(f2_pack(x[ch * 8 + 2], x[ch * 8 + 3]), rstd2, nmr2)), gm.y, bt.y);
@@ -234,17 +242,15 @@
         f2_unpack(f2_add(f2_pack(x[j + 2], x[j + 3]), b.y), x[j + 2], x[j + 3]);
       }
       tmem_st32(tl + TM_X + col0, reinterpret_cast<const uint32_t(&)[32]>(x));
-#if AVF_A0_HALF
-      if (c0 == 32) arrive(B_A0_HALF);
-#endif
+      if (A0_HALF<D> && c0 == 32) arrive(B_A0_HALF);
     }
     tmem_st_wait();
     arrive(B_A0_READY);
   }
 };
 
-template <int NC, int TAILV>
-__device__ __forceinline__ float softmax_fixed(Worker& w, uint32_t ts, uint32_t tp, float sm_scale, Prof& pf) {
+template <int NC, int TAILV, class W>
+__device__ __forceinline__ float softmax_fixed(W& w, uint32_t ts, uint32_t tp, float sm_scale, Prof& pf) {
   float s[NC][8];
 #pragma unroll
   for (int c = 0; c < NC; ++c) tmem_ld8(ts + c * 8, reinterpret_cast<uint32_t(&)[8]>(s[c]));
@@ -298,9 +304,11 @@
 __host__ __device__ constexpr int slot_of(int n_tok) { return n_tok <= 16 ? 16 : (n_tok <= 32 ? 32 : 64); }
 __host__ __device__ constexpr int log2_of(int v) { return v == 16 ? 4 : (v == 32 ? 5 : 6); }
 
-template <int IO, int NTOK>
+template <int IO, int NTOK, int D>
 __device__ void worker_main(const FusedArgs& a, uint8_t* smem, uint64_t* bars, uint32_t tmem) {
-  Worker w;
+  using W = Worker<D>;
+  constexpr int CW = W::CW;
+  W w;
   w.smem = smem;
   w.bars = bars;
   w.vec = reinterpret_cast<const float*>(smem + OFF_VEC);
@@ -340,12 +348,12 @@
 
     float mean, rstd;
     {
-      Worker::Stats st{0.f, 0.f, 0.f};
+      typename W::Stats st{0.f, 0.f, 0.f};
       const int t_safe = valid ? t_in_seq : 0, seq_safe = valid ? seq_in_tile : 0;
-      const float* pp = (IO == IO_ROWS_F32 && a.pos != nullptr) ? a.pos + t_safe * DIM + g * CW : nullptr;
+      const float* pp = (IO == IO_ROWS_F32 && a.pos != nullptr) ? a.pos + t_safe * D + g * CW : nullptr;
       const float4* ppt = reinterpret_cast<const float4*>(a.pos_t) + size_t(g * CW / 4) * POS_LD + t_safe;
       if constexpr (IO == IO_NCHW_BF16) mbar_wait(&bars[B_X0_FULL], (n_x0++) & 1);
-      const __nv_bfloat16* src16 = reinterpret_cast<const __nv_bfloat16*>(smem + OFF_A0) + size_t(seq_safe * DIM + g * CW) * n_tok + t_safe;
+      const __nv_bfloat16* src16 = reinterpret_cast<const __nv_bfloat16*>(smem + OFF_A0) + size_t(seq_safe * D + g * CW) * n_tok + t_safe;
       const float* src32 = static_cast<const float*>(a.in) + ((size_t(tile) * spt + seq_safe) * n_tok + t_safe) * a.ld_in + g * CW;
 #pragma unroll 1
       for (int c0 = 0; c0 < CW; c0 += 32) {
@@ -403,11 +411,11 @@
       if (a.depth > 1 || !vec_loaded) {
         if (vec_loaded) bar_sync(5, NUM_WORKERS);
         float* vs = reinterpret_cast<float*>(smem + OFF_VEC);
-        for (int i = wt; i < DIM; i += NUM_WORKERS) {
+        for (int i = wt; i < D; i += NUM_WORKERS) {
           vs[V_BOUT + i] = L.b_out[i]; vs[V_BFF2 + i] = L.b_ff2[i];
           __nv_bfloat16* v16 = reinterpret_cast<__nv_bfloat16*>(vs + V_B16);
-          v16[i] = __float2bfloat16_rn(L.ln1_g[i]); v16[256 + i] = __float2bfloat16_rn(L.ln1_b[i]);
-          v16[512 + i] = __float2bfloat16_rn(L.ln2_g[i]); v16[768 + i] = __float2bfloat16_rn(L.ln2_b[i]);
+          v16[i] = __float2bfloat16_rn(L.ln1_g[i]); v16[DIM + i] = __float2bfloat16_rn(L.ln1_b[i]);
+          v16[2 * DIM + i] = __float2bfloat16_rn(L.ln2_g[i]); v16[3 * DIM + i] = __float2bfloat16_rn(L.ln2_b[i]);
         }
         for (int i = wt; i < a.n_chunks * 128; i += NUM_WORKERS) vs[V_BFF1 + i] = L.b_ff1[i];
         bar_sync(5, NUM_WORKERS);
@@ -626,14 +634,18 @@
     }
 
     {
-      __nv_bfloat16* dst16 = reinterpret_cast<__nv_bfloat16*>(smem + OFF_OUTST) + size_t(seq_in_tile * DIM + g * CW) * n_tok + t_in_seq;
+      __nv_bfloat16* dst16 = reinterpret_cast<__nv_bfloat16*>(smem + OFF_OUTST) + size_t(seq_in_tile * D + g * CW) * n_tok + t_in_seq;
+      const bool store = valid && (IO == IO_NCHW_BF16 || a.out != nullptr);
       float* dst32 = static_cast<float*>(a.out) + grow * a.ld_out + g * CW;
+      const bool logits = IO == IO_ROWS_F32 && a.w_last != nullptr;
+      const float* wl = logits ? a.w_last + (valid ? t_in_seq : 0) * D + g * CW : nullptr;
+      float dot = 0.f;
 #pragma unroll 1
       for (int c0 = 0; c0 < CW; c0 += 32) {
         float x[32];
         tmem_ld32(tl + TM_X + g * CW + c0, reinterpret_cast<uint32_t(&)[32]>(x));
         tmem_ld_wait();
-        if (valid) {
+        if (store) {
           if constexpr (IO == IO_NCHW_BF16) {
 #pragma unroll
             for (int j = 0; j < 32; ++j) dst16[(c0 + j) * n_tok] = __float2bfloat16_rn(x[j]);
@@ -641,14 +653,34 @@
 #pragma unroll
             for (int j = 0; j < 32; j += 4) *reinterpret_cast<float4*>(dst32 + c0 + j) = make_float4(x[j], x[j + 1], x[j + 2], x[j + 3]);
           }
+        }
+        if constexpr (IO == IO_ROWS_F32) {
+          if (logits) {
+#pragma unroll
+            for (int j = 0; j < 32; j += 4) {
+              const float4 w4 = __ldg(reinterpret_cast<const float4*>(wl + c0 + j));
+              dot = fmaf(x[j], w4.x, fmaf(x[j + 1], w4.y, fmaf(x[j + 2], w4.z, fmaf(x[j + 3], w4.w, dot))));
+            }
+          }
+        }
+      }
+      if constexpr (IO == IO_ROWS_F32) {
+        if (logits) {
+          const float lg = w.exchange_sum(dot);
+          const size_t clip = grow / 12;
+          if (valid && g == 0) {
+            if (a.out21 != nullptr) a.out21[clip * 21 + t_in_seq] = lg;
+            if (a.decisions != nullptr) a.decisions[clip * 12 + t_in_seq] = lg > 0.f ? 1 : 0;
+          }
+          if (valid && g == 1 && t_in_seq < 9 && a.out21 != nullptr) a.out21[clip * 21 + 12 + t_in_seq] = 0.f;
         }
       }
       if constexpr (IO == IO_NCHW_BF16) {
         fence_proxy_async_smem();
         bar_sync(5, NUM_WORKERS);
         if (threadIdx.x == WORKER_T0) {
-          __nv_bfloat16* gdst = static_cast<__nv_bfloat16*>(a.out) + size_t(tile) * spt * n_tok * DIM;
-          bulk_store_1d(gdst, smem + OFF_OUTST, uint32_t(seqs_here) * n_tok * DIM * 2);
+          __nv_bfloat16* gdst = static_cast<__nv_bfloat16*>(a.out) + size_t(tile) * spt * n_tok * D;
+          bulk_store_1d(gdst, smem + OFF_OUTST, uint32_t(seqs_here) * n_tok * D * 2);
         }
       }
     }
@@ -661,7 +693,7 @@
   }
 }
 
-template <int IO>
+template <int IO, int D>
 __device__ void producer_main(const FusedArgs& a, uint8_t* smem, uint64_t* bars) {
   uint32_t it = 0;
   int load_tile = blockIdx.x;
@@ -678,9 +710,9 @@
       ++n_free;
     }
     const int seqs_here = min(a.spt, a.n_seq - load_tile * a.spt);
-    const uint32_t bytes = uint32_t(seqs_here) * a.n_tok * DIM * 2;
+    const uint32_t bytes = uint32_t(seqs_here) * a.n_tok * D * 2;
     mbar_expect_tx(&bars[B_X0_FULL], bytes);
-    bulk_load_1d(smem + OFF_A0, static_cast<const __nv_bfloat16*>(a.in) + size_t(load_tile) * a.spt * a.n_tok * DIM, bytes, &bars[B_X0_FULL]);
+    bulk_load_1d(smem + OFF_A0, static_cast<const __nv_bfloat16*>(a.in) + size_t(load_tile) * a.spt * a.n_tok * D, bytes, &bars[B_X0_FULL]);
     load_tile = -1;
     need_free = true;
   };
@@ -738,21 +770,22 @@
       const LayerArgs& L = a.layer[l];
       for (int h = 0; h < HEADS; ++h) {
         const uint32_t s = RING_LO + h % (RING_HI - RING_LO);
-        load(s, &L.tm_out, h * DH, 0, &bars[B_RING_FULL + s], SLOT_BYTES);
+        load(s, &L.tm_out, h * DH, 0, &bars[B_RING_FULL + s], D * DH * 2);
       }
       poll_wait(&bars[B_QKV_FREE], (n_gate++) & 1);
       uint32_t m = 0;
+      constexpr int G = GSLOTS<D>, NH = D / 128;
       auto ff1 = [&](int c) {
-        for (int kp = 0; kp < 4; ++kp) {
-          if (kp % MLPG == 0) ++gidx;
-          load((m++) % RING, &L.tm_w1, kpanel(kp) * 64, c * 128, &bars[B_G_FULL + ((gidx - 1) & 7u)], kp % MLPG == 0 ? MLPG * SLOT_BYTES : 0);
+        for (int kp = 0; kp < D / 64; ++kp) {
+          if (kp % G == 0) ++gidx;
+          load((m++) % RING, &L.tm_w1, kpanel<D>(kp) * 64, c * 128, &bars[B_G_FULL + ((gidx - 1) & 7u)], kp % G == 0 ? G * SLOT_BYTES : 0);
         }
       };
       auto ff2 = [&](int c) {
-        for (int i = 0; i < 4; ++i) {
-          const int kp = i >> 1, nh = i & 1;
-          if (i % MLPG == 0) ++gidx;
-          load((m++) % RING, &L.tm_w2, c * 128 + kp * 64, nh * 128, &bars[B_G_FULL + ((gidx - 1) & 7u)], i % MLPG == 0 ? MLPG * SLOT_BYTES : 0);
+        for (int i = 0; i < 2 * NH; ++i) {
+          const int kp = i / NH, nh = i % NH;
+          if (i % G == 0) ++gidx;
+          load((m++) % RING, &L.tm_w2, c * 128 + kp * 64, nh * 128, &bars[B_G_FULL + ((gidx - 1) & 7u)], i % G == 0 ? G * SLOT_BYTES : 0);
         }
       };
       ff1(0);
@@ -767,7 +800,7 @@
   }
 }
 
-template <int IO>
+template <int IO, int D>
 __device__ void qkv_producer_main(const FusedArgs& a, uint8_t* smem, uint64_t* bars) {
   uint32_t qit = 0, hq = 0, n_free = 0, n_read = 0;
   bool first = true;
@@ -778,13 +811,13 @@
       if (!first) mbar_wait(&bars[B_A1_FREE], (n_free++) & 1);
       first = false;
       for (int h = 0; h < HEADS; ++h, ++hq) {
-        uint64_t* fb = &bars[B_QG_FULL + (hq & 1u)];
-        for (int kp = 0; kp < 4; ++kp) {
+        uint64_t* fb = &bars[B_QG_FULL + (hq % uint32_t(NQG<D>))];
+        for (int kp = 0; kp < KPH<D>; ++kp) {
           const uint32_t s = qit % QRING, ph = (qit / QRING) & 1;
           mbar_wait(&bars[B_QR_EMPTY + s], ph ^ 1);
           uint8_t* d = smem + OFF_QRING + s * QSLOT_BYTES;
-          if (kp == 0) mbar_expect_tx(fb, 4 * QSLOT_BYTES);
-          for (int s3 = 0; s3 < 3; ++s3) tma_load_2d(d + s3 * 4096, &L.tm_qkv, fb, kpanel(kp) * 64, s3 * (HEADS * DH) + h * DH);
+          if (kp == 0) mbar_expect_tx(fb, KPH<D> * QSLOT_BYTES);
+          for (int s3 = 0; s3 < 3; ++s3) tma_load_2d(d + s3 * 4096, &L.tm_qkv, fb, kpanel<D>(kp) * 64, s3 * (HEADS * DH) + h * DH);
           ++qit;
         }
       }
@@ -792,6 +825,7 @@
   }
 }
 
+template <int D>
 __device__ void mma_main(const FusedArgs& a, uint8_t* smem, uint64_t* bars, uint32_t tmem) {
   const bool leader = elect_one();
   const uint32_t a0 = smem_u32(smem + OFF_A0);
@@ -799,7 +833,7 @@
   const uint32_t smem0 = smem_u32(smem), qring = smem_u32(smem + OFF_QRING), ost = smem_u32(smem + OFF_OST);
   const int kmax = 128;
   const uint32_t id_qkv = make_idesc_bf16(128, 96), id_s = make_idesc_bf16(128, kmax), id_pv = make_idesc_bf16(128, DH, 0, 1),
-                 id_128 = make_idesc_bf16(128, 128), id_256 = make_idesc_bf16(128, 256);
+                 id_128 = make_idesc_bf16(128, 128), id_out = make_idesc_bf16(128, D);
   uint32_t obits = 0, m = 0, qit = 0, hq = 0, gidx = 0, n_a0 = 0, n_hready[2] = {0, 0};
   Prof pf;
   pf.start(blockIdx.x == 0 && leader);
@@ -823,27 +857,27 @@
     if (leader) umma_commit(&bars[B_RING_EMPTY + s]);
   };
   auto a0_wait = [&](int i, bool fresh) {
-#if AVF_A0_HALF
-    if (!fresh || (i != 0 && i != 2)) return;
-    pf.mark(ring_phase);
-    if (i == 0) mbar_wait(&bars[B_A0_HALF], n_a0 & 1);
-    else mbar_wait(&bars[B_A0_READY], (n_a0++) & 1);
-#else
-    if (!fresh || i != 0) return;
-    pf.mark(ring_phase);
-    mbar_wait(&bars[B_A0_READY], (n_a0++) & 1);
-#endif
+    if constexpr (A0_HALF<D>) {
+      if (!fresh || (i != 0 && i != 2)) return;
+      pf.mark(ring_phase);
+      if (i == 0) mbar_wait(&bars[B_A0_HALF], n_a0 & 1);
+      else mbar_wait(&bars[B_A0_READY], (n_a0++) & 1);
+    } else {
+      if (!fresh || i != 0) return;
+      pf.mark(ring_phase);
+      mbar_wait(&bars[B_A0_READY], (n_a0++) & 1);
+    }
     tc_fence_after();
     pf.mark(ring_phase == PM_QKV ? PM_WAIT_A0 : PM_WAIT_A0B);
   };
   auto qkv = [&](bool fresh) {
     pf.mark(ring_phase);
-    mbar_wait(&bars[B_QG_FULL + (hq & 1u)], (hq >> 1) & 1u);
+    mbar_wait(&bars[B_QG_FULL + (hq % uint32_t(NQG<D>))], (hq / uint32_t(NQG<D>)) & 1u);
     ++hq;
     tc_fence_after();
     pf.mark(PM_RW_QKV);
-    for (int i = 0; i < 4; ++i) {
-      const int kp = kpanel(i);
+    for (int i = 0; i < KPH<D>; ++i) {
+      const int kp = kpanel<D>(i);
       a0_wait(i, fresh);
       const uint32_t s = qit % QRING;
       const uint64_t da = make_desc_sw128_kmajor(a0 + kp * 16384), db = make_desc_sw128_kmajor(qring + s * QSLOT_BYTES);
@@ -858,21 +892,21 @@
     const uint32_t s = RING_LO + h % (RING_HI - RING_LO), sb = slot_wait(s);
     const uint64_t db = desc_sw64(sb);
 #if AVF_O_TMEM
-    if (leader) umma_bf16_ts(tmem + TM_X, tmem + TM_O, db, id_256, 1u);
-    if (leader) umma_bf16_ts(tmem + TM_X, tmem + TM_O + 16, db + 2, id_256, 1u);
+    if (leader) umma_bf16_ts(tmem + TM_X, tmem + TM_O, db, id_out, 1u);
+    if (leader) umma_bf16_ts(tmem + TM_X, tmem + TM_O + 16, db + 2, id_out, 1u);
 #else
     const uint64_t da = desc_sw64(ost);
-    if (leader) umma_bf16(tmem + TM_X, da, db, id_256, 1u);
-    if (leader) umma_bf16(tmem + TM_X, da + 2, db + 2, id_256, 1u);
+    if (leader) umma_bf16(tmem + TM_X, da, db, id_out, 1u);
+    if (leader) umma_bf16(tmem + TM_X, da + 2, db + 2, id_out, 1u);
 #endif
     slot_release(s);
   };
   bool last_layer = false;
   auto ff1 = [&](int c, bool fresh) {
     const uint32_t d = tmem + ((c & 1) ? TM_H1 : TM_H0);
-    for (int i = 0; i < 4; ++i) {
-      const int kp = kpanel(i);
-      if (i % MLPG == 0) group_wait();
+    for (int i = 0; i < D / 64; ++i) {
+      const int kp = kpanel<D>(i);
+      if (i % GSLOTS<D> == 0) group_wait();
       a0_wait(i, fresh);
       const uint32_t s = (m++) % RING, sb = smem0 + uint32_t(slot_offset(s));
       const uint64_t da = make_desc_sw128_kmajor(a0 + kp * 16384), db = make_desc_sw128_kmajor(sb);
@@ -941,8 +975,8 @@
         pf.mark(PM_WAIT_H);
         ring_phase = PM_FF2;
         for (int kp = 0; kp < 2; ++kp)
-          for (int nh = 0; nh < 2; ++nh) {
-            if ((kp * 2 + nh) % MLPG == 0) group_wait();
+          for (int nh = 0; nh < D / 128; ++nh) {
+            if ((kp * (D / 128) + nh) % GSLOTS<D> == 0) group_wait();
             const uint32_t s = (m++) % RING, sb = smem0 + uint32_t(slot_offset(s));
             const uint32_t ta = tmem + (b ? TM_H1 : TM_H0) + uint32_t(kp * 64);
             const uint64_t db = make_desc_sw128_kmajor(sb);
@@ -961,7 +995,7 @@
   pf.flush(32, 64);
 }
 
-template <int IO, int NTOK>
+template <int IO, int NTOK, int D>
 __global__ void __launch_bounds__(NUM_THREADS, 1) encoder_fused_kernel(const __grid_constant__ FusedArgs a) {
   extern __shared__ __align__(1024) uint8_t smem_raw[];
   uint8_t* smem = smem_raw;
@@ -998,13 +1032,13 @@
   pdl_trigger();
 
   if (warp == 0) {
-    if (lane == 0) producer_main<IO>(a, smem, bars);
+    if (lane == 0) producer_main<IO, D>(a, smem, bars);
   } else if (warp == 1) {
-    mma_main(a, smem, bars, tmem);
+    mma_main<D>(a, smem, bars, tmem);
   } else if (warp == 2) {
-    if (lane == 0) qkv_producer_main<IO>(a, smem, bars);
+    if (lane == 0) qkv_producer_main<IO, D>(a, smem, bars);
   } else {
-    worker_main<IO, NTOK>(a, smem, bars, tmem);
+    worker_main<IO, NTOK, D>(a, smem, bars, tmem);
   }
 
   tc_fence_before();
@@ -1064,22 +1098,26 @@
 }
 
 bool encoder_fused_supported(const avf_stack_shape* s) {
-  return s->dim == DIM && s->heads == HEADS && s->dim_head == DH && s->mlp_dim % 128 == 0 && s->mlp_dim >= 128 && s->mlp_dim <= MAX_MLP && s->n_tok >= 1 &&
+  return (s->dim == 256 || s->dim == 128) && s->heads == HEADS && s->dim_head == DH && s->mlp_dim % 128 == 0 && s->mlp_dim >= 128 && s->mlp_dim <= MAX_MLP && s->n_tok >= 1 &&
          s->n_tok <= 64 && s->depth >= 1 && s->depth <= MAX_DEPTH;
 }
 
 size_t encoder_fused_scratch_bytes() { return size_t(DIM) * POS_LD * sizeof(float) + 64; }
 
 int encoder_fused(int io_kind, const avf_stack_shape* s, const avf_layer_weights* L, const void* in, int ld_in, void* out, int ld_out,
-                  const float* pos, void* scratch, cudaStream_t st) {
+                  const float* pos, void* scratch, const float* w_last, float* out21, int* decisions, cudaStream_t st) {
   AVF_REQUIRE(encoder_fused_supported(s), AVF_EUNSUPPORTED, "fused encoder: unsupported shape dim=%d heads=%d dh=%d mlp=%d n_tok=%d depth=%d",
               s->dim, s->heads, s->dim_head, s->mlp_dim, s->n_tok, s->depth);
   AVF_REQUIRE(io_kind == IO_ROWS_F32 || (pos != nullptr && scratch != nullptr), AVF_EINVAL,
               "fused encoder: NCHW input needs the positional embedding and the scratch buffer");
-  AVF_REQUIRE(io_kind == IO_NCHW_BF16 || (ld_in % 4 == 0 && ld_out % 4 == 0), AVF_EINVAL, "fused encoder: row strides must be multiples of 4");
+  AVF_REQUIRE(io_kind == IO_ROWS_F32 || s->dim == DIM, AVF_EUNSUPPORTED, "fused encoder: the NCHW form is dim %d only", DIM);
+  AVF_REQUIRE(io_kind == IO_NCHW_BF16 || (ld_in % 4 == 0 && (out == nullptr || ld_out % 4 == 0)), AVF_EINVAL, "fused encoder: row strides must be multiples of 4");
+  AVF_REQUIRE(w_last == nullptr || (io_kind == IO_ROWS_F32 && s->n_tok == 12), AVF_EINVAL, "fused encoder: AU logits need 12-token rows");
+  AVF_REQUIRE(out != nullptr || w_last != nullptr, AVF_EINVAL, "fused encoder: no output");
   static thread_local FusedArgs a;
   static_assert(sizeof(FusedArgs) <= 4000, "kernel parameter space");
   a.in = in; a.out = out; a.pos = pos; a.pos_t = static_cast<const float*>(scratch); a.ld_in = ld_in; a.ld_out = ld_out;
+  a.w_last = w_last; a.out21 = out21; a.decisions = decisions;
   a.tile_counter = nullptr;
   if (io_kind == IO_NCHW_BF16) {
     if (dynamic_tiles_enabled()) a.tile_counter = reinterpret_cast<int*>(static_cast<uint8_t*>(scratch) + size_t(DIM) * POS_LD * sizeof(float));
@@ -1092,31 +1130,34 @@
   a.spt = 128 / a.slot;
   a.n_tiles = ceil_div(s->n_seq, a.spt);
   a.n_chunks = s->mlp_dim / 128; a.depth = s->depth;
-  const int inner = HEADS * DH;
+  const int inner = HEADS * DH, D = s->dim;
   for (int l = 0; l < s->depth; ++l) {
     LayerArgs& A = a.layer[l];
     int e;
-    if ((e = make_tmap_bf16_2d(&A.tm_qkv, L[l].w_qkv, 3 * inner, DIM, DIM, 32))) return e;
-    if ((e = make_tmap_bf16_2d(&A.tm_out, L[l].w_out, DIM, inner, inner, 256, DH))) return e;
-    if ((e = make_tmap_bf16_2d(&A.tm_w1, L[l].w_ff1, s->mlp_dim, DIM, DIM, 128))) return e;
-    if ((e = make_tmap_bf16_2d(&A.tm_w2, L[l].w_ff2, DIM, s->mlp_dim, s->mlp_dim, 128))) return e;
+    if ((e = make_tmap_bf16_2d(&A.tm_qkv, L[l].w_qkv, 3 * inner, D, D, 32))) return e;
+    if ((e = make_tmap_bf16_2d(&A.tm_out, L[l].w_out, D, inner, inner, D, DH))) return e;
+    if ((e = make_tmap_bf16_2d(&A.tm_w1, L[l].w_ff1, s->mlp_dim, D, D, 128))) return e;
+    if ((e = make_tmap_bf16_2d(&A.tm_w2, L[l].w_ff2, D, s->mlp_dim, s->mlp_dim, 128))) return e;
     A.ln1_g = L[l].ln1_gamma; A.ln1_b = L[l].ln1_beta; A.b_out = L[l].b_out;
     A.ln2_g = L[l].ln2_gamma; A.ln2_b = L[l].ln2_beta; A.b_ff1 = L[l].b_ff1; A.b_ff2 = L[l].b_ff2;
   }
   static PerDeviceOnce once;
   if (once.first()) {
-    AVF_CUDA(cudaFuncSetAttribute(encoder_fused_kernel<IO_NCHW_BF16, 49>, cudaFuncAttributeMaxDynamicSharedMemorySize, SMEM_ALLOC));
-    AVF_CUDA(cudaFuncSetAttribute(encoder_fused_kernel<IO_NCHW_BF16, 0>, cudaFuncAttributeMaxDynamicSharedMemorySize, SMEM_ALLOC));
-    AVF_CUDA(cudaFuncSetAttribute(encoder_fused_kernel<IO_ROWS_F32, 0>, cudaFuncAttributeMaxDynamicSharedMemorySize, SMEM_ALLOC));
+    AVF_CUDA(cudaFuncSetAttribute(encoder_fused_kernel<IO_NCHW_BF16, 49, 256>, cudaFuncAttributeMaxDynamicSharedMemorySize, SMEM_ALLOC));
+    AVF_CUDA(cudaFuncSetAttribute(encoder_fused_kernel<IO_NCHW_BF16, 0, 256>, cudaFuncAttributeMaxDynamicSharedMemorySize, SMEM_ALLOC));
+    AVF_CUDA(cudaFuncSetAttribute(encoder_fused_kernel<IO_ROWS_F32, 0, 256>, cudaFuncAttributeMaxDynamicSharedMemorySize, SMEM_ALLOC));
+    AVF_CUDA(cudaFuncSetAttribute(encoder_fused_kernel<IO_ROWS_F32, 0, 128>, cudaFuncAttributeMaxDynamicSharedMemorySize, SMEM_ALLOC));
   }
   const int cap = sm_cap();
   const int grid = min(a.n_tiles, cap > 0 ? min(cap, sm_count_cached()) : sm_count_cached());
   if (io_kind == IO_NCHW_BF16 && a.n_tok == 49 && NSPLIT == 2 && fixed_ntok_enabled())
-    launch_pdl(encoder_fused_kernel<IO_NCHW_BF16, 49>, grid, NUM_THREADS, SMEM_ALLOC, st, a);
+    launch_pdl(encoder_fused_kernel<IO_NCHW_BF16, 49, 256>, grid, NUM_THREADS, SMEM_ALLOC, st, a);
   else if (io_kind == IO_NCHW_BF16)
-    launch_pdl(encoder_fused_kernel<IO_NCHW_BF16, 0>, grid, NUM_THREADS, SMEM_ALLOC, st, a);
+    launch_pdl(encoder_fused_kernel<IO_NCHW_BF16, 0, 256>, grid, NUM_THREADS, SMEM_ALLOC, st, a);
+  else if (D == 256)
+    launch_pdl(encoder_fused_kernel<IO_ROWS_F32, 0, 256>, grid, NUM_THREADS, SMEM_ALLOC, st, a);
   else
-    launch_pdl(encoder_fused_kernel<IO_ROWS_F32, 0>, grid, NUM_THREADS, SMEM_ALLOC, st, a);
+    launch_pdl(encoder_fused_kernel<IO_ROWS_F32, 0, 128>, grid, NUM_THREADS, SMEM_ALLOC, st, a);
   AVF_LAUNCH_CHECK("encoder_fused_kernel");
   return 0;
 }
diff --git a/multi-modal-multi-label-facial-action-unit-detection-with-transformer_b200/encoder.py b/multi-modal-multi-label-facial-action-unit-detection-with-transformer_b200/encoder.py
--- a/multi-modal-multi-label-facial-action-unit-detection-with-transformer_b200/encoder.py
+++ b/multi-modal-multi-label-facial-action-unit-detection-with-transformer_b200/encoder.py
@@ -150,16 +150,19 @@
             seed ^= _rank_salt()
         return float(self.dropout), seed, self.dropout_salt
 
-    def forward_(self, x2d: torch.Tensor, n_seq: int, n_tok: int, out: Optional[torch.Tensor] = None, ld_out: int = 0) -> torch.Tensor:
+    def forward_(self, x2d: torch.Tensor, n_seq: int, n_tok: int, out: Optional[torch.Tensor] = None, ld_out: int = 0,
+                 pos: Optional[torch.Tensor] = None) -> torch.Tensor:
         p, seed, salt = self.dropout_state()
         if p > 0.0:
+            if pos is not None:
+                AF.add_row_periodic_(x2d, pos, n_tok)
             y, _ = AF.encoder_stack_fwd_train(x2d, self.packed(), self.shape(n_seq, n_tok), p, seed, salt)
             if out is None:
                 x2d.copy_(y)
                 return x2d
             torch.as_strided(out, (y.shape[0], y.shape[1]), (ld_out, 1)).copy_(y)
             return out
-        return AF.encoder_stack_fwd_(x2d, self.packed(), self.shape(n_seq, n_tok), out, ld_out)
+        return AF.token_stack_fwd_(x2d, self.packed(), self.shape(n_seq, n_tok), pos, out, ld_out)
 
     def forward_train(self, x2d: torch.Tensor, n_seq: int, n_tok: int) -> torch.Tensor:
         from .autograd import EncoderStackFn
diff --git a/multi-modal-multi-label-facial-action-unit-detection-with-transformer_b200/functional.py b/multi-modal-multi-label-facial-action-unit-detection-with-transformer_b200/functional.py
--- a/multi-modal-multi-label-facial-action-unit-detection-with-transformer_b200/functional.py
+++ b/multi-modal-multi-label-facial-action-unit-detection-with-transformer_b200/functional.py
@@ -131,6 +131,25 @@
     return x if out is None else out
 
 
+def token_stack_fwd_(x: torch.Tensor, packed: PackedStack, shape: StackShape, pos: Optional[torch.Tensor] = None,
+                     out: Optional[torch.Tensor] = None, ld_out: int = 0, w_last: Optional[torch.Tensor] = None, want_decisions: bool = False):
+    _cuda(x, "x")
+    if x.dtype != torch.float32 or x.stride(-1) != 1:
+        raise TypeError("token_stack_fwd_: x must be a float32 residual stream with unit column stride")
+    L = _lib.lib()
+    ws = workspace(L.avf_encoder_workspace_bytes(ctypes.byref(shape), packed.mode), x.device)
+    out21 = dec = None
+    if w_last is not None:
+        out21 = torch.empty((shape.n_seq, 21), dtype=torch.float32, device=x.device)
+        dec = torch.empty((shape.n_seq, 12), dtype=torch.int32, device=x.device) if want_decisions else None
+    check(L.avf_token_stack_fwd(packed.mode, ctypes.byref(shape), packed.array, _ptr(x), x.stride(0), _ptr(None if pos is None else _f32c(pos)),
+                                _ptr(out), ld_out, _ptr(None if w_last is None else _f32c(w_last)), _ptr(out21), _ptr(dec), _ptr(ws), ws.numel(),
+                                _stream()), "token_stack_fwd")
+    if w_last is not None:
+        return (out21, dec) if want_decisions else out21
+    return x if out is None else out
+
+
 def layernorm_fwd(x: torch.Tensor, gamma: torch.Tensor, beta: torch.Tensor, precision="bf16") -> torch.Tensor:
     x = _f32c(_cuda(x, "x"))
     rows, dim = x.numel() // x.shape[-1], x.shape[-1]
@@ -213,27 +232,27 @@
 
 
 def au_former_front(emb: torch.Tensor, ld_emb: int, n_clips: int, bn: Sequence[torch.Tensor], w_cat: torch.Tensor, b_cat: torch.Tensor,
-                    pos: torch.Tensor, mode: int) -> torch.Tensor:
+                    pos: Optional[torch.Tensor], mode: int) -> torch.Tensor:
     _cuda(emb, "emb")
     in_dim, emb_dim = w_cat.shape[1], w_cat.shape[0] // 12
     x = torch.empty((n_clips * 12, emb_dim), dtype=torch.float32, device=emb.device)
     ws = workspace(n_clips * in_dim * 4 + 256, emb.device)
     g, b, mu, var = (_f32c(t) for t in bn)
     check(_lib.lib().avf_au_former_front_fwd(mode, _ptr(emb), ld_emb, _ptr(g), _ptr(b), _ptr(mu), _ptr(var), _ptr(w_cat), _ptr(b_cat),
-                                             _ptr(_f32c(pos)), _ptr(x), n_clips, in_dim, emb_dim, _ptr(ws), ws.numel(), _stream()),
+                                             _ptr(None if pos is None else _f32c(pos)), _ptr(x), n_clips, in_dim, emb_dim, _ptr(ws), ws.numel(), _stream()),
           "au_former_front_fwd")
     return x
 
 
 def token_front(emb: torch.Tensor, ld_emb: int, n_clips: int, n_tok: int, bn: Sequence[torch.Tensor], w_cat: torch.Tensor, b_cat: torch.Tensor,
-                pos: torch.Tensor, mode: int) -> torch.Tensor:
+                pos: Optional[torch.Tensor], mode: int) -> torch.Tensor:
     _cuda(emb, "emb")
     in_dim, emb_dim = w_cat.shape[1], w_cat.shape[0] // n_tok
     x = torch.empty((n_clips * n_tok, emb_dim), dtype=torch.float32, device=emb.device)
     ws = workspace(n_clips * in_dim * 4 + 256, emb.device)
     g, b, mu, var = (_f32c(t) for t in bn)
     check(_lib.lib().avf_token_front_fwd(mode, _ptr(emb), ld_emb, _ptr(g), _ptr(b), _ptr(mu), _ptr(var), _ptr(w_cat), _ptr(b_cat),
-                                         _ptr(_f32c(pos)), _ptr(x), n_clips, in_dim, emb_dim, n_tok, _ptr(ws), ws.numel(), _stream()),
+                                         _ptr(None if pos is None else _f32c(pos)), _ptr(x), n_clips, in_dim, emb_dim, n_tok, _ptr(ws), ws.numel(), _stream()),
           "token_front_fwd")
     return x
 
@@ -272,6 +291,10 @@
 
 def set_fused_enabled(enabled: bool) -> bool:
     return bool(_lib.lib().avf_set_fused_enabled(1 if enabled else 0))
+
+
+def set_fused_small_enabled(enabled: bool) -> bool:
+    return bool(_lib.lib().avf_set_fused_small_enabled(1 if enabled else 0))
 
 
 def encoder_fused_supported(shape: StackShape, precision="bf16") -> bool:
diff --git a/multi-modal-multi-label-facial-action-unit-detection-with-transformer_b200/heads.py b/multi-modal-multi-label-facial-action-unit-detection-with-transformer_b200/heads.py
--- a/multi-modal-multi-label-facial-action-unit-detection-with-transformer_b200/heads.py
+++ b/multi-modal-multi-label-facial-action-unit-detection-with-transformer_b200/heads.py
@@ -70,10 +70,9 @@
             x, _ = AF.au_former_front_train(view, n_clips, bn.weight, bn.bias, bn.running_mean, bn.running_var, True,
                                             0.1 if bn.momentum is None else bn.momentum, f.w, f.b, self.pos_embedding[0], f.mode)
             bn.num_batches_tracked += 1
-        else:
-            x = AF.au_former_front(emb, ld_emb, n_clips, (bn.weight, bn.bias, bn.running_mean, bn.running_var), f.w, f.b,
-                                   self.pos_embedding[0], f.mode)
-        return self.corr_transformer.forward_(x, n_clips, 12, out, ld_out)
+            return self.corr_transformer.forward_(x, n_clips, 12, out, ld_out)
+        x = AF.au_former_front(emb, ld_emb, n_clips, (bn.weight, bn.bias, bn.running_mean, bn.running_var), f.w, f.b, None, f.mode)
+        return self.corr_transformer.forward_(x, n_clips, 12, out, ld_out, pos=self.pos_embedding[0])
 
     def front_params(self):
         return [p for i in range(1, 13) for p in (getattr(self, f"AU_linear_p{i}").weight, getattr(self, f"AU_linear_p{i}").bias)]
@@ -113,9 +112,12 @@
         return self._last
 
     def logits21_(self, tokens2d: torch.Tensor, n_clips: int, want_decisions: bool = False):
-        AF.add_row_periodic_(tokens2d, self.pos_embedding[0], 12)
-        self.corr_transformer.forward_(tokens2d, n_clips, 12)
-        return AF.au_logits(tokens2d, self._packed_last().w, n_clips, want_decisions)
+        t = self.corr_transformer
+        if t.training and t.dropout > 0.0:
+            t.forward_(tokens2d, n_clips, 12, pos=self.pos_embedding[0])
+            return AF.au_logits(tokens2d, self._packed_last().w, n_clips, want_decisions)
+        return AF.token_stack_fwd_(tokens2d, t.packed(), t.shape(n_clips, 12), self.pos_embedding[0], w_last=self._packed_last().w,
+                                   want_decisions=want_decisions)
 
     def last_params(self):
         return [getattr(self, f"AU_linear_last{i}").weight for i in range(1, 13)]
@@ -167,8 +169,8 @@
         emb = emb.detach().float().contiguous()
         f = self._packed_front()
         bn = self.VA_BN1
-        x = AF.token_front(emb, emb.shape[1], bs, 2, (bn.weight, bn.bias, bn.running_mean, bn.running_var), f.w, f.b, self.pos_embedding[0], f.mode)
-        tok = self.corr_transformer.forward_(x, bs, 2).view(bs, 2, -1)
+        x = AF.token_front(emb, emb.shape[1], bs, 2, (bn.weight, bn.bias, bn.running_mean, bn.running_var), f.w, f.b, None, f.mode)
+        tok = self.corr_transformer.forward_(x, bs, 2, pos=self.pos_embedding[0]).view(bs, 2, -1)
         w = torch.stack([self.VA_linear_last1.weight[0], self.VA_linear_last2.weight[0]]).float()
         va_out = (tok * w.unsqueeze(0)).sum(-1)
         return va_out, tok
```
